# Tanveer81/ReVisionLLM

Measured on AMD Instinct MI355X. Metric: video-segments/sec (whole node), stage-2 100-seg recursion, Vicuna-7B, higher is better.
Workload: dtype fp16

## Files before the change

### include/revision_hip.h

```cpp
#ifndef REVISION_HIP_H
#define REVISION_HIP_H

#include <stddef.h>
#include <stdint.h>

#ifdef __cplusplus
extern "C" {
#endif

#define RV_ABI_VERSION 5

typedef enum { RV_OK = 0, RV_ERR_ARG = -1, RV_ERR_UNBOUND = -2, RV_ERR_HIP = -3, RV_ERR_WORKSPACE = -4 } rv_status;
typedef enum { RV_F32 = 0, RV_BF16 = 1, RV_I32 = 2, RV_I64 = 3, RV_U8 = 4, RV_F16 = 5 } rv_dtype;
typedef enum { RV_ACT_NONE = 0, RV_ACT_RELU = 1, RV_ACT_SILU_MUL = 2, RV_ACT_QUICK_GELU = 3 } rv_act;
typedef enum { RV_W_ROWMAJOR = 0, RV_W_PACKED = 1 } rv_wlayout;
typedef enum { RV_FEAT_CLS = 0, RV_FEAT_ALL = 2 } rv_feature;

typedef struct rv_ctx rv_ctx;

typedef struct rv_config {
    int32_t hidden, inter, layers, heads, vocab;
    float rms_eps, rope_theta;
    int32_t adapter_dim, adapter_heads, adapter_ff, adapter_layers;
    int32_t adapter_text;
} rv_config;

#if defined(__GNUC__)
#pragma GCC visibility push(default)
#endif

int rv_abi_version(void);
int rv_operand_dtype(void);
int rv_last_error(char* buf, size_t n);

int rv_ctx_create(const rv_config* cfg, rv_ctx** out);
void rv_ctx_destroy(rv_ctx* ctx);
int rv_ctx_set_option(rv_ctx* ctx, const char* key, int64_t value);
int rv_ctx_get_option(const rv_ctx* ctx, const char* key, int64_t* value);
int rv_numeric_status_bind(uint32_t* status_dev);
int rv_weights_bind(rv_ctx* ctx, const char* name, const void* dptr, int dtype, int64_t numel);

int rv_init_hash(void* dst, int dtype, int64_t n, uint64_t key, float step, float base, void* stream);

size_t rv_gemm_ws_bytes(void);
int rv_gemv_fp8(const void* A, int64_t lda, const void* W8, const float* w_scale, const float* bias, const float* residual,
                int64_t ldr, void* C, int64_t ldc, int out_dtype, int act, int64_t M, int64_t N, int64_t K, void* stream);
int rv_rmsnorm_quant_fp8(const float* x, const float* w, void* q8, float* scale, int64_t rows, int32_t d, float eps, void* stream);
int rv_quant_rows_fp8(const void* x16, int64_t ldx, void* q8, int64_t ldq, float* scale, int64_t rows, int64_t K, void* stream);
int rv_gemm_fp8(const rv_ctx* ctx , const void* A8, int64_t lda, const float* a_scale, const void* W8p, const float* w_scale, const float* residual,
                int64_t ldr, void* C, int64_t ldc, int out_dtype, int act, int64_t M, int64_t N, int64_t K, void* ws, size_t ws_bytes,
                void* stream);
int rv_gemm(const rv_ctx* ctx , const void* A, int64_t lda, const void* W, int64_t ldw, int w_layout, const float* bias, const float* residual,
            int64_t ldr, void* C, int64_t ldc, int out_dtype, int act, int64_t M, int64_t N, int64_t K, void* ws,
            size_t ws_bytes, void* stream);
size_t rv_gemm_rows_ws_bytes(void);
int rv_gemm_rows(const void* Xp, const void* Wp, const float* w_scale, void* C, int32_t M, int32_t N, int32_t K, void* planes,
                 int32_t* arrive, int act, int out_dtype, void* stream);
int rv_layernorm(const float* x, const float* w, const float* b, float* y_f32, void* y_bf16, void* y_pos_bf16,
                 const float* pos, int64_t period, int64_t rows, int32_t d, void* stream);
int rv_rmsnorm(const float* x, const float* w, void* y_bf16, int64_t rows, int32_t d, float eps, void* stream);
int rv_sine_pos(float* pos, int32_t T, int32_t d, void* stream);
int rv_attention(const void* q, int64_t q_row_stride, int64_t q_batch_stride, const void* k, int64_t k_row_stride,
                 int64_t k_batch_stride, int64_t k_head_stride, const void* vt, int64_t vt_batch_stride,
                 int64_t vt_head_stride, int64_t vt_d_stride, void* out, int64_t o_row_stride, int64_t o_batch_stride,
                 const uint8_t* key_pad, int32_t B, int32_t H, int32_t dh, int32_t Lq, int32_t Lk, int32_t causal,
                 int32_t q_pos0, int32_t kv_batch_div, float scale, void* stream);

int rv_frames_to_patches(const uint8_t* frames, int layout, int64_t frame_stride, int64_t row_stride, int32_t n, int32_t H, int32_t W, int32_t R,
                         int32_t patch, const float mean[3], const float std[3], void* patches, int64_t ldp, float* image, void* stream);

int rv_yuv_to_patches(const uint8_t* y, int64_t y_frame_stride, int64_t y_row_stride, const uint8_t* cb, const uint8_t* cr, int64_t c_frame_stride,
                      int64_t c_row_stride, int32_t c_pix, int32_t n, int32_t H, int32_t W, int32_t matrix, int32_t full_range, int32_t chroma_loc,
                      int32_t R, int32_t patch, const float mean[3], const float std[3], void* patches, int64_t ldp, float* image, void* stream);

typedef struct rv_yuv_surface {
    const void *y, *cb, *cr;
    int64_t y_frame_stride, y_row_stride, c_frame_stride, c_row_stride;
    int32_t sample_bytes;
    int32_t depth;
    int32_t msb_aligned;
    int32_t c_pix;
    int32_t sub_x, sub_y;
    int32_t n, H, W;
    int32_t matrix;
    int32_t full_range;
    int32_t chroma_loc;
} rv_yuv_surface;
int rv_yuv_surface_to_patches(const rv_yuv_surface* s, int32_t R, int32_t patch, const float mean[3], const float std[3], void* patches, int64_t ldp,
                              float* image, void* stream);

int rv_project_dense(rv_ctx* ctx, const void* x_bf16, void* y, int out_dtype, int64_t rows, void* stream);
size_t rv_clip_encoder_ws_bytes(const rv_ctx* ctx, int32_t N, int32_t T, int32_t Nq, int32_t Lq);
int rv_clip_encoder(rv_ctx* ctx, const void* x, const void* txt, const uint8_t* txt_mask, int32_t N, int32_t T,
                    int32_t Nq, int32_t Lq, int32_t feature, float* out, void* ws, size_t ws_bytes, void* stream);

int rv_splice_embed(rv_ctx* ctx, const int32_t* map, const float* video_rows, float* h, int64_t rows, void* stream);
size_t rv_kv_bytes(const rv_ctx* ctx, int32_t B, int32_t Smax);
size_t rv_llm_ws_bytes(const rv_ctx* ctx, int32_t B, int32_t S);
int rv_llm_forward(rv_ctx* ctx, float* h, int32_t B, int32_t S, int32_t pos0, void* kv, int32_t Smax, float* logits,
                   void* ws, size_t ws_bytes, void* stream);

int rv_llm_layers(rv_ctx* ctx, float* h, int32_t B, int32_t S, int32_t pos0, void* kv, int32_t Smax, int32_t layer_begin,
                  int32_t layer_end, void* ws, size_t ws_bytes, void* stream);

size_t rv_llm_prefill_shared_ws_bytes(const rv_ctx* ctx, int32_t B, int32_t P0, int32_t S);
int rv_llm_prefill_shared(rv_ctx* ctx, float* h, int32_t B, int32_t P0, int32_t S, void* kv, int32_t Smax, float* logits,
                          void* ws, size_t ws_bytes, void* stream);

int rv_llm_prefill_pool(rv_ctx* ctx, float* h, int32_t B, int32_t P0, int32_t S, void* kv, int32_t kv_rows, int32_t kv_row0, int32_t Smax,
                        float* logits, void* ws, size_t ws_bytes, void* stream);
int rv_llm_prefill_pool_groups(rv_ctx* ctx, float* h, int32_t G, int32_t B, int32_t P0, int32_t S, void* kv, int32_t kv_rows,
                               const int32_t* kv_row0, int32_t Smax, float* logits, void* ws, size_t ws_bytes, void* stream);
int rv_llm_prefill_pool_groups_ragged(rv_ctx* ctx, float* h, int32_t G, int32_t B, int32_t P0, int32_t S, void* kv, int32_t kv_rows,
                                      const int32_t* kv_row0, int32_t Smax, const int32_t* last_rows, float* logits, void* ws, size_t ws_bytes,
                                      void* stream);
typedef struct rv_prefill_group { int32_t B, P0, S, kv_row0; } rv_prefill_group;
int rv_llm_prefill_pool_mixed(rv_ctx* ctx, float* h, int32_t G, const rv_prefill_group* groups, void* kv, int32_t kv_rows, int32_t Smax,
                              const int32_t* last_rows, float* logits, void* ws, size_t ws_bytes, void* stream);
int rv_llm_decode_rows(rv_ctx* ctx, float* h, int32_t R, const int32_t* row_pos, void* kv, int32_t Smax, float* logits, void* ws,
                       size_t ws_bytes, void* stream);
int rv_llm_decode_rows_shared(rv_ctx* ctx, float* h, int32_t R, const int32_t* row_pos, const int32_t* row_share, void* kv, int32_t Smax,
                              float* logits, void* ws, size_t ws_bytes, void* stream);

int rv_sample(const rv_ctx* ctx , const float* logits, int32_t B, int32_t V, const float* uniforms, int32_t do_sample, float temperature,
              int32_t top_k, float top_p, int32_t* out_tokens, float* out_entropy_proc, float* out_entropy_raw,
              int32_t* out_topk_idx, float* out_topk_val, int32_t* out_nkeep, float* out_threshold, void* stream);
int rv_entropy_stats(const float* logits, int32_t B, int32_t G, int32_t V, float* out, void* stream);
int rv_topk_cosine(const void* feat, int feat_dtype, const float* q_cls, int32_t n, int32_t T, int32_t d, int32_t k,
                   float* out, void* stream);

int rv_topk_pool(const void* video, int dtype, const float* text, int32_t Nv, int32_t T, int32_t d, int32_t Nt, int32_t k,
                 float* out, int32_t* out_idx, void* stream);

#if defined(__GNUC__)
#pragma GCC visibility pop
#endif

#ifdef __cplusplus
}
#endif
#endif
```

### revisionllm_amd/csrc/engine.hip

```cpp
#include <string>
#include <unordered_map>
#include <vector>

#include "kernels.h"

struct Tensor {
    const void* p = nullptr;
    int dtype = 0;
    int64_t numel = 0;
};

struct AdapterLayer {
    const op16_t *w_in, *w_out, *w1, *w2;
    const float *b_in, *b_out, *b1, *b2, *ln1_w, *ln1_b, *ln2_w, *ln2_b;
};
struct LlmLayer {
    const op16_t *wqkv, *wo, *wgu, *wdown;
    const float *norm1, *norm2;
    const uint8_t *wqkv8 = nullptr, *wo8 = nullptr, *wgu8 = nullptr, *wdown8 = nullptr;
    const float *sqkv = nullptr, *so = nullptr, *sgu = nullptr, *sdown = nullptr;
    const uint8_t *wqkv8p = nullptr, *wo8p = nullptr, *wgu8p = nullptr, *wdown8p = nullptr;
    const op16_t *wqkv2 = nullptr, *wo2 = nullptr, *wgu2 = nullptr, *wdown2 = nullptr;
};

// ... 380 lines not shown
        const int64_t RT = (int64_t)Nq * Lq;
        hipLaunchKernelGGL(invert_mask_kernel, dim3((unsigned)cdiv(RT, 256)), dim3(256), 0, st, txt_mask, w.pad, (int)RT);
        RV_CHECK_LAUNCH("invert_mask");
        float* v32 = w.x32;
        op16_t* vp16 = w.xp16;
        RV_TRY(k_frames_in(x, w.pm + d, s16 ? nullptr : v32, vp16, R0, T, (int)d, st));
        const op16_t* vres16 = (const op16_t*)x;
        for (size_t l = 0; l < c->t2v.size(); ++l) {
            const AdapterLayer& L = c->t2v[l];
            op16_t* q16 = w.qk16;
            RV_TRY(rv_gemm_impl(txt, d, L.w_in + d * d, d, 1, L.b_in + d, nullptr, 0, w.tk16, 2 * d, RV_OP16, RV_ACT_NONE, RT, 2 * d, d, w.sk, w.sk_bytes, st));
            const int LK = Lq <= 16 ? 16 : 32;
            const int64_t NK = (int64_t)H * LK, Rq = (int64_t)(N / Nq) * T;
            const bool fold = c->opt.adapter_fold_t2v != 0 && Lq <= 32 && dh <= 128 && NK % 64 == 0 && Rq > 32;
            if (fold) {
                float* S32 = (float*)w.qk16;
                op16_t* P16 = w.a16;
                RV_TRY(k_t2v_fold(L.w_in, L.b_in, L.w_out, w.tk16, w.tv16, 2 * d, Nq, Lq, LK, H, dh, scale, w.fa1, w.fc1, w.fa2, st));
                if (Nq > 1) {
                    RV_TRY(rv_gemm_grouped_impl(vp16, d, w.fa1, NK * d, w.fc1, NK, nullptr, 0, S32, NK, RV_F32, R0, NK, d, Rq, st));
                    RV_TRY(k_t2v_softmax(S32, w.pad, P16, R0, H, LK, Lq, Rq, st));
                    if (s16)
                        RV_TRY(rv_gemm_grouped_impl(P16, NK, w.fa2, NK * d, L.b_out, 0, (const float*)vres16, d, ys16, d, RV_OP16, R0, d, NK, Rq, st, 1));
                    else
                        RV_TRY(rv_gemm_grouped_impl(P16, NK, w.fa2, NK * d, L.b_out, 0, v32, d, w.y32, d, RV_F32, R0, d, NK, Rq, st));
                }
                for (int qi = 0; qi < Nq && Nq == 1; ++qi)
                    RV_TRY(rv_gemm_impl(vp16 + qi * Rq * d, d, w.fa1 + qi * NK * d, d, 1, w.fc1 + qi * NK, nullptr, 0, S32 + qi * Rq * NK, NK, RV_F32, RV_ACT_NONE, Rq, NK, d,
                                        w.sk, w.sk_bytes, st));
                if (Nq == 1) RV_TRY(k_t2v_softmax(S32, w.pad, P16, R0, H, LK, Lq, Rq, st));
                for (int qi = 0; qi < Nq && Nq == 1; ++qi) {
                    const int64_t r0 = qi * Rq;
                    if (s16)
                        RV_TRY(rv_gemm_impl(P16 + r0 * NK, NK, w.fa2 + qi * NK * d, NK, 1, L.b_out, (const float*)(vres16 + r0 * d), d, ys16 + r0 * d, d, RV_OP16, RV_ACT_NONE, Rq, d,
                                            NK, w.sk, w.sk_bytes, st, nullptr, 1));
                    else
                        RV_TRY(rv_gemm_impl(P16 + r0 * NK, NK, w.fa2 + qi * NK * d, NK, 1, L.b_out, v32 + r0 * d, d, w.y32 + r0 * d, d, RV_F32, RV_ACT_NONE, Rq, d, NK, w.sk,
                                            w.sk_bytes, st));
                }
            } else {
                RV_TRY(rv_gemm_impl(vp16, d, L.w_in, d, 1, L.b_in, nullptr, 0, q16, d, RV_OP16, RV_ACT_NONE, R0, d, d, w.sk, w.sk_bytes, st));
                RV_TRY(k_transpose_v(w.tv16, 2 * d, w.tvt16, Nq, Lq, w.Lqpad, H, dh, st));
                AttnArgs a{q16, d, (int64_t)T * d, w.tk16, 2 * d, (int64_t)Lq * 2 * d, dh, w.tvt16, (int64_t)d * w.Lqpad, (int64_t)dh * w.Lqpad,
                           w.Lqpad, w.a16, d, (int64_t)T * d, w.pad, N, H, dh, T, Lq, 0, 0, N / Nq, scale};
                RV_TRY(k_attention(a, st));
            }
            if (s16) {
                if (!fold)
                    RV_TRY(rv_gemm_impl(w.a16, d, L.w_out, d, 1, L.b_out, (const float*)vres16, d, ys16, d, RV_OP16, RV_ACT_NONE, R0, d, d, w.sk, w.sk_bytes, st, nullptr, 1));
                RV_TRY(k_layernorm(nullptr, L.ln1_w, L.ln1_b, nullptr, w.x16, nullptr, nullptr, 0, R0, (int)d, st, 0, ys16));
                RV_TRY(rv_gemm_impl(w.x16, d, L.w1, d, 1, L.b1, nullptr, 0, w.h16, ff, RV_OP16, RV_ACT_RELU, R0, ff, d, w.sk, w.sk_bytes, st));
                RV_TRY(rv_gemm_impl(w.h16, ff, L.w2, ff, 1, L.b2, (const float*)ys16, d, ys16, d, RV_OP16, RV_ACT_NONE, R0, d, ff, w.sk, w.sk_bytes, st, nullptr, 1));
                if (l + 1 < c->t2v.size()) {
                    RV_TRY(k_layernorm(nullptr, L.ln2_w, L.ln2_b, nullptr, xs16, vp16, w.pm + d, T, R0, (int)d, st, 0, ys16));
                    vres16 = xs16;
                } else {
                    RV_TRY(k_layernorm(nullptr, L.ln2_w, L.ln2_b, nullptr, w.x16, w.xp16, w.pm + d, T, R0, (int)d, st, T, ys16));
                    RV_TRY(k_cls_rows(c->cls_token, w.pm, nullptr, w.x16, w.xp16, N, T, (int)d, st));
                }
                continue;
            }
            if (!fold)
                RV_TRY(rv_gemm_impl(w.a16, d, L.w_out, d, 1, L.b_out, v32, d, w.y32, d, RV_F32, RV_ACT_NONE, R0, d, d, w.sk, w.sk_bytes, st));
            RV_TRY(k_layernorm(w.y32, L.ln1_w, L.ln1_b, nullptr, w.x16, nullptr, nullptr, 0, R0, (int)d, st));
            RV_TRY(rv_gemm_impl(w.x16, d, L.w1, d, 1, L.b1, nullptr, 0, w.h16, ff, RV_OP16, RV_ACT_RELU, R0, ff, d, w.sk, w.sk_bytes, st));
            RV_TRY(rv_gemm_impl(w.h16, ff, L.w2, ff, 1, L.b2, w.y32, d, w.y32, d, RV_F32, RV_ACT_NONE, R0, d, ff, w.sk, w.sk_bytes, st));
            if (l + 1 < c->t2v.size()) {
                RV_TRY(k_layernorm(w.y32, L.ln2_w, L.ln2_b, v32, nullptr, vp16, w.pm + d, T, R0, (int)d, st));
            } else {
                RV_TRY(k_layernorm(w.y32, L.ln2_w, L.ln2_b, w.x32, w.x16, w.xp16, w.pm + d, T, R0, (int)d, st, T));
                RV_TRY(k_cls_rows(c->cls_token, w.pm, w.x32, w.x16, w.xp16, N, T, (int)d, st));
            }
        }
    } else {
        RV_TRY(k_build_x(x, nullptr, c->cls_token, w.pm, s16 ? nullptr : w.x32, w.x16, w.xp16, N, T, (int)d, st));
    }

    for (size_t l = 0; l < c->enc.size(); ++l) {
        const AdapterLayer& L = c->enc[l];
        if (feature == RV_FEAT_CLS && l + 1 == c->enc.size() && N > 16 && T >= 3) {
            const int64_t sx = (int64_t)(T + 1) * d;
            op16_t* kk16 = w.qk16;
            op16_t* qc16 = w.h16;
            float* y0 = w.y32;
            float* y1 = w.y32 + (int64_t)N * d;
            float* y2 = w.y32 + (int64_t)2 * N * d;
            RV_TRY(rv_gemm_impl(w.xp16, d, L.w_in + d * d, d, 1, L.b_in + d, nullptr, 0, kk16, d, RV_OP16, RV_ACT_NONE, R1, d, d, w.sk, w.sk_bytes, st));
            RV_TRY(rv_gemm_impl(w.xp16, sx, L.w_in, d, 1, L.b_in, nullptr, 0, qc16, d, RV_OP16, RV_ACT_NONE, N, d, d, w.sk, w.sk_bytes, st, nullptr, 0, 1));
            RV_TRY(rv_gemm_impl(w.x16, d, L.w_in + 2 * d * d, d, 1, L.b_in + 2 * d, nullptr, 0, w.vv16, d, RV_OP16, RV_ACT_NONE, R1, d, d, w.sk, w.sk_bytes, st));
            RV_TRY(k_transpose_v(w.vv16, d, w.vt16, N, T + 1, w.Lpad, H, dh, st));
            AttnArgs a{qc16, d, d, kk16, d, (int64_t)(T + 1) * d, dh, w.vt16, (int64_t)d * w.Lpad, (int64_t)dh * w.Lpad, w.Lpad, w.a16, d, d,
                       nullptr, N, H, dh, 1, T + 1, 0, 0, 1, scale, 1};
            RV_TRY(k_attention(a, st));
            const float* cls_res = w.x32;
            int64_t cls_ld = sx;
            if (s16) {
                float* y3 = w.y32 + (int64_t)3 * N * d;
                RV_TRY(k_rows_to_f32(w.x16, sx, y3, N, (int)d, st));
                cls_res = y3;
                cls_ld = d;
            }
            RV_TRY(rv_gemm_impl(w.a16, d, L.w_out, d, 1, L.b_out, cls_res, cls_ld, y0, d, RV_F32, RV_ACT_NONE, N, d, d, w.sk, w.sk_bytes, st, nullptr, 0, 1));
            RV_TRY(k_layernorm(y0, L.ln1_w, L.ln1_b, y1, w.x16, nullptr, nullptr, 0, N, (int)d, st, 0, nullptr, s16 ? 3 : 0));
            RV_TRY(rv_gemm_impl(w.x16, d, L.w1, d, 1, L.b1, nullptr, 0, w.h16, ff, RV_OP16, RV_ACT_RELU, N, ff, d, w.sk, w.sk_bytes, st, nullptr, 0, 1));
            RV_TRY(rv_gemm_impl(w.h16, ff, L.w2, ff, 1, L.b2, y1, d, y2, d, RV_F32, RV_ACT_NONE, N, d, ff, w.sk, w.sk_bytes, st, nullptr, 0, 1));
            if (!c->adp_proj_w)
                return k_layernorm(y2, L.ln2_w, L.ln2_b, (float*)out, nullptr, nullptr, nullptr, 0, N, (int)d, st);
            RV_TRY(k_layernorm(y2, L.ln2_w, L.ln2_b, nullptr, w.x16, nullptr, nullptr, 0, N, (int)d, st, 0, nullptr, s16 ? 1 : 0));
            return rv_gemm_impl(w.x16, d, c->adp_proj_w, d, 1, c->adp_proj_b, nullptr, 0, out, D, RV_F32, RV_ACT_NONE, N, D, d, w.sk, w.sk_bytes, st, nullptr, 0, 1);
        }
        RV_TRY(rv_gemm_impl(w.xp16, d, L.w_in, d, 1, L.b_in, nullptr, 0, w.qk16, 2 * d, RV_OP16, RV_ACT_NONE, R1, 2 * d, d, w.sk, w.sk_bytes, st));
        RV_TRY(rv_gemm_impl(w.x16, d, L.w_in + 2 * d * d, d, 1, L.b_in + 2 * d, nullptr, 0, w.vv16, d, RV_OP16, RV_ACT_NONE, R1, d, d, w.sk, w.sk_bytes, st));
        RV_TRY(k_transpose_v(w.vv16, d, w.vt16, N, T + 1, w.Lpad, H, dh, st));
        AttnArgs a{w.qk16, 2 * d, (int64_t)(T + 1) * 2 * d, w.qk16 + d, 2 * d, (int64_t)(T + 1) * 2 * d, dh, w.vt16,
                   (int64_t)d * w.Lpad, (int64_t)dh * w.Lpad, w.Lpad, w.a16, d, (int64_t)(T + 1) * d, nullptr, N, H, dh, T + 1,
                   T + 1, 0, 0, 1, scale};
        RV_TRY(k_attention(a, st));
        if (s16) {
            RV_TRY(rv_gemm_impl(w.a16, d, L.w_out, d, 1, L.b_out, (const float*)w.x16, d, ys16, d, RV_OP16, RV_ACT_NONE, R1, d, d, w.sk, w.sk_bytes, st, nullptr, 1));
            RV_TRY(k_layernorm(nullptr, L.ln1_w, L.ln1_b, nullptr, w.x16, nullptr, nullptr, 0, R1, (int)d, st, 0, ys16));
            RV_TRY(rv_gemm_impl(w.x16, d, L.w1, d, 1, L.b1, nullptr, 0, w.h16, ff, RV_OP16, RV_ACT_RELU, R1, ff, d, w.sk, w.sk_bytes, st));
            RV_TRY(rv_gemm_impl(w.h16, ff, L.w2, ff, 1, L.b2, (const float*)w.x16, d, ys16, d, RV_OP16, RV_ACT_NONE, R1, d, ff, w.sk, w.sk_bytes, st, nullptr, 1));
            RV_TRY(k_layernorm(nullptr, L.ln2_w, L.ln2_b, nullptr, w.x16, w.xp16, w.pm, T + 1, R1, (int)d, st, 0, ys16));
            continue;
        }
        RV_TRY(rv_gemm_impl(w.a16, d, L.w_out, d, 1, L.b_out, w.x32, d, w.y32, d, RV_F32, RV_ACT_NONE, R1, d, d, w.sk, w.sk_bytes, st));
        RV_TRY(k_layernorm(w.y32, L.ln1_w, L.ln1_b, w.x32, w.x16, nullptr, nullptr, 0, R1, (int)d, st));
        RV_TRY(rv_gemm_impl(w.x16, d, L.w1, d, 1, L.b1, nullptr, 0, w.h16, ff, RV_OP16, RV_ACT_RELU, R1, ff, d, w.sk, w.sk_bytes, st));
        RV_TRY(rv_gemm_impl(w.h16, ff, L.w2, ff, 1, L.b2, w.x32, d, w.y32, d, RV_F32, RV_ACT_NONE, R1, d, ff, w.sk, w.sk_bytes, st));
        RV_TRY(k_layernorm(w.y32, L.ln2_w, L.ln2_b, w.x32, w.x16, w.xp16, w.pm, T + 1, R1, (int)d, st));
    }
    if (!c->adp_proj_w) {
        const hipError_t e = feature == RV_FEAT_CLS
                                 ? hipMemcpy2DAsync(out, (size_t)d * 4, w.x32, (size_t)(T + 1) * d * 4, (size_t)d * 4, (size_t)N, hipMemcpyDeviceToDevice, st)
                                 : hipMemcpyAsync(out, w.x32, (size_t)R1 * d * 4, hipMemcpyDeviceToDevice, st);
        if (e != hipSuccess) {
            rv_set_error("rv_clip_encoder: output copy failed: %s", hipGetErrorString(e));
            return RV_ERR_HIP;
        }
        return RV_OK;
    }
    if (feature == RV_FEAT_CLS)
        return rv_gemm_impl(w.x16, (int64_t)(T + 1) * d, c->adp_proj_w, d, 1, c->adp_proj_b, nullptr, 0, out, D, RV_F32, RV_ACT_NONE, N, D,
                            d, w.sk, w.sk_bytes, st);
    return rv_gemm_impl(w.x16, d, c->adp_proj_w, d, 1, c->adp_proj_b, nullptr, 0, out, D, RV_F32, RV_ACT_NONE, R1, D, d, w.sk, w.sk_bytes, st);
}

extern "C" int rv_splice_embed(rv_ctx* c, const int32_t* map, const float* video_rows, float* h, int64_t rows, void* stream) {
    RV_CHECK_ARG(c && map && h && rows > 0, "rv_splice_embed: bad arguments");
    RV_TRY(resolve_llm(c));
    return k_splice_embed(map, c->embed, video_rows, h, rows, c->cfg.hidden, as_stream(stream));
}

extern "C" size_t rv_kv_bytes(const rv_ctx* c, int32_t B, int32_t Smax) {
    if (!c || B <= 0 || Smax <= 0) return 0;
    return (size_t)2 * c->cfg.layers * B * c->cfg.hidden * (size_t)Smax * 2;
}

namespace {
inline bool llm_parity(const rv_ctx* c) { return c->opt.precision == 1 && c->w.count("llm.L0.wqkv.p2") != 0 && c->w.count("llm.lm_head.p2") != 0; }
struct LlmWs {
    op16_t *xn16, *q16, *a16, *act16, *xl16;
    float* g32;
    float *cs, *ss;
    float* planes;
    int* arrive;
    uint8_t* x8;
    float* sa;
    void* sk;
    size_t sk_bytes;
    size_t bytes;
};
inline const int* mixed_last_rows(const LlmWs& w) { return (const int*)((const char*)w.ss + sizeof(QkvGroup) * RV_MAX_PREFILL_GROUPS); }
inline size_t mixed_tables_bytes(const rv_ctx* c) { return (size_t)RV_XP_MAX_BLOCKS * (c->cfg.hidden / 16) * 16 * 4; }
LlmWs carve_llm(const rv_ctx* c, void* ws, size_t cap, int B, int S) {
    const int64_t M = (int64_t)B * S, D = c->cfg.hidden, F = c->cfg.inter;
    Carver k(ws, cap);
    LlmWs w;
    w.sk_bytes = gemm_pp_ws_bytes();
    w.sk = k.take(w.sk_bytes);
    w.arrive = (int*)k.take((size_t)RV_ROWS_COUNTERS * 4);
    const int64_t Mp = M <= RV_ROWS_MAX ? 16 * rv_xp_blocks(M) : M;
    const size_t par = llm_parity(c) ? 2 : 1;
    w.xn16 = (op16_t*)k.take((size_t)Mp * D * 2 * par);
    w.q16 = (op16_t*)k.take((size_t)M * D * 2 * par);
    w.a16 = (op16_t*)k.take((size_t)Mp * D * 2 * par);
    w.act16 = (op16_t*)k.take((size_t)Mp * F * 2 * par);
    w.xl16 = (op16_t*)k.take((size_t)Mp * D * 2 * 2);
    w.g32 = (float*)k.take(par == 2 ? (size_t)M * (F > 3 * D ? F : 3 * D) * 4 : 0);
    w.cs = (float*)k.take((size_t)S * (D / c->cfg.heads) * 4);
    w.ss = (float*)k.take((size_t)RV_XP_MAX_BLOCKS * (D / 16) * 16 * 4);
    w.planes = (float*)k.take(gemm_rows_ws_bytes());
    w.x8 = (uint8_t*)k.take((size_t)M * (F > D ? F : D));
    w.sa = (float*)k.take((size_t)M * 4);
    w.bytes = k.off;
    return w;
}
}

extern "C" size_t rv_llm_ws_bytes(const rv_ctx* c, int32_t B, int32_t S) {
    if (!c || B <= 0 || S <= 0) return 0;
    return carve_llm(c, nullptr, 0, 1, B * S).bytes;
}

namespace {
int llm_forward_impl(rv_ctx* c, float* h, int B, int S, int pos0, int P0, void* kv, int Smax, float* logits, void* ws,
                     size_t ws_bytes, hipStream_t st, int kv_rows = 0, int kv_row0 = 0, const int* row_pos = nullptr, int G = 1,
                     const int* grow = nullptr, int l0 = 0, int l1 = -1, const int* row_share = nullptr, const int* last_rows = nullptr,
                     const AttnMixed* mx = nullptr) {
    RV_TRY(resolve_llm(c));
    const rv_config& g = c->cfg;
    if (G > 1) kv_row0 = grow[0];
    const int64_t D = g.hidden, F = g.inter, V = g.vocab, Mg = (int64_t)B * S + P0, M = Mg * G;
    const LlmWs w = carve_llm(c, ws, ws_bytes, 1, (int)M);
    if (w.bytes > ws_bytes) {
        rv_set_error("rv_llm_forward: workspace %zu < required %zu", ws_bytes, w.bytes);
        return RV_ERR_WORKSPACE;
    }
    const int H = g.heads, dh = (int)(D / H);
    if (kv_rows <= 0) kv_rows = B;
    const int64_t per_layer = (int64_t)kv_rows * D * Smax;
    op16_t* kbase = (op16_t*)kv + (int64_t)kv_row0 * D * Smax;
    op16_t* vbase = (op16_t*)kv + (int64_t)g.layers * per_layer + (int64_t)kv_row0 * D * Smax;
    const float scale = 1.0f / sqrtf((float)dh);
    int mx_len = 0, mx_min = 0;
    int64_t nseq = (int64_t)G * B;
    if (mx) {
        nseq = 0;
        for (int gi = 0; gi < mx->G; ++gi) {
            const int len = mx->gt[gi].P0 + mx->gt[gi].S;
            mx_len = len > mx_len ? len : mx_len;
            mx_min = (gi == 0 || len < mx_min) ? len : mx_min;
            nseq += mx->gt[gi].B;
        }
    }
    const int tab0 = P0 > 0 ? 0 : pos0;
    if (row_pos) RV_TRY(k_rope_table_rows(w.cs, row_pos, B, dh, g.rope_theta, st));
    else RV_TRY(k_rope_table(w.cs, mx ? mx_len : pos0 + S - tab0, tab0, dh, g.rope_theta, st));
    const bool par = llm_parity(c);
    if (c->opt.precision == 1 && !par) {
        rv_set_error("rv_llm_forward: precision = 1 (parity) needs the K-duplicated weight copies (\"<name>.p2\") bound");
        return RV_ERR_UNBOUND;
    }
    const bool fuse_norm = !par && S == 1 && P0 == 0 && M <= RV_ROWS_MAX && D % 128 == 0 && F % 128 == 0 && (M <= 32 || (D % 64 == 0 && F % 32 == 0 && V % 64 == 0));
    const bool f8 = fuse_norm && c->fp8_decode && c->opt.fp8_decode;
    const bool p8 = !par && !fuse_norm && M > 32 && c->fp8_prefill && c->opt.fp8_prefill && w.sk_bytes >= 8192;
    const bool p8_qkv = p8 && gemm_pp_fp8_supported(M, 3 * D, D, false, true), p8_o = p8 && gemm_pp_fp8_supported(M, D, D, false, false);
    const bool p8_gu = p8 && gemm_pp_fp8_supported(M, 2 * F, D, true, false), p8_down = p8 && gemm_pp_fp8_supported(M, D, F, false, false);
    auto norm_quant = [&](const float* nw) -> int {
        if (D == 4096) return k_rmsnorm_quant(h, D, nw, w.x8, w.sa, M, (int)D, g.rms_eps, st);
        RV_TRY(k_rmsnorm(h, D, nw, w.xn16, M, (int)D, g.rms_eps, st));
        return k_quant_rows_fp8(w.xn16, D, w.x8, D, w.sa, M, (int)D, st);
    };
    const int nb_d = gemv_blocks(RV_ACT_NONE, D);
    const int xp = fuse_norm ? rv_xp_blocks(M) : 0;
    GemvNorm consume;
    consume.in_sumsq = w.ss;
    consume.in_nblk = nb_d;
    consume.inv_d = 1.0f / (float)D;
    consume.eps = g.rms_eps;
    consume.x_packed = xp;
    consume.out_packed = xp;
    consume.planes = w.planes;
    consume.arrive = w.arrive;
    if (l1 < 0 || l1 > g.layers) l1 = g.layers;
    const bool tail_block = logits && l1 == g.layers && !par && !p8 && !fuse_norm && !row_pos && (S > 1 || P0 > 0) && c->opt.last_block_rows &&
                            (mx ? (int64_t)mx_min : (int64_t)P0 + S) >= 32 && (size_t)M * F * 2 >= (((size_t)nseq * D * 4 + 255) & ~(size_t)255) + (size_t)nseq * F * 2;
    QkvGroup* mx_gt = (QkvGroup*)w.ss;
    if (mx) RV_TRY(k_mixed_tables(*mx, mx_gt, last_rows == mixed_last_rows(w) ? (int*)mixed_last_rows(w) : nullptr, st));
    for (int l = l0; l < l1; ++l) {
        const LlmLayer& L = c->layers[l];
        op16_t* kc = kbase + l * per_layer;
        op16_t* vtc = vbase + l * per_layer;
        if (par) RV_TRY(k_rmsnorm_split(h, D, L.norm1, w.xn16, M, (int)D, g.rms_eps, st));
        else if (p8_qkv) RV_TRY(norm_quant(L.norm1));
        else if (!fuse_norm || l == l0) RV_TRY(k_rmsnorm(h, D, L.norm1, w.xn16, M, (int)D, g.rms_eps, st, xp));
        QkvRope qr;
        qr.cs = w.cs;
        qr.q16 = w.q16;
        qr.kc = kc;
        qr.vtc = vtc;
        qr.B = B; qr.S = S; qr.P0 = P0; qr.pos0 = pos0; qr.cs_pos0 = tab0; qr.H = H; qr.Smax = Smax;
        qr.row_pos = row_pos;
        qr.G = G;
        qr.Mg = (int)Mg;
        for (int gi = 1; gi < G; ++gi) qr.grow[gi] = grow[gi] - grow[0];
        if (mx) {
            qr.ng = mx->G;
            qr.gt = mx_gt;
        }
        if (par) {
            qr.q_ld = (int)(2 * D);
            qr.q_lo = (int)D;
            RV_TRY(rv_gemm_impl(w.xn16, 2 * D, L.wqkv2, 2 * D, 1, nullptr, nullptr, 0, w.g32, 3 * D, RV_F32, RV_ACT_NONE, M, 3 * D, 2 * D, w.sk, w.sk_bytes, st, nullptr));
            RV_TRY(k_qkv_rope_split(w.g32, 3 * D, qr, M, D, st));
        } else if (p8_qkv) {
            RV_TRY(gemm_pp_fp8(w.x8, D, w.sa, L.wqkv8p, L.sqkv, nullptr, 0, nullptr, 0, RV_F32, RV_ACT_NONE, M, 3 * D, D, &qr, w.sk, st));
        } else if (f8) {
            GemvNorm cq = (fuse_norm && l > l0) ? consume : GemvNorm{};
            cq.w_scale = L.sqkv;
            cq.x_packed = xp;
            cq.planes = w.planes;
            cq.arrive = w.arrive;
            RV_TRY(gemm_qkv_rope(w.xn16, D, L.wqkv8, M, D, qr, &cq, nullptr, 0, st, 2));
        } else {
            GemvNorm first;
// ... 330 lines not shown
```

### revisionllm_amd/csrc/kernels.h

```cpp
#pragma once
#include "common.h"

struct RvOpts {
    int gemm_tile_variant = 2;
    int gemm_cus = 0;
    int fp8_decode = 1;
    int fp8_prefill = 1;
    int sample_variant = 1;
    int gemm_arows = 1;
    int gemm_waves = 8;
    int gemm_mhalf = 2;
    int rows_single = 1;
    int rows_persistent = 1;
    int rows_spread = 0;
    int rows_fill = 240;
    int lm_head_split = 1;
    int last_block_rows = 1;
    int adapter_stream16 = 1;
    int adapter_fold_t2v = 1;
    int attn_lds = 1;
    int qkv_lds = 1;
    int precision = 0;
};
extern const RvOpts g_default_opts;
// ... 50 lines not shown
    const QkvGroup e = q.gt[gi];
    m -= e.base;
    return e;
}
#ifndef RS_PROBE
#define RS_PROBE_K_ 0
#else
#define RS_PROBE_K_ RS_PROBE
#endif
static __device__ __forceinline__ f32x4 qkv_rope_coeffs(const QkvRope& q, int m, int n) {
    const int D = q.H * 128;
    const int sec = n / D, p = (n - sec * D) & 127;
    if (sec >= 2) return f32x4{0.f, 0.f, 0.f, 0.f};
    if constexpr ((RS_PROBE_K_ & 4096) != 0) return f32x4{1.f, 0.f, 1.f, 0.f};
    if (q.row_pos) return *(const f32x4*)(q.cs + ((int64_t)m * 64 + (p >> 1)) * 2);
    int P0 = q.P0, S = q.S, pos0 = q.pos0;
    if (q.ng) { const QkvGroup e = qkv_rope_group(q, m); P0 = pos0 = e.P0; S = e.S; }
    else if (q.G > 1) m -= (m / q.Mg) * q.Mg;
    int pos;
    if (m < P0) pos = m;
    else { const int r = m - P0; const int b = r / S; pos = pos0 + (r - b * S); }
    return *(const f32x4*)(q.cs + ((int64_t)(pos - q.cs_pos0) * 64 + (p >> 1)) * 2);
}
template <bool QSPLIT>
static __device__ __forceinline__ void qkv_rope_store_t(const QkvRope& q, int m, int n, f32x4 v, f32x4 t) {
    const int D = q.H * 128;
    const int sec = n / D, hd = n - sec * D, head = hd >> 7, p = hd & 127;
    int b, pos, goff = 0;
    bool prefix = false;
    const int mrow = m;
    int B = q.B, P0 = q.P0, S = q.S, pos0 = q.pos0;
    if (q.ng) { const QkvGroup e = qkv_rope_group(q, m); B = e.B; P0 = pos0 = e.P0; S = e.S; goff = e.row; }
    else if (q.G > 1) { const int gi = m / q.Mg; m -= gi * q.Mg; goff = q.grow[gi]; }
    if (q.row_pos) { b = m; pos = (RS_PROBE_K_ & 8192) ? 170 + (m & 7) : q.row_pos[m]; if (pos < 0 || pos >= q.Smax) return; }
    else if (m < P0) { b = 0; pos = m; prefix = true; }
    else { const int r = m - P0; b = r / S; pos = pos0 + (r - b * S); }
    if (sec < 2) {
        const float a0 = __fmaf_rn(v[0], t[0], -__fmul_rn(v[1], t[1])), b0 = __fmaf_rn(v[1], t[0], __fmul_rn(v[0], t[1]));
        const float a1 = __fmaf_rn(v[2], t[2], -__fmul_rn(v[3], t[3])), b1 = __fmaf_rn(v[3], t[2], __fmul_rn(v[2], t[3]));
        const u32x2 o = pack_op16x4(f32x4{a0, b0, a1, b1});
        if (sec == 0) {
            if constexpr ((RS_PROBE_K_ & 1024) != 0) return;
            if constexpr (QSPLIT) {
                op16_t* dst = (op16_t*)q.q16 + (int64_t)mrow * q.q_ld + hd;
                *(u32x2*)dst = o;
                *(u32x2*)(dst + q.q_lo) = u32x2{pack_op16x2_lo(a0, b0), pack_op16x2_lo(a1, b1)};
            } else {
                *(u32x2*)((op16_t*)q.q16 + (int64_t)mrow * D + hd) = o;
            }
        } else {
            if constexpr ((RS_PROBE_K_ & 512) != 0) return;
            const int b0_ = (prefix ? 0 : b) + goff, b1_ = (prefix ? B : b + 1) + goff;
            for (int bb = b0_; bb < b1_; ++bb)
                *(u32x2*)((op16_t*)q.kc + (((int64_t)bb * q.H + head) * q.Smax + pos) * 128 + p) = o;
        }
    } else {
        if constexpr ((RS_PROBE_K_ & 256) != 0) return;
        const int b0_ = (prefix ? 0 : b) + goff, b1_ = (prefix ? B : b + 1) + goff;
        for (int bb = b0_; bb < b1_; ++bb) {
            op16_t* dst = (op16_t*)q.vtc + ((int64_t)bb * q.H + head) * 128 * q.Smax + rv_vt_index(p, pos);
#pragma unroll
            for (int r = 0; r < 4; ++r) dst[r * 8] = f32_to_op16(v[r]);
        }
    }
}
static __device__ __forceinline__ void qkv_rope_store(const QkvRope& q, int m, int n, f32x4 v, f32x4 t) { qkv_rope_store_t<false>(q, m, n, v, t); }
struct QkvRow {
    int mrow, pos, b0, b1;
    const float* cs;
};
static __device__ __forceinline__ QkvRow qkv_rope_row(const QkvRope& q, int m) {
    QkvRow r;
    r.mrow = m;
    int goff = 0, b;
    bool prefix = false;
    int mt = m;
    int B = q.B, P0 = q.P0, S = q.S, pos0 = q.pos0;
    if (q.ng) { const QkvGroup e = qkv_rope_group(q, mt); B = e.B; P0 = pos0 = e.P0; S = e.S; goff = e.row; }
    else if (q.G > 1) { const int gi = m / q.Mg; mt = m - gi * q.Mg; goff = q.grow[gi]; }
    if (q.row_pos) { b = mt; r.pos = q.row_pos[mt]; r.cs = q.cs + (int64_t)mt * 128; }
    else {
        if (mt < P0) { b = 0; r.pos = mt; prefix = true; }
        else { const int rr = mt - P0; b = rr / S; r.pos = pos0 + (rr - b * S); }
        r.cs = q.cs + (int64_t)(r.pos - q.cs_pos0) * 128;
    }
    r.b0 = (prefix ? 0 : b) + goff;
    r.b1 = (prefix ? B : b + 1) + goff;
    if (q.row_pos && (r.pos < 0 || r.pos >= q.Smax)) r.b1 = r.b0 - 1;
    return r;
}
static __device__ __forceinline__ void qkv_rope_store(const QkvRope& q, int m, int n, f32x4 v) {
    qkv_rope_store(q, m, n, v, qkv_rope_coeffs(q, m, n));
}

int gemm_qkv_rope(const void* A, int64_t lda, const void* Wp, int64_t M, int64_t D, const QkvRope& r, const GemvNorm* norm,
                  void* ws, size_t ws_bytes, hipStream_t st, int w_layout = 1, int64_t Kdim = 0);

int rv_gemm_impl(const void* A, int64_t lda, const void* W, int64_t ldw, int w_layout, const float* bias,
                 const float* residual, int64_t ldr, void* C, int64_t ldc, int out_dtype, int act, int64_t M, int64_t N,
                 int64_t K, void* ws, size_t ws_bytes, hipStream_t st, const GemvNorm* norm = nullptr, int res16 = 0, int no_stream = 0);
struct GemmGroups {
    int rows = 0, tiles = 0;
    int64_t w_stride = 0, bias_stride = 0;
};
int rv_gemm_grouped_impl(const void* A, int64_t lda, const void* Wp, int64_t w_stride, const float* bias, int64_t bias_stride, const float* residual, int64_t ldr, void* C,
                         int64_t ldc, int out_dtype, int64_t M, int64_t N, int64_t K, int64_t rows_per_group, hipStream_t st, int res16 = 0);
int gemv_blocks(int act, int64_t N);
int gemm_rows(const op16_t* X, const op16_t* W, const float* bias, const float* res, int64_t ldr, void* C, int64_t ldc, int out_dtype, int act,
              int M, int N, int K, hipStream_t st, const GemvNorm& nrm, const QkvRope* qr, int w_layout = 1);
size_t gemm_rows_ws_bytes();
bool gemm_arows_supported(int w_layout, int act, int64_t M, int64_t N, int64_t K);
int gemm_arows_launch(const void* A, int64_t lda, const void* Wp, const float* bias, const float* res, int64_t ldr, void* C, int64_t ldc,
                      int out_dtype, int act, int64_t M, int64_t N, int64_t K, hipStream_t st);
bool gemm_pp_supported(int w_layout, int64_t M, int64_t N, int64_t K);
bool gemm_pp_sk_supported(int w_layout, int64_t M, int64_t N, int64_t K);
int gemm_pp_sk_plan(int64_t M, int64_t N, int64_t K, bool gated);
bool gemm_pp_sk_profitable(int64_t M, int64_t N, int64_t K);
bool gemm_pp_dp_profitable(int64_t M, int64_t N, int64_t K);
int gemm_pp_dp_plan(int64_t M, int64_t N, int64_t K, bool gated);
size_t gemm_pp_ws_bytes();
bool gemm_pp_fp8_supported(int64_t M, int64_t N, int64_t K, bool gated, bool rope);
int gemm_pp_fp8(const void* A8, int64_t lda, const float* sa, const void* W8p, const float* sw, const float* res, int64_t ldr, void* C,
                int64_t ldc, int out_dtype, int act, int64_t M, int64_t N, int64_t K, const QkvRope* r, void* ws, hipStream_t st);
int gemm_pp_launch(const void* A, int64_t lda, const void* Wp, const float* bias, const float* res, int64_t ldr, void* C,
                   int64_t ldc, int out_dtype, int act, int64_t M, int64_t N, int64_t K, void* ws, hipStream_t st);
int gemm_pp_qkv_rope(const void* A, int64_t lda, const void* Wp, int64_t M, int64_t N, int64_t K, const QkvRope& r, void* ws,
                     hipStream_t st);
int k_layernorm(const float* x, const float* w, const float* b, float* y32, void* y16, void* yp16, const float* pos,
                int64_t period, int64_t rows, int d, hipStream_t st, int64_t gap = 0, const void* x_op16 = nullptr, int rnd = 0);
int k_rmsnorm_quant(const float* x, int64_t x_row_stride, const float* w, void* q8, float* scale, int64_t rows, int d, float eps,
                    hipStream_t st);
int k_quant_rows_fp8(const void* x16, int64_t ldx, void* q8, int64_t ldq, float* scale, int64_t rows, int K, hipStream_t st);
int k_rmsnorm(const float* x, int64_t x_row_stride, const float* w, void* y16, int64_t rows, int d, float eps, hipStream_t st,
              int out_packed = 0, const int* row_idx = nullptr);
int k_rmsnorm_split(const float* x, int64_t x_row_stride, const float* w, void* y16, int64_t rows, int d, float eps, hipStream_t st, int out_packed = 0,
                    const int* row_idx = nullptr);
int k_split_bf16(const float* x, int64_t ldx, void* y16, int64_t rows, int n, hipStream_t st);
int k_qkv_rope_split(const float* qkv32, int64_t ld, const QkvRope& qr, int64_t M, int64_t D, hipStream_t st);
int k_gather_last_rows(const void* a16, const float* h, const int* idx, int64_t rows, int Mg, int P0, int B, int S, void* a_out, float* h_out, int D, hipStream_t st);
int k_t2v_fold(const void* wq_p, const float* bq, const void* wo_p, const void* tk16, const void* tv16, int64_t ld, int Nq, int Lq, int LK, int H, int dh, float scale,
               void* A1p, float* c1, void* A2p, hipStream_t st);
int k_t2v_softmax(const float* S, const uint8_t* pad, void* P16, int64_t rows, int H, int LK, int Lq, int64_t rows_per_query, hipStream_t st);
int k_sine_pos(float* pos, int T, int d, hipStream_t st);
int k_frames_in(const void* x16, const float* pos, float* v32, void* vp16, int64_t rows, int T, int d, hipStream_t st);
int k_build_x(const void* src16, const float* src32, const float* cls, const float* pm, float* x32, void* x16, void* xp16,
              int64_t N, int T, int d, hipStream_t st);
int k_copy_f32(const float* src, float* dst, int64_t n, hipStream_t st);
int k_rows_to_f32(const void* src16, int64_t ld, float* dst, int64_t rows, int d, hipStream_t st);
int k_cls_rows(const float* cls, const float* pm, float* x32, void* x16, void* xp16, int64_t N, int T, int d, hipStream_t st);
int k_transpose_v(const void* v, int64_t ld, void* vt, int64_t Nb, int L, int Lpad, int H, int dh, hipStream_t st);
int k_rope_table(float* cs, int S, int pos0, int dh, float theta, hipStream_t st);
int k_rope_table_rows(float* cs, const int* row_pos, int rows, int dh, float theta, hipStream_t st);
int k_splice_embed(const int32_t* map, const void* embed, const float* video, float* h, int64_t rows, int D, hipStream_t st);

struct AttnArgs {
    const void* q; int64_t q_rs, q_bs;
    const void* k; int64_t k_rs, k_bs, k_hs;
    const void* vt; int64_t vt_bs, vt_hs, vt_ds;
    void* out; int64_t o_rs, o_bs;
    const uint8_t* key_pad;
    int B, H, dh, Lq, Lk, causal, q_pos0, kv_div;
    float scale;
    int no_split = 0;
    const int* row_pos = nullptr;
    int out_packed = 0;
    int64_t vt_ks = 8;
    int64_t out_lo = 0;
    int64_t q_lo = 0;
    const int* row_share = nullptr;
};
int k_attention(const AttnArgs& a, hipStream_t st);
struct AttnGroups {
    int G = 1;
    int64_t q_off[RV_MAX_PREFILL_GROUPS] = {0, 0, 0, 0, 0, 0, 0, 0};
    int64_t o_off[RV_MAX_PREFILL_GROUPS] = {0, 0, 0, 0, 0, 0, 0, 0};
    int64_t kv_off[RV_MAX_PREFILL_GROUPS] = {0, 0, 0, 0, 0, 0, 0, 0};
};
int k_attention_pair(const AttnArgs& a, const AttnArgs& b, hipStream_t st, const AttnGroups* groups = nullptr);
int k_attention_groups(const AttnArgs& a, hipStream_t st, const AttnGroups& groups);
struct AttnMixed {
    int G = 0, problems = 0;
    int first[RV_MAX_PREFILL_GROUPS] = {};
    QkvGroup gt[RV_MAX_PREFILL_GROUPS] = {};
};
int k_attention_mixed(const AttnArgs& a, const AttnMixed& mx, hipStream_t st);
int k_mixed_tables(const AttnMixed& mx, QkvGroup* gt, int* last_rows, hipStream_t st);
```

### revisionllm_amd/csrc/rowops.hip

```cpp
#include "common.h"
#include "kernels.h"

namespace {

template <int NV>
__global__ __launch_bounds__(256) void layernorm_kernel(const float* __restrict__ x, const float* __restrict__ w,
                                                        const float* __restrict__ b, float* __restrict__ y32,
                                                        op16_t* __restrict__ y16, op16_t* __restrict__ yp16,
                                                        const float* __restrict__ pos, int64_t period, int64_t rows, int64_t gap,
                                                        const op16_t* __restrict__ x16in, int rnd) {
    constexpr int D = NV * 256;
    const int lane = threadIdx.x & 63;
    const int64_t row = (int64_t)blockIdx.x * 4 + (threadIdx.x >> 6);
    if (row >= rows) return;
    const float* xr = x + row * D;
    const int64_t orow = gap > 0 ? row + row / gap + 1 : row;
    f32x4 v[NV];
    float s = 0.f;
#pragma unroll
    for (int i = 0; i < NV; ++i) {
        v[i] = x16in ? op16x4_to_f32(*(const u32x2*)(x16in + row * D + i * 256 + lane * 4)) : *(const f32x4*)(xr + i * 256 + lane * 4);
        if (rnd & 1) v[i] = op16x4_to_f32(pack_op16x4(f32x4{v[i][0], v[i][1], v[i][2], v[i][3]}));
        s += v[i][0] + v[i][1] + v[i][2] + v[i][3];
    }
// ... 300 lines not shown
__device__ __forceinline__ int64_t rv_wp_index(int n, int k, int K) {
    return ((((int64_t)(n >> 4) * (K >> 5) + (k >> 5)) * 64 + (n & 15) + 16 * ((k >> 3) & 3)) * 8) + (k & 7);
}
__global__ __launch_bounds__(256) void t2v_fold_kernel(const op16_t* __restrict__ wq_p, const float* __restrict__ bq, const op16_t* __restrict__ wo_p,
                                                       const op16_t* __restrict__ tk, const op16_t* __restrict__ tv, int64_t ld, int Lq, int LK, int H, int dh, int d, float scale,
                                                       op16_t* __restrict__ A1p, float* __restrict__ c1, op16_t* __restrict__ A2p) {
    const int k = blockIdx.x * 256 + threadIdx.x;
    const int hj = blockIdx.y, h = hj / LK, j = hj % LK, q = blockIdx.z;
    const int NK = H * LK;
    __shared__ float kr[128], vr[128];
    const bool valid = j < Lq;
    for (int t = threadIdx.x; t < dh; t += 256) {
        kr[t] = valid ? op16_to_f32(tk[((int64_t)q * Lq + j) * ld + h * dh + t]) : 0.f;
        vr[t] = valid ? op16_to_f32(tv[((int64_t)q * Lq + j) * ld + h * dh + t]) : 0.f;
    }
    __syncthreads();
    if (k < d) {
        float a1 = 0.f, a2 = 0.f;
        for (int t = 0; t < dh; ++t) {
            a1 += kr[t] * op16_to_f32(wq_p[rv_wp_index(h * dh + t, k, d)]);
            a2 += vr[t] * op16_to_f32(wo_p[rv_wp_index(k, h * dh + t, d)]);
        }
        A1p[(int64_t)q * NK * d + rv_wp_index(hj, k, d)] = f32_to_op16(a1 * scale);
        A2p[(int64_t)q * NK * d + rv_wp_index(k, hj, NK)] = f32_to_op16(a2);
    }
    if (blockIdx.x == 0 && threadIdx.x < 64) {
        float c = 0.f;
        for (int t = threadIdx.x; t < dh; t += 64) c += kr[t] * bq[h * dh + t];
        c = wave_sum(c);
        if (threadIdx.x == 0) c1[(int64_t)q * NK + hj] = c * scale;
    }
}
template <int DH, int LK>
__global__ __launch_bounds__(256) void t2v_fold_reg_kernel(const op16_t* __restrict__ wq_p, const float* __restrict__ bq, const op16_t* __restrict__ wo_p,
                                                           const op16_t* __restrict__ tk, const op16_t* __restrict__ tv, int64_t ld, int Lq, int H, int d, float scale,
                                                           op16_t* __restrict__ A1p, float* __restrict__ c1, op16_t* __restrict__ A2p, int Nq, int qpw) {
    const int which = blockIdx.x & 1;
    const int k = (blockIdx.x >> 1) * 256 + threadIdx.x;
    const int h = blockIdx.y;
    const int NK = H * LK;
    __shared__ __attribute__((aligned(16))) float rr[LK][DH];
    float w[DH];
    const int kc = k < d ? k : d - 1;
#pragma unroll
    for (int t = 0; t < DH; ++t) w[t] = op16_to_f32(which ? wo_p[rv_wp_index(kc, h * DH + t, d)] : wq_p[rv_wp_index(h * DH + t, kc, d)]);
    const op16_t* rows = which ? tv : tk;
    const float mul = which ? 1.0f : scale;
    for (int q = blockIdx.z * qpw; q < Nq && q < (blockIdx.z + 1) * qpw; ++q) {
        __syncthreads();
        for (int i = threadIdx.x; i < LK * DH; i += 256) {
            const int j = i / DH, t = i - j * DH;
            rr[j][t] = j < Lq ? op16_to_f32(rows[((int64_t)q * Lq + j) * ld + h * DH + t]) : 0.f;
        }
        __syncthreads();
        if (k < d) {
#pragma unroll 2
            for (int j = 0; j < LK; ++j) {
                float acc = 0.f;
#pragma unroll
                for (int t = 0; t < DH; t += 4) {
                    const f32x4 kk = *(const f32x4*)&rr[j][t];
#pragma unroll
                    for (int e = 0; e < 4; ++e) acc += kk[e] * w[t + e];
                }
                const int hj = h * LK + j;
                if (which) A2p[(int64_t)q * NK * d + rv_wp_index(k, hj, NK)] = f32_to_op16(acc);
                else A1p[(int64_t)q * NK * d + rv_wp_index(hj, k, d)] = f32_to_op16(acc * mul);
            }
        }
        if (blockIdx.x == 0 && threadIdx.x < 64) {
            for (int j = 0; j < LK; ++j) {
                float c = 0.f;
                for (int t = threadIdx.x; t < DH; t += 64) c += rr[j][t] * bq[h * DH + t];
                c = wave_sum(c);
                if (threadIdx.x == 0) c1[(int64_t)q * NK + h * LK + j] = c * scale;
            }
        }
    }
}

template <int LK>
__global__ __launch_bounds__(256) void t2v_softmax_kernel(const float* __restrict__ S, const uint8_t* __restrict__ pad, op16_t* __restrict__ P, int64_t rows, int H, int Lq,
                                                          int64_t rows_per_query) {
    const int64_t i = (int64_t)blockIdx.x * 256 + threadIdx.x;
    if (i >= rows * H) return;
    const int64_t r = i / H;
    const uint8_t* pq = pad + (r / rows_per_query) * Lq;
    unsigned valid = 0u;
    for (int j = 0; j < Lq; ++j) valid |= (pq[j] == 0 ? 1u : 0u) << j;
    const f32x4* s4 = (const f32x4*)(S + i * LK);
    f32x4 v[LK / 4];
    float mx = -INFINITY;
#pragma unroll
    for (int c = 0; c < LK / 4; ++c) {
        v[c] = s4[c];
#pragma unroll
        for (int e = 0; e < 4; ++e) {
            if (!((valid >> (c * 4 + e)) & 1u)) v[c][e] = -INFINITY;
            mx = fmaxf(mx, v[c][e]);
        }
    }
    float z = 0.f;
#pragma unroll
    for (int c = 0; c < LK / 4; ++c)
#pragma unroll
        for (int e = 0; e < 4; ++e) {
            v[c][e] = mx == -INFINITY ? 0.f : __expf(v[c][e] - mx);
            z += v[c][e];
        }
    const float iz = z > 0.f ? 1.0f / z : 0.f;
    u32x2* p2 = (u32x2*)(P + i * LK);
#pragma unroll
    for (int c = 0; c < LK / 4; ++c) p2[c] = pack_op16x4(f32x4{v[c][0] * iz, v[c][1] * iz, v[c][2] * iz, v[c][3] * iz});
}

__global__ void rope_table_kernel(float2* __restrict__ cs, int S, int pos0, int dh, float theta) {
    const int i = blockIdx.x * blockDim.x + threadIdx.x;
    const int half = dh / 2;
    if (i >= S * half) return;
    const int s = i / half, j = i % half;
    const float inv = 1.0f / powf(theta, (float)(2 * j) / (float)dh);
    const float ang = (float)(pos0 + s) * inv;
    cs[i] = make_float2(cosf(ang), sinf(ang));
}

__global__ void rope_table_rows_kernel(float2* __restrict__ cs, const int* __restrict__ row_pos, int rows, int dh, float theta) {
    const int i = blockIdx.x * blockDim.x + threadIdx.x;
    const int half = dh / 2;
    if (i >= rows * half) return;
    const int s = i / half, j = i % half;
    const int pos = row_pos[s] > 0 ? row_pos[s] : 0;
    const float inv = 1.0f / powf(theta, (float)(2 * j) / (float)dh);
    const float ang = (float)pos * inv;
    cs[i] = make_float2(cosf(ang), sinf(ang));
}

__global__ __launch_bounds__(256) void splice_embed_kernel(const int32_t* __restrict__ map, const op16_t* __restrict__ embed,
                                                           const float* __restrict__ video, float* __restrict__ h, int D) {
    const int64_t r = blockIdx.x;
    const int src = map[r];
    float* o = h + r * D;
    if (src >= 0) {
        const op16_t* e = embed + (int64_t)src * D;
        for (int c = threadIdx.x * 4; c < D; c += 1024) {
            const u32x2 raw = *(const u32x2*)(e + c);
            *(f32x4*)(o + c) = op16x4_to_f32(raw);
        }
    } else {
        const float* v = video + (int64_t)(-(src + 1)) * D;
        for (int c = threadIdx.x * 4; c < D; c += 1024) *(f32x4*)(o + c) = *(const f32x4*)(v + c);
    }
}

}

int k_layernorm(const float* x, const float* w, const float* b, float* y32, void* y16, void* yp16, const float* pos,
                int64_t period, int64_t rows, int d, hipStream_t st, int64_t gap, const void* x_op16, int rnd) {
    RV_CHECK_ARG((x || x_op16) && w && b && rows >= 0, "layernorm: bad arguments");
    RV_CHECK_ARG(!yp16 || (pos && period > 0), "layernorm: y_pos needs pos table and period");
    if (rows == 0) return RV_OK;
    const unsigned blocks = (unsigned)cdiv(rows, 4);
    if (d == 768)
        hipLaunchKernelGGL(layernorm_kernel<3>, dim3(blocks), dim3(256), 0, st, x, w, b, y32, (op16_t*)y16, (op16_t*)yp16, pos, period, rows, gap, (const op16_t*)x_op16, rnd);
    else if (d == 4096)
        hipLaunchKernelGGL(layernorm_kernel<16>, dim3(blocks), dim3(256), 0, st, x, w, b, y32, (op16_t*)y16, (op16_t*)yp16, pos, period, rows, gap, (const op16_t*)x_op16, rnd);
    else if (d == 1024)
        hipLaunchKernelGGL(layernorm_kernel<4>, dim3(blocks), dim3(256), 0, st, x, w, b, y32, (op16_t*)y16, (op16_t*)yp16, pos, period, rows, gap, (const op16_t*)x_op16, rnd);
    else if (d == 256)
        hipLaunchKernelGGL(layernorm_kernel<1>, dim3(blocks), dim3(256), 0, st, x, w, b, y32, (op16_t*)y16, (op16_t*)yp16, pos, period, rows, gap, (const op16_t*)x_op16, rnd);
    else if (d == 512)
        hipLaunchKernelGGL(layernorm_kernel<2>, dim3(blocks), dim3(256), 0, st, x, w, b, y32, (op16_t*)y16, (op16_t*)yp16, pos, period, rows, gap, (const op16_t*)x_op16, rnd);
    else {
        rv_set_error("layernorm: unsupported width %d (256, 512, 768, 1024, 4096)", d);
        return RV_ERR_ARG;
    }
    RV_CHECK_LAUNCH("layernorm");
    return RV_OK;
}

int k_rmsnorm(const float* x, int64_t x_row_stride, const float* w, void* y16, int64_t rows, int d, float eps, hipStream_t st, int out_packed, const int* row_idx) {
    RV_CHECK_ARG(x && w && y16 && d % 4 == 0 && x_row_stride % 4 == 0, "rmsnorm: bad arguments");
    RV_CHECK_ARG(!out_packed || (rows <= 16 * out_packed && d % 32 == 0), "rmsnorm: the packed decode layout holds <= 16 rows per block");
    if (rows == 0) return RV_OK;
    const dim3 grid((unsigned)cdiv(rows, 4));
    if (d == 4096)
        hipLaunchKernelGGL(rmsnorm_kernel<16>, grid, dim3(256), 0, st, x, x_row_stride, w, (op16_t*)y16, rows, d, eps, out_packed, row_idx);
    else if (d == 512)
        hipLaunchKernelGGL(rmsnorm_kernel<2>, grid, dim3(256), 0, st, x, x_row_stride, w, (op16_t*)y16, rows, d, eps, out_packed, row_idx);
    else
        hipLaunchKernelGGL(rmsnorm_kernel<0>, grid, dim3(256), 0, st, x, x_row_stride, w, (op16_t*)y16, rows, d, eps, out_packed, row_idx);
    RV_CHECK_LAUNCH("rmsnorm");
    return RV_OK;
}

int k_rmsnorm_split(const float* x, int64_t x_row_stride, const float* w, void* y16, int64_t rows, int d, float eps, hipStream_t st, int out_packed, const int* row_idx) {
    RV_CHECK_ARG(x && w && y16 && d % 4 == 0 && x_row_stride % 4 == 0, "rmsnorm_split: bad arguments");
    RV_CHECK_ARG(!out_packed || (rows <= 16 * out_packed && d % 32 == 0), "rmsnorm_split: the packed decode layout holds <= 16 rows per block");
    if (rows == 0) return RV_OK;
    hipLaunchKernelGGL(rmsnorm_split_kernel, dim3((unsigned)cdiv(rows, 4)), dim3(256), 0, st, x, x_row_stride, w, (op16_t*)y16, rows, d, eps, out_packed, row_idx);
    RV_CHECK_LAUNCH("rmsnorm_split");
    return RV_OK;
}

int k_qkv_rope_split(const float* qkv32, int64_t ld, const QkvRope& qr, int64_t M, int64_t D, hipStream_t st) {
    RV_CHECK_ARG(qkv32 && qr.cs && qr.q16 && qr.kc && qr.vtc && qr.q_ld >= 2 * D && qr.q_lo >= D && ld % 4 == 0 && D == (int64_t)qr.H * 128, "qkv_rope_split: bad arguments");
    if (M == 0) return RV_OK;
    hipLaunchKernelGGL(qkv_rope_split_kernel, dim3((unsigned)cdiv(M * (3 * D / 4), 256)), dim3(256), 0, st, qkv32, ld, qr, M, (int)(3 * D));
    RV_CHECK_LAUNCH("qkv_rope_split");
    return RV_OK;
}

int k_split_bf16(const float* x, int64_t ldx, void* y16, int64_t rows, int n, hipStream_t st) {
    RV_CHECK_ARG(x && y16 && n % 4 == 0 && ldx % 4 == 0, "split_bf16: bad arguments");
    if (rows == 0) return RV_OK;
    hipLaunchKernelGGL(split_bf16_kernel, dim3((unsigned)cdiv(rows * n / 4, 256)), dim3(256), 0, st, x, ldx, (op16_t*)y16, rows, n);
    RV_CHECK_LAUNCH("split_bf16");
    return RV_OK;
}

int k_quant_rows_fp8(const void* x16, int64_t ldx, void* q8, int64_t ldq, float* scale, int64_t rows, int K, hipStream_t st) {
    RV_CHECK_ARG(x16 && q8 && scale && K > 0 && K % 8 == 0 && ldx % 8 == 0 && ldq % 8 == 0, "quant_rows_fp8: K, ldx, ldq must be multiples of 8");
    if (rows == 0) return RV_OK;
    hipLaunchKernelGGL(quant_rows_fp8_kernel, dim3((unsigned)cdiv(rows, 4)), dim3(256), 0, st, (const op16_t*)x16, ldx, (uint8_t*)q8, ldq,
                       scale, rows, K);
    RV_CHECK_LAUNCH("quant_rows_fp8");
    return RV_OK;
}

int k_rmsnorm_quant(const float* x, int64_t x_row_stride, const float* w, void* q8, float* scale, int64_t rows, int d, float eps,
                    hipStream_t st) {
    RV_CHECK_ARG(d == 4096, "rmsnorm_quant: d = %d (only 4096 is instantiated)", d);
    if (rows == 0) return RV_OK;
    hipLaunchKernelGGL(rmsnorm_quant_kernel<16>, dim3((unsigned)cdiv(rows, 4)), dim3(256), 0, st, x, x_row_stride, w, (uint8_t*)q8, scale, rows,
                       d, eps);
    RV_CHECK_LAUNCH("rmsnorm_quant");
    return RV_OK;
}

int k_sine_pos(float* pos, int T, int d, hipStream_t st) {
    RV_CHECK_ARG(pos && T > 0 && d > 0, "sine_pos: bad arguments");
    hipLaunchKernelGGL(sine_pos_kernel, dim3((unsigned)cdiv((int64_t)T * d, 256)), dim3(256), 0, st, pos, T, d);
    RV_CHECK_LAUNCH("sine_pos");
    return RV_OK;
}

int k_frames_in(const void* x16, const float* pos, float* v32, void* vp16, int64_t rows, int T, int d, hipStream_t st) {
    hipLaunchKernelGGL(frames_in_kernel, dim3((unsigned)cdiv(rows * d / 4, 256)), dim3(256), 0, st, (const op16_t*)x16, pos, v32,
                       (op16_t*)vp16, rows, T, d);
    RV_CHECK_LAUNCH("frames_in");
    return RV_OK;
}

int k_build_x(const void* src16, const float* src32, const float* cls, const float* pm, float* x32, void* x16, void* xp16,
              int64_t N, int T, int d, hipStream_t st) {
    hipLaunchKernelGGL(build_x_kernel, dim3((unsigned)cdiv(N * (T + 1) * d / 4, 256)), dim3(256), 0, st, (const op16_t*)src16,
                       src32, cls, pm, x32, (op16_t*)x16, (op16_t*)xp16, N, T, d);
    RV_CHECK_LAUNCH("build_x");
    return RV_OK;
}

int k_cls_rows(const float* cls, const float* pm, float* x32, void* x16, void* xp16, int64_t N, int T, int d, hipStream_t st) {
    hipLaunchKernelGGL(cls_rows_kernel, dim3((unsigned)cdiv(N * d / 4, 256)), dim3(256), 0, st, cls, pm, x32, (op16_t*)x16, (op16_t*)xp16, N, T, d);
    RV_CHECK_LAUNCH("cls_rows");
    return RV_OK;
}

int k_rows_to_f32(const void* src16, int64_t ld, float* dst, int64_t rows, int d, hipStream_t st) {
    hipLaunchKernelGGL(rows_to_f32_kernel, dim3((unsigned)cdiv(rows * d / 4, 256)), dim3(256), 0, st, (const op16_t*)src16, ld, dst, rows, d);
    RV_CHECK_LAUNCH("rows_to_f32");
    return RV_OK;
}

int k_copy_f32(const float* src, float* dst, int64_t n, hipStream_t st) {
    hipLaunchKernelGGL(copy_f32_kernel, dim3((unsigned)cdiv(n, 256)), dim3(256), 0, st, src, dst, n);
    RV_CHECK_LAUNCH("copy_f32");
    return RV_OK;
}

int k_transpose_v(const void* v, int64_t ld, void* vt, int64_t Nb, int L, int Lpad, int H, int dh, hipStream_t st) {
    RV_CHECK_ARG(Lpad % 2 == 0 && Lpad >= L, "transpose_v: bad Lpad");
    dim3 grid((unsigned)cdiv(Lpad, 64), (unsigned)H, (unsigned)Nb);
    if (dh == 96)
        hipLaunchKernelGGL(transpose_v_kernel<96>, grid, dim3(256), 0, st, (const op16_t*)v, ld, (op16_t*)vt, L, Lpad, H);
    else if (dh == 128)
        hipLaunchKernelGGL(transpose_v_kernel<128>, grid, dim3(256), 0, st, (const op16_t*)v, ld, (op16_t*)vt, L, Lpad, H);
    else if (dh == 512)
        hipLaunchKernelGGL(transpose_v_kernel<512>, dim3(grid.x, grid.y * 4, grid.z), dim3(256), 0, st, (const op16_t*)v, ld, (op16_t*)vt, L, Lpad, H);
    else {
        rv_set_error("transpose_v: head dim %d unsupported", dh);
        return RV_ERR_ARG;
    }
    RV_CHECK_LAUNCH("transpose_v");
    return RV_OK;
}

int k_gather_last_rows(const void* a16, const float* h, const int* idx, int64_t rows, int Mg, int P0, int B, int S, void* a_out, float* h_out, int D, hipStream_t st) {
    RV_CHECK_ARG(a16 && h && a_out && h_out && rows > 0 && D % 4 == 0, "gather_last_rows: bad arguments");
    hipLaunchKernelGGL(gather_last_rows_kernel, dim3((unsigned)rows), dim3(256), 0, st, (const op16_t*)a16, h, idx, Mg, P0, B, S, (op16_t*)a_out, h_out, D);
    RV_CHECK_LAUNCH("gather_last_rows");
    return RV_OK;
}

int k_t2v_fold(const void* wq_p, const float* bq, const void* wo_p, const void* tk16, const void* tv16, int64_t ld, int Nq, int Lq, int LK, int H, int dh, float scale,
               void* A1p, float* c1, void* A2p, hipStream_t st) {
    const int d = H * dh;
    RV_CHECK_ARG(wq_p && bq && wo_p && tk16 && tv16 && A1p && c1 && A2p && ld >= d && Nq > 0 && Lq > 0 && Lq <= LK && (LK == 16 || LK == 32) && dh <= 128 && d % 32 == 0,
                 "t2v_fold: bad arguments");
#define RV_FOLD_REG(DH_, LK_)                                                                                                                                  \
    hipLaunchKernelGGL((t2v_fold_reg_kernel<DH_, LK_>), dim3((unsigned)(2 * cdiv(d, 256)), (unsigned)H, (unsigned)cdiv(Nq, qpw)), dim3(256), 0, st, (const op16_t*)wq_p, bq, \
                       (const op16_t*)wo_p, (const op16_t*)tk16, (const op16_t*)tv16, ld, Lq, H, d, scale, (op16_t*)A1p, c1, (op16_t*)A2p, Nq, qpw)
    const bool reg = Nq >= 3;
    const int qpw = (int)cdiv((int64_t)Nq * 2 * cdiv(d, 256) * H, 1024);
    if (reg && dh == 96 && LK == 16) RV_FOLD_REG(96, 16);
    else if (reg && dh == 96 && LK == 32) RV_FOLD_REG(96, 32);
    else if (reg && dh == 64 && LK == 16) RV_FOLD_REG(64, 16);
    else if (reg && dh == 64 && LK == 32) RV_FOLD_REG(64, 32);
    else
        hipLaunchKernelGGL(t2v_fold_kernel, dim3((unsigned)cdiv(d, 256), (unsigned)(H * LK), (unsigned)Nq), dim3(256), 0, st, (const op16_t*)wq_p, bq, (const op16_t*)wo_p,
                           (const op16_t*)tk16, (const op16_t*)tv16, ld, Lq, LK, H, dh, d, scale, (op16_t*)A1p, c1, (op16_t*)A2p);
#undef RV_FOLD_REG
    RV_CHECK_LAUNCH("t2v_fold");
    return RV_OK;
}

int k_t2v_softmax(const float* S, const uint8_t* pad, void* P16, int64_t rows, int H, int LK, int Lq, int64_t rows_per_query, hipStream_t st) {
    RV_CHECK_ARG(S && pad && P16 && rows > 0 && (LK == 16 || LK == 32) && Lq <= LK && rows_per_query > 0, "t2v_softmax: bad arguments");
    if (LK == 16)
        hipLaunchKernelGGL(t2v_softmax_kernel<16>, dim3((unsigned)cdiv(rows * H, 256)), dim3(256), 0, st, S, pad, (op16_t*)P16, rows, H, Lq, rows_per_query);
    else
        hipLaunchKernelGGL(t2v_softmax_kernel<32>, dim3((unsigned)cdiv(rows * H, 256)), dim3(256), 0, st, S, pad, (op16_t*)P16, rows, H, Lq, rows_per_query);
    RV_CHECK_LAUNCH("t2v_softmax");
    return RV_OK;
}

int k_rope_table(float* cs, int S, int pos0, int dh, float theta, hipStream_t st) {
    hipLaunchKernelGGL(rope_table_kernel, dim3((unsigned)cdiv((int64_t)S * (dh / 2), 256)), dim3(256), 0, st, (float2*)cs, S, pos0, dh, theta);
    RV_CHECK_LAUNCH("rope_table");
    return RV_OK;
}

int k_rope_table_rows(float* cs, const int* row_pos, int rows, int dh, float theta, hipStream_t st) {
    hipLaunchKernelGGL(rope_table_rows_kernel, dim3((unsigned)cdiv((int64_t)rows * (dh / 2), 256)), dim3(256), 0, st, (float2*)cs, row_pos, rows, dh, theta);
    RV_CHECK_LAUNCH("rope_table_rows");
    return RV_OK;
}

int k_splice_embed(const int32_t* map, const void* embed, const float* video, float* h, int64_t rows, int D, hipStream_t st) {
    hipLaunchKernelGGL(splice_embed_kernel, dim3((unsigned)rows), dim3(256), 0, st, map, (const op16_t*)embed, video, h, D);
    RV_CHECK_LAUNCH("splice_embed");
    return RV_OK;
}

extern "C" int rv_layernorm(const float* x, const float* w, const float* b, float* y_f32, void* y_bf16, void* y_pos_bf16,
                            const float* pos, int64_t period, int64_t rows, int32_t d, void* stream) {
    return k_layernorm(x, w, b, y_f32, y_bf16, y_pos_bf16, pos, period, rows, d, as_stream(stream));
}
extern "C" int rv_rmsnorm(const float* x, const float* w, void* y_bf16, int64_t rows, int32_t d, float eps, void* stream) {
    return k_rmsnorm(x, d, w, y_bf16, rows, d, eps, as_stream(stream));
}
extern "C" int rv_rmsnorm_quant_fp8(const float* x, const float* w, void* q8, float* scale, int64_t rows, int32_t d, float eps, void* stream) {
    RV_CHECK_ARG(x && w && q8 && scale, "rv_rmsnorm_quant_fp8: null argument");
    return k_rmsnorm_quant(x, d, w, q8, scale, rows, d, eps, as_stream(stream));
}
extern "C" int rv_sine_pos(float* pos, int32_t T, int32_t d, void* stream) { return k_sine_pos(pos, T, d, as_stream(stream)); }
```

### revisionllm_amd/engine.py

```python
import ctypes as C

import torch

from . import hip, ops
from .utils import synth


def _dev_f32(t, device):
    return t.to(device=device, dtype=torch.float32).contiguous()


def _dev16(t, device, dtype):
    if dtype == torch.float16 and t.dtype != torch.float16:
        t = t.to(device=device, dtype=torch.float32).clamp(-65504.0, 65504.0)
    return t.to(device=device, dtype=dtype).contiguous()


class PersistGate:

    _by_device = {}

    def __init__(self):
        self._event = None

    @classmethod
    def for_device(cls, device):
        key = torch.device(device).index or 0
        if key not in cls._by_device:
            cls._by_device[key] = cls()
        return cls._by_device[key]

    def begin(self, stream=None):
        if self._event is not None:
            (stream or torch.cuda.current_stream()).wait_event(self._event)

    def end(self, stream=None):
        ev = torch.cuda.Event()
        ev.record(stream or torch.cuda.current_stream())
        self._event = ev


class Engine:
    def __init__(self, shape: synth.LlamaShape = synth.VICUNA_7B, adapter_text=True, device="cuda:0", adapter_dim=768,
                 adapter_heads=8, adapter_ff=2048, adapter_layers=2, gate=None, op_dtype=None):
        if not torch.cuda.is_available():
            raise hip.HipLibraryError("no GPU visible: revisionllm_amd runs only on the HIP device path")
        self.flavour = hip.flavour_of(op_dtype)
        self.op_dtype = hip.op_dtype(self.flavour)
        self.lib = hip.lib(self.flavour)
        self.shape = shape
        self.device = torch.device(device)
        self.adapter_text = bool(adapter_text)
        self.adapter_dim, self.adapter_ff, self.adapter_layers = adapter_dim, adapter_ff, adapter_layers
        cfg = hip.RvConfig(shape.hidden, shape.inter, shape.layers, shape.heads, shape.vocab, shape.eps, shape.theta,
                           adapter_dim, adapter_heads, adapter_ff, adapter_layers, int(adapter_text))
        self._ctx = C.c_void_p()
        hip.check(self.lib.rv_ctx_create(C.byref(cfg), C.byref(self._ctx)), "rv_ctx_create")
        self._keep = {}
        self._ws = {}
        self.slot = 0
        self.slots_in_flight = set()
        self.gate = gate if gate is not None else PersistGate.for_device(self.device)
        self.has_llm = self.has_clip = self.has_linear = False
        self.numeric_status = hip.numeric_status(self.flavour, self.device)
        self.on_saturation = "warn"
        self.saturated_seen = 0

    def __del__(self):
        try:
            if getattr(self, "_ctx", None) and self._ctx.value:
                self.lib.rv_ctx_destroy(self._ctx)
                self._ctx = C.c_void_p()
        except Exception:
            pass

    def set_option(self, key, value):
        hip.check(self.lib.rv_ctx_set_option(self._ctx, key.encode(), int(value)), f"rv_ctx_set_option({key})")
        return self

    def get_option(self, key):
        v = C.c_int64()
        hip.check(self.lib.rv_ctx_get_option(self._ctx, key.encode(), C.byref(v)), f"rv_ctx_get_option({key})")
        return int(v.value)

    def _dev16(self, t):
        return _dev16(t, self.device, self.op_dtype)

    def _dev_packed(self, t):
        return ops.pack_fragments(self._dev16(t))

    def bind(self, name, t):
        assert t.is_cuda and t.is_contiguous()
        self._keep[name] = t
        hip.check(self.lib.rv_weights_bind(self._ctx, name.encode(), hip.ptr(t), hip.dtype_code(t), t.numel()),
                  f"rv_weights_bind({name})")

    def weight(self, name):
        return self._keep[name]

    def _loaded(self):
        if self.device.type == "cuda":
            torch.cuda.synchronize(self.device)

    def _bind_matrix(self, name, w, fp8, fp8_prefill=False, parity=False):
        self.bind(name, ops.pack_fragments(w))
        if parity:
            self.bind(name + ".p2", ops.pack_fragments(torch.cat([w, w], dim=1).contiguous()))
        if fp8 or fp8_prefill:
            q, sc = ops.quantize_rows_fp8(w)
            self.bind(name + ".s8", sc)
            if fp8:
                self.bind(name + ".f8", ops.pack_fp8_decode(q))
            if fp8_prefill:
                self.bind(name + ".f8p", ops.pack_fp8_prefill(q))

    def load_llm(self, get, fp8_decode=False, fp8_prefill=False, parity=False):
        s, dev = self.shape, self.device
        self.parity = bool(parity)
        self.fp8_decode = bool(fp8_decode)
        self.fp8_prefill = bool(fp8_prefill)
        self.bind("llm.embed", self._dev16(get("model.embed_tokens.weight")))
        self._bind_matrix("llm.lm_head", self._dev16(get("lm_head.weight")), fp8_decode, parity=True)
        self.bind("llm.norm", _dev_f32(get("model.norm.weight"), dev))
        for i in range(s.layers):
            p = f"model.layers.{i}."
            q, k, v = (self._dev16(get(p + f"self_attn.{n}_proj.weight")) for n in "qkv")
            q, k = pair_interleave_heads(q, s.heads), pair_interleave_heads(k, s.heads)
            self._bind_matrix(f"llm.L{i}.wqkv", torch.cat([q, k, v], dim=0).contiguous(), fp8_decode, fp8_prefill, parity)
            del q, k, v
            self._bind_matrix(f"llm.L{i}.wo", self._dev16(get(p + "self_attn.o_proj.weight")), fp8_decode, fp8_prefill, parity)
            g = self._dev16(get(p + "mlp.gate_proj.weight"))
            u = self._dev16(get(p + "mlp.up_proj.weight"))
            self._bind_matrix(f"llm.L{i}.wgu", pack_gate_up(g, u), fp8_decode, fp8_prefill, parity)
            del g, u
            self._bind_matrix(f"llm.L{i}.wdown", self._dev16(get(p + "mlp.down_proj.weight")), fp8_decode, fp8_prefill, parity)
            self.bind(f"llm.L{i}.norm1", _dev_f32(get(p + "input_layernorm.weight"), dev))
            self.bind(f"llm.L{i}.norm2", _dev_f32(get(p + "post_attention_layernorm.weight"), dev))
        self.has_llm = True
        self._loaded()

    def load_clip_adapter(self, get):
        dev = self.device
        self.bind("adp.cls_token", _dev_f32(get("global_rep_token"), dev))
        self.bind("adp.cls_pos", _dev_f32(get("global_rep_pos"), dev))
        if self.adapter_dim == self.shape.hidden and self.adapter_dim != 768:
            self.txt_proj = (self._dev_packed(get("text_mm_projector.weight")), _dev_f32(get("text_mm_projector.bias"), dev))
        else:
            self.bind("adp.proj_w", self._dev_packed(get("mm_projector.weight")))
            self.bind("adp.proj_b", _dev_f32(get("mm_projector.bias"), dev))
        stacks = ([("t2v_encoder", "t2v")] if self.adapter_text else []) + [("encoder", "enc")]
        for ref, tag in stacks:
            for l in range(self.adapter_layers):
                r, o = f"{ref}.layers.{l}.", f"adp.{tag}.{l}."
                self.bind(o + "w_in", self._dev_packed(get(r + "self_attn.in_proj_weight")))
                self.bind(o + "b_in", _dev_f32(get(r + "self_attn.in_proj_bias"), dev))
                self.bind(o + "w_out", self._dev_packed(get(r + "self_attn.out_proj.weight")))
                self.bind(o + "b_out", _dev_f32(get(r + "self_attn.out_proj.bias"), dev))
                self.bind(o + "w1", self._dev_packed(get(r + "linear1.weight")))
                self.bind(o + "b1", _dev_f32(get(r + "linear1.bias"), dev))
                self.bind(o + "w2", self._dev_packed(get(r + "linear2.weight")))
                self.bind(o + "b2", _dev_f32(get(r + "linear2.bias"), dev))
                for n in ("1", "2"):
                    self.bind(o + f"ln{n}_w", _dev_f32(get(r + f"norm{n}.weight"), dev))
                    self.bind(o + f"ln{n}_b", _dev_f32(get(r + f"norm{n}.bias"), dev))
        self.has_clip = True
        self._loaded()

    def load_linear_projector(self, get):
        if self.adapter_dim != 768:
            self.frame_proj = (self._dev_packed(get("weight")), _dev_f32(get("bias"), self.device))
        else:
            self.bind("proj.w", self._dev_packed(get("weight")))
            self.bind("proj.b", _dev_f32(get("bias"), self.device))
        self.has_linear = True
        self._loaded()

    def _synth_get(self, spec, seed, prefix, grid=None):
        table = {n: (shp, a, base) for n, shp, a, base in spec}
        grid_dt = {None: None, "bf16": torch.bfloat16, "f16": torch.float16}[grid]

        def get(name):
            shp, a, base = table[name]
            t = torch.empty(shp, dtype=torch.float32, device=self.device)
            ops.init_hash_(t, prefix + name, seed, a, base)
            if grid_dt is not None and len(shp) > 1:
                t = t.to(grid_dt).float()
            return t
        return get

    def init_synthetic(self, seed=0, llm=True, clip=True, linear=False, llm_prefix="", clip_prefix="model.mm_projector.",
                       linear_prefix="model.mm_projector.", fp8_decode=False, fp8_prefill=False, cond=None, parity=False, grid=None):
        if llm:
            self.load_llm(self._synth_get(synth.llama_spec(self.shape, cond=cond), seed, llm_prefix, grid), fp8_decode=fp8_decode, fp8_prefill=fp8_prefill, parity=parity)
        if clip:
            self.load_clip_adapter(self._synth_get(synth.clip_encoder_spec(hidden=self.shape.hidden, text=self.adapter_text,
                                                                           cross_attn=self.adapter_dim != 768), seed,
                                                   clip_prefix, grid))
        if linear:
            self.load_linear_projector(self._synth_get(synth.linear_projector_spec(hidden=self.shape.hidden), seed, linear_prefix, grid))
        return self

    def _workspace(self, key, nbytes):
        key = (self.slot, key)
        t = self._ws.get(key)
        if t is None or t.numel() < nbytes:
            t = torch.zeros(max(int(nbytes), 256), dtype=torch.uint8, device=self.device)
            self._ws[key] = t
        return t

    _NUMERIC_KEY = ("numeric", "saturated")

    def _status_words(self):
        words = [(key, ws[8188:8192].view(torch.int32)) for key, ws in list(self._ws.items())
                 if isinstance(key, tuple) and key[0] != "kv" and key[1] in ("llm", "clip") and ws.numel() >= 8192]
        if words:
            words.append((self._NUMERIC_KEY, self.numeric_status[:1]))
        return words

    def saturated(self, reset=False):
        n = self.get_option("saturated")
        if reset:
            self.set_option("saturated", 0)
            self.saturated_seen = 0
        return n

    def _note_saturation(self, count):
        if count <= self.saturated_seen:
            return
        new, self.saturated_seen = count - self.saturated_seen, count
        msg = (f"{new} fp16 store(s) saturated at +-65504 since the last check ({count} in total): activations of this checkpoint leave the fp16 range; "
               "the affected elements lost accuracy (no inf was produced).  Use op_dtype='bf16' for the reference's exponent range.")
        if self.on_saturation == "raise":
            raise hip.HipLibraryError(msg)
        if self.on_saturation == "warn":
            import warnings
            warnings.warn(msg, RuntimeWarning, stacklevel=3)

    def handoff_status_async(self):
        words = self._status_words()
        if not words:
            return None
        host = torch.empty(len(words), dtype=torch.int32, pin_memory=True)
        host.copy_(torch.cat([w for _, w in words]), non_blocking=True)
        return [k for k, _ in words], host

    def check_handoff_status(self, snapshot=None):
        if snapshot is None:
            words = self._status_words()
            if not words:
                return
            keys, vals = [k for k, _ in words], torch.cat([w for _, w in words]).cpu()
        else:
            keys, vals = snapshot
        bad = [(k, int(v)) for k, v in zip(keys, vals.tolist()) if v != 0 and k != self._NUMERIC_KEY]
        sat = [int(v) & 0xffffffff for k, v in zip(keys, vals.tolist()) if k == self._NUMERIC_KEY]
        if sat:
            self._note_saturation(sat[0])
        if bad:
            for k, _ in bad:
                ws = self._ws.get(k)
                if ws is not None:
                    ws[8188:8192].zero_()
            key, st = bad[0]
            raise hip.HipLibraryError(f"workspace '{key}': an in-kernel hand-off wait timed out (status {st}); results of the last calls are invalid")

    def project_dense(self, x, out_dtype=torch.float32):
        lead = x.shape[:-1]
        x2 = self._dev16(x).reshape(-1, x.shape[-1])
        y = torch.empty(x2.shape[0], self.shape.hidden, dtype=out_dtype, device=self.device)
        hip.check(self.lib.rv_project_dense(self._ctx, hip.ptr(x2), hip.ptr(y), hip.dtype_code(y), x2.shape[0], hip.stream()),
                  "rv_project_dense")
        return y.reshape(*lead, self.shape.hidden)

    def clip_encoder(self, x, txt=None, txt_mask=None, feature="cls"):
        N, T, _ = x.shape
        x = self._dev16(x)
        wide = self.adapter_dim != 768
        if wide:
            if getattr(self, "frame_proj", None) is None or getattr(self, "txt_proj", None) is None:
                raise hip.HipLibraryError("the cross_attn ClipEncoder needs the Linear projector (load_linear_projector) and its text projector bound")
            x = ops.gemm(x.reshape(N * T, -1), self.frame_proj[0], bias=self.frame_proj[1], out_dtype=self.op_dtype, w_packed=True,
                         ctx=self).view(N, T, self.adapter_dim)
        if self.adapter_text:
            txt = self._dev16(txt)
            Nq, Lq = txt.shape[0], txt.shape[1]
            if wide:
                txt = ops.gemm(txt.reshape(Nq * Lq, -1), self.txt_proj[0], bias=self.txt_proj[1], out_dtype=self.op_dtype, w_packed=True,
                               ctx=self).view(Nq, Lq, self.adapter_dim)
            m = ops.h2d((txt_mask != 0).to(torch.uint8), self.device).contiguous()
        else:
            txt, m, Nq, Lq = None, None, 0, 0
        feat = hip.RV_FEAT_CLS if feature == "cls" else hip.RV_FEAT_ALL
        D = self.shape.hidden
        out = torch.empty((N, D) if feat == hip.RV_FEAT_CLS else (N, T + 1, D), dtype=torch.float32, device=self.device)
        nbytes = self.lib.rv_clip_encoder_ws_bytes(self._ctx, N, T, Nq, Lq)
        ws = self._workspace("clip", nbytes)
        hip.check(self.lib.rv_clip_encoder(self._ctx, hip.ptr(x), hip.ptr(txt), hip.ptr(m), N, T, Nq, Lq, feat, hip.ptr(out),
                                           hip.ptr(ws), ws.numel(), hip.stream()), "rv_clip_encoder")
        return out

    def splice_embed(self, row_map, video_rows):
        B, S = row_map.shape
        h = torch.empty(B, S, self.shape.hidden, dtype=torch.float32, device=self.device)
        rm = ops.h2d(row_map, self.device, torch.int32).contiguous()
        vr = _dev_f32(video_rows, self.device) if video_rows is not None else None
        hip.check(self.lib.rv_splice_embed(self._ctx, hip.ptr(rm), hip.ptr(vr), hip.ptr(h), B * S, hip.stream()), "rv_splice_embed")
        return h

    def new_kv(self, B, Smax, reuse=True):
        Smax = (Smax + 31) // 32 * 32
        key = ("kv", self.slot, B, Smax)
        t = self._ws.get(key) if reuse else None
        if t is None:
            nbytes = self.lib.rv_kv_bytes(self._ctx, B, Smax)
            t = torch.zeros(nbytes // 2, dtype=self.op_dtype, device=self.device)
            if reuse:
                for k_ in [k_ for k_ in self._ws if isinstance(k_, tuple) and k_[0] == "kv" and k_[1] == self.slot][:-3]:
                    del self._ws[k_]
                self._ws[key] = t
        return t, Smax

    @staticmethod
    def vt_logical(vt, *lead, head_dim=128, Smax=None):
        return vt.view(*lead, Smax // 8, head_dim, 8).movedim(-3, -2).reshape(*lead, head_dim, Smax)

    def _persist_begin(self):
        self.gate.begin(torch.cuda.current_stream(self.device))

    def _persist_end(self):
        self.gate.end(torch.cuda.current_stream(self.device))

    def llm_forward(self, h, pos0, kv, Smax, logits=None):
        B, S, _ = h.shape
        assert h.dtype == torch.float32 and h.is_contiguous()
        if logits is None:
            logits = torch.empty(B, self.shape.vocab, dtype=torch.float32, device=self.device)
        nbytes = self.lib.rv_llm_ws_bytes(self._ctx, B, S)
        ws = self._workspace("llm", nbytes)
        if B * S > 16:
            self._persist_begin()
        hip.check(self.lib.rv_llm_forward(self._ctx, hip.ptr(h), B, S, pos0, hip.ptr(kv), Smax, hip.ptr(logits), hip.ptr(ws),
                                          ws.numel(), hip.stream()), "rv_llm_forward")
        if B * S > 16:
            self._persist_end()
        return logits


    def llm_layers(self, h, pos0, kv, Smax, layer_begin, layer_end):
        B, S, _ = h.shape
        assert h.dtype == torch.float32 and h.is_contiguous()
        ws = self._workspace("llm", self.lib.rv_llm_ws_bytes(self._ctx, B, S))
        if B * S > 16:
            self._persist_begin()
        hip.check(self.lib.rv_llm_layers(self._ctx, hip.ptr(h), B, S, pos0, hip.ptr(kv), Smax, layer_begin, layer_end, hip.ptr(ws), ws.numel(),
                                         hip.stream()), "rv_llm_layers")
        if B * S > 16:
            self._persist_end()
        return h

    def llm_prefill_shared(self, h, B, P0, kv, Smax, logits=None):
        assert h.dtype == torch.float32 and h.is_contiguous() and (h.shape[0] - P0) % B == 0
        S = (h.shape[0] - P0) // B
        if logits is None:
            logits = torch.empty(B, self.shape.vocab, dtype=torch.float32, device=self.device)
        ws = self._workspace("llm", self.lib.rv_llm_prefill_shared_ws_bytes(self._ctx, B, P0, S))
        self._persist_begin()
        hip.check(self.lib.rv_llm_prefill_shared(self._ctx, hip.ptr(h), B, P0, S, hip.ptr(kv), Smax, hip.ptr(logits), hip.ptr(ws),
                                                 ws.numel(), hip.stream()), "rv_llm_prefill_shared")
        self._persist_end()
        return logits


    def new_kv_pool(self, rows, Smax):
        Smax = (Smax + 31) // 32 * 32
        nbytes = self.lib.rv_kv_bytes(self._ctx, rows, Smax)
        return torch.zeros(nbytes // 2, dtype=self.op_dtype, device=self.device), Smax

    def llm_prefill_pool(self, h, B, P0, kv, kv_rows, kv_row0, Smax, logits=None):
        assert h.dtype == torch.float32 and h.is_contiguous() and (h.shape[0] - P0) % B == 0
        S = (h.shape[0] - P0) // B
        if logits is None:
            logits = torch.empty(B, self.shape.vocab, dtype=torch.float32, device=self.device)
        ws = self._workspace("llm", self.lib.rv_llm_prefill_shared_ws_bytes(self._ctx, B, P0, S))
        self._persist_begin()
        hip.check(self.lib.rv_llm_prefill_pool(self._ctx, hip.ptr(h), B, P0, S, hip.ptr(kv), kv_rows, kv_row0, Smax, hip.ptr(logits), hip.ptr(ws),
                                               ws.numel(), hip.stream()), "rv_llm_prefill_pool")
        self._persist_end()
        return logits

    def llm_prefill_pool_groups(self, h, G, B, P0, kv, kv_rows, row0s, Smax, logits=None, last_rows=None):
        import ctypes
        assert h.dtype == torch.float32 and h.is_contiguous() and h.shape[0] % G == 0 and (h.shape[0] // G - P0) % B == 0
        S = (h.shape[0] // G - P0) // B
        if logits is None:
            logits = torch.empty(G * B, self.shape.vocab, dtype=torch.float32, device=self.device)
        ws = self._workspace("llm", self.lib.rv_llm_ws_bytes(self._ctx, h.shape[0], 1))
        rows = (ctypes.c_int32 * G)(*[int(r) for r in row0s])
        self._persist_begin()
        if last_rows is not None:
            assert last_rows.dtype == torch.int32 and last_rows.is_cuda and last_rows.numel() == G * B
            hip.check(self.lib.rv_llm_prefill_pool_groups_ragged(self._ctx, hip.ptr(h), G, B, P0, S, hip.ptr(kv), kv_rows, rows, Smax, hip.ptr(last_rows),
                                                                 hip.ptr(logits), hip.ptr(ws), ws.numel(), hip.stream()), "rv_llm_prefill_pool_groups_ragged")
        else:
            hip.check(self.lib.rv_llm_prefill_pool_groups(self._ctx, hip.ptr(h), G, B, P0, S, hip.ptr(kv), kv_rows, rows, Smax, hip.ptr(logits), hip.ptr(ws),
                                                          ws.numel(), hip.stream()), "rv_llm_prefill_pool_groups")
        self._persist_end()
        return logits

    def mixed_prefill_supported(self):
        return not (self.get_option("precision") == 1 or (getattr(self, "fp8_prefill", False) and self.get_option("fp8_prefill")))

    def llm_prefill_pool_mixed(self, h, groups, kv, R, Smax, last_rows=None, logits=None):
        groups = [tuple(int(v) for v in g) for g in groups]
        rows, nb = sum(P0 + B * S for B, P0, S, _ in groups), sum(g[0] for g in groups)
        assert h.dtype == torch.float32 and h.is_contiguous() and h.shape[0] == rows, (tuple(h.shape), rows)
        if logits is None:
            logits = torch.empty(nb, self.shape.vocab, dtype=torch.float32, device=self.device)
        ws = self._workspace("llm", self.lib.rv_llm_ws_bytes(self._ctx, max(rows, 1), 1))
        tab = (hip.RvPrefillGroup * max(len(groups), 1))(*[hip.RvPrefillGroup(*g) for g in groups])
        if last_rows is not None:
            assert last_rows.dtype == torch.int32 and last_rows.is_cuda and last_rows.numel() == nb
        self._persist_begin()
        try:
            hip.check(self.lib.rv_llm_prefill_pool_mixed(self._ctx, hip.ptr(h), len(groups), tab, hip.ptr(kv), R, Smax, hip.ptr(last_rows), hip.ptr(logits), hip.ptr(ws),
                                                         ws.numel(), hip.stream()), "rv_llm_prefill_pool_mixed")
        finally:
            self._persist_end()
        return logits

    def llm_decode_rows(self, h, row_pos, kv, Smax, logits=None, row_share=None):
        R = h.shape[0]
        assert h.dtype == torch.float32 and h.is_contiguous() and row_pos.dtype == torch.int32 and row_pos.is_cuda
        if logits is None:
            logits = torch.empty(R, self.shape.vocab, dtype=torch.float32, device=self.device)
        ws = self._workspace("llm", self.lib.rv_llm_ws_bytes(self._ctx, R, 1))
        if row_share is not None:
            assert row_share.dtype == torch.int32 and row_share.is_cuda and row_share.numel() == R
            hip.check(self.lib.rv_llm_decode_rows_shared(self._ctx, hip.ptr(h), R, hip.ptr(row_pos), hip.ptr(row_share), hip.ptr(kv), Smax, hip.ptr(logits),
                                                         hip.ptr(ws), ws.numel(), hip.stream()), "rv_llm_decode_rows_shared")
            return logits
        hip.check(self.lib.rv_llm_decode_rows(self._ctx, hip.ptr(h), R, hip.ptr(row_pos), hip.ptr(kv), Smax, hip.ptr(logits), hip.ptr(ws), ws.numel(),
                                              hip.stream()), "rv_llm_decode_rows")
        return logits


def pair_interleave_heads(w, heads):
    rows, D = w.shape
    dh = rows // heads
    return w.view(heads, 2, dh // 2, D).transpose(1, 2).reshape(rows, D).contiguous()


def pack_gate_up(gate, up):
    F, D = gate.shape
    assert F % 16 == 0
    return torch.stack([gate.view(F // 16, 16, D), up.view(F // 16, 16, D)], dim=1).reshape(2 * F, D).contiguous()
```

### revisionllm_amd/eval/stage2.py

```python
import json
import math
import re

import numpy as np
import torch

from .. import ops, sched
from ..inference import _decode, _prompt_ids, inference
from ..model.adapter import pad_sequences_1d

QUERY_TEMPLATE = "During which video can we see {}?"


def cut_windows(ctx_l, debug_window=125, feature_fps=5, stride=5, num_frames=250):
    clip_length = debug_window * feature_fps
    num_window = math.ceil(ctx_l / (clip_length // stride)) - 1
    times, idx = [], []
    for i in range(num_window):
        start = max(i * clip_length // stride, 0)
        end = min(i * clip_length // stride + clip_length, ctx_l - 1)
        if end - start < clip_length:
            start = end - clip_length
        times.append((start, end))
        idx.append(np.linspace(start, end, num_frames, dtype=np.int32))
    return times, (np.stack(idx) if idx else np.zeros((0, num_frames), np.int32))


def plan_groups(W, batch, zooms=(4, 2, 1)):
    plan = []
    for z in zooms:
        b = batch // z
        for g in range(math.ceil(W / b)):
            start = g * b
            end = min(start + b, W)
            if end - start < b:
                start = end - b
            plan.append((z, start, end))
    return plan


def group_span(W, start, end):
    r = range(W)[start:end]
    return (r.start if len(r) else 0), len(r)


def get_ground_truth_windows(start, end, duration):
    clip_len = 0.2
    start, end = start / clip_len, end / clip_len
    size = int(900 / 2)
    ids = list(range(math.floor(start / size), math.ceil(end / size) + 1))
    return ids, math.ceil(duration / clip_len / size) + 1


def answer_to_window(output, zoom, index, start, grounding_windows):
    m = re.search(r"(\d+)", output)
    if not m:
        return None
    n = int(m.group(1)) // zoom
    if n < len(index):
        n = int(index[n])
    n = min(len(grounding_windows) - 1, max(0, start + n))
    return grounding_windows[n]


def iou(outputs, gt, num_frames_clip, num_frames_video, starts, indexes, single, hierarchy_zooms, grounding_windows):
    clip_frames, frames = {}, []
    for i, output in enumerate(outputs):
        w = answer_to_window(output, hierarchy_zooms[i], indexes[i], starts[i], grounding_windows)
        if w is None:
            continue
        f, t = max(0, w - 1), min(num_frames_video, w + 1)
        clip_frames[i] = (int(f), int(t))
        frames.append((f, t))
    s, e = min(gt), max(gt)
    inter = [max(0, min(t, e) - max(f, s)) for f, t in frames]
    return clip_frames, [1] if sum(inter) > 0 else [0]


def write_log(log_path, video_id, task, query_id, answer, info=None):
    log = {"video_id": video_id, "task": task, "query_id": query_id, "answer": answer}
    if info is not None:
        log["info"] = info
    with open(log_path, "a") as f:
        f.write(json.dumps(log) + "\n")


def _proposal_rows(answer0, n_group_rows, zooms_so_far, indexes, starts, i_inner, grounding_windows, single=True):
    m = None
    if not single:
        m = re.search(r"(\d+) (to|and) (\d+)", answer0)
    if not m:
        m = re.search(r"(\d+)", answer0)
    if not m:
        return None
    n = int(m.group(1)) // zooms_so_far[i_inner]
    if n < len(indexes[i_inner]):
        n = int(indexes[i_inner][n])
    n = min(len(grounding_windows) - 1, max(0, starts[i_inner] + n))
    w = grounding_windows[n]
    return list(range(max(0, w - 1), min(w + 1, n_group_rows - 1)))


def _steps_until_eos(new_tokens, eos):
    G = new_tokens.shape[1]
    if eos is None:
        return [G] * new_tokens.shape[0]
    out = []
    for row in new_tokens.tolist():
        out.append(row.index(eos) + 1 if eos in row else G)
    return out



def encode_windows(model, features, query_feats):
    mask = torch.ones(1, query_feats.shape[0])
    return model.engine.clip_encoder(features, query_feats[None], mask, "cls")


def window_cosine(features, query_cls, k=3):
    return ops.topk_cosine(features, query_cls, min(features.shape[1], k))


def call_row_index(plan, perms, device, W=None):
    firsts = [start if start >= 0 else group_span(W, start, end)[0] for _, start, end in plan]
    idx = [(f + p.long()).repeat_interleave(z) if z > 1 else f + p.long() for f, (z, _, _), p in zip(firsts, plan, perms)]
    return ops.h2d(torch.cat(idx), device), [int(i.numel()) for i in idx]


def build_call_rows(cls, plan, perms, index=None):
    idx, counts = index if index is not None else call_row_index(plan, perms, cls.device, cls.shape[0])
    return list(cls.index_select(0, idx).split(counts))


def launch_calls(model, tokenizer, query, rows, calls, uniforms=None, max_new_tokens=1024, max_calls_per_generate=16, width=None,
                 forced_tokens=None):
    return sched.drive(launch_calls_steps(model, tokenizer, query, rows, calls, uniforms, max_new_tokens, max_calls_per_generate, width,
                                          forced_tokens))


def launch_calls_steps(model, tokenizer, query, rows, calls, uniforms=None, max_new_tokens=1024, max_calls_per_generate=16, width=None,
                       forced_tokens=None, server=None):
    ids_of = {}

    def prompt_ids(c):
        q = query if isinstance(query, str) else query[c]
        if q not in ids_of:
            ids_of[q] = _prompt_ids(q, tokenizer, 1)[0]
        return ids_of[q]

    ragged = server is not None and getattr(server, "prefill_batch", 1) > 1 and getattr(server, "ragged", True)
    groups = {}
    for c in calls:
        groups.setdefault((None if ragged else rows[c].shape[0], prompt_ids(c).shape[1]), []).append(c)
    order, toks, ents = [], [], []
    for (_, _), cs in groups.items():
        for c0 in range(0, len(cs), max_calls_per_generate):
            sel = cs[c0:c0 + max_calls_per_generate]
            counts = [int(rows[c].shape[0]) for c in sel]
            n_rows = counts[0] if len(set(counts)) == 1 else counts
            ids = torch.cat([prompt_ids(c) for c in sel], 0)
            u = None if uniforms is None else uniforms[:, sel]
            forced = None if forced_tokens is None else forced_tokens[:, sel]
            out = yield from model.generate_steps(ids, video_rows=torch.cat([rows[c] for c in sel], 0), rows_per_sample=n_rows,
                                                  do_sample=True, temperature=0.05, num_beams=1, max_new_tokens=max_new_tokens,
                                                  output_scores=False, return_dict_in_generate=True, uniforms=u, forced_tokens=forced,
                                                  server=server, new_tokens_only=True)
            order.extend(sel)
            toks.append(out["new_tokens"] if out.get("new_tokens") is not None else out["sequences"][:, ids.shape[1]:])
            ents.append(out["entropy"])
    dev = model.engine.device
    if not order:
        w0 = width or 0
        return [], torch.zeros(0, w0, dtype=torch.int32, device=dev), torch.zeros(0, w0, device=dev), torch.zeros(0, dtype=torch.int32, device=dev)
    width = width or max(t.shape[1] for t in toks)
    if len(toks) == 1 and toks[0].shape[1] == width and toks[0].dtype == torch.int32:
        return order, toks[0], ents[0], torch.full((len(order),), width, dtype=torch.int32, device=dev)
    tok = torch.zeros(len(order), width, dtype=torch.int32, device=dev)
    ent = torch.zeros(len(order), width, dtype=torch.float32, device=dev)
    nst = torch.empty(len(order), dtype=torch.int32, device=dev)
    r = 0
    for t, e in zip(toks, ents):
        n, g = t.shape
        if g > width:
            raise ValueError(f"a call generated {g} tokens > wire capacity {width}")
        tok[r:r + n, :g] = t
        ent[r:r + n, :g] = e
        nst[r:r + n] = g
        r += n
    return order, tok, ent, nst


def finish_calls(order, tok, ent, nst, eos):
    res = {}
    for j, c in enumerate(order):
        n = int(nst[j])
        row = tok[j, :n]
        g = _steps_until_eos(row[None], eos)[0]
        e = ent[j, :g]
        res[c] = (row[:g].tolist(), float(e.max()), float(e.mean()))
    return res


def generate_calls(model, tokenizer, query, rows, calls, uniforms=None, max_new_tokens=1024, max_calls_per_generate=16, forced_tokens=None):
    order, tok, ent, nst = launch_calls(model, tokenizer, query, rows, calls, uniforms, max_new_tokens, max_calls_per_generate,
                                        forced_tokens=forced_tokens)
    tok, ent, nst = tok.cpu(), ent.cpu(), nst.cpu()
    model.engine.check_handoff_status()
    return finish_calls(order, tok, ent, nst, model.generation_config.eos_token_id)


def assemble(plan, perms, call_results, cos, tokenizer, zooms, grounding_windows, single=True):
    stop_str = "</s>"
    W = len(cos)
    answers, max_ent, mean_ent, score_cos, starts, indexes, hz = [], [], [], [], [], [], []
    i_call = 0
    for z in zooms:
        level = [p for p in plan if p[0] == z]
        for i, (_, start, end) in enumerate(level):
            idx = perms[i_call]
            toks, emax, emean = call_results[i_call]
            text = tokenizer.batch_decode([toks], skip_special_tokens=True)[0].strip()
            if text.endswith(stop_str):
                text = text[:-len(stop_str)]
            text = text.strip()
            starts.append(start)
            indexes.append(idx)
            hz.append(z)
            answers.append(text)
            max_ent.append(1 / emax)
            mean_ent.append(1 / emean)
            first, count = (start, end - start) if start >= 0 else group_span(W, start, end)
            prop = _proposal_rows(text, count * z, hz, indexes, starts, i, grounding_windows, single)
            if prop is None:
                score_cos.append(0)
            else:
                score_cos.extend(float(cos[first + int(idx[n // z])]) for n in prop)
            i_call += 1
    return dict(answers=answers, starts=starts, indexes=indexes, hierarchy_zooms=hz, max_entropy=max_ent,
                mean_entropy=mean_ent, score_cos=score_cos, grounding_windows=grounding_windows, plan=plan)


def make_perms(plan, generator=None, W=None):
    return [torch.randperm(end - start if start >= 0 else group_span(W, start, end)[1], generator=generator) for _, start, end in plan]


def run_query(model, tokenizer, features, query_feats, query_cls, sentence, batch=100, zooms=(4, 2, 1), perms=None,
              mode="batched", grounding_windows=None, uniforms=None, max_new_tokens=1024, max_calls_per_generate=16, single=True,
              forced_tokens=None):
    W = features.shape[0]
    if grounding_windows is None:
        grounding_windows = list(range(W))
    zooms = tuple(zooms)
    if W == 0:
        return dict(answers=[], starts=[], indexes=[], hierarchy_zooms=[], max_entropy=[], mean_entropy=[], score_cos=[],
                    grounding_windows=grounding_windows, plan=[])
    plan = plan_groups(W, batch, zooms)
    perms = [torch.as_tensor(p).long() for p in (perms if perms is not None else make_perms(plan, W=W))]
    query = "<video>\n" + QUERY_TEMPLATE.format(sentence)

    if mode == "batched":
        index = call_row_index(plan, perms, features.device, W)
        cls = encode_windows(model, features, query_feats)
        cos = window_cosine(features, query_cls)
        rows = build_call_rows(cls, plan, perms, index)
        res = generate_calls(model, tokenizer, query, rows, list(range(len(plan))), uniforms, max_new_tokens, max_calls_per_generate,
                             forced_tokens)
        return assemble(plan, perms, res, cos.cpu(), tokenizer, zooms, grounding_windows, single)
    if mode != "reference":
        raise ValueError(f"mode must be 'reference' or 'batched', got {mode!r}")

    qf = pad_sequences_1d(query_feats[None], dtype=query_feats.dtype, device=query_feats.device)
    answers, max_ent, mean_ent, score_cos, starts, indexes, hz = [], [], [], [], [], [], []
    i_call = 0
    for z in zooms:
        level = [p for p in plan if p[0] == z]
        for i, (_, start, end) in enumerate(level):
            idx = perms[i_call]
            feat = features[start:end][None][:, idx.to(features.device)]
            if z > 1:
                feat = feat.repeat_interleave(z, 1)
            starts.append(start)
            indexes.append(idx)
            ans, out = inference(model, feat, qf, query, tokenizer, return_list=True)
            answers.extend(ans)
            hz.append(z)
            st = ops.entropy_stats(torch.stack(out["scores"], 1))
            max_ent.extend(1 / float(e[0]) for e in st)
            mean_ent.extend(1 / float(e[2]) for e in st)
            prop = _proposal_rows(ans[0], feat.shape[1], hz, indexes, starts, i, grounding_windows, single)
            if prop is None:
                score_cos.append(0)
            elif prop:
                sc = ops.topk_cosine(feat[0, prop[0]:prop[-1] + 1], query_cls, min(feat.shape[2], 3))
                score_cos.extend(float(x) for x in sc.tolist())
            i_call += 1
    return dict(answers=answers, starts=starts, indexes=indexes, hierarchy_zooms=hz, max_entropy=max_ent,
                mean_entropy=mean_ent, score_cos=score_cos, grounding_windows=grounding_windows, plan=plan)


def log_record(res, timestamps, batch, num_frames=250, single=True):
    frames, ious = iou(res["answers"], timestamps, num_frames, batch, res["starts"], res["indexes"], single,
                       res["hierarchy_zooms"], res["grounding_windows"])
    return {"gt": timestamps, "frames": frames, "iou": ious, "score_cos": res["score_cos"], "mean_entropy": res["mean_entropy"],
            "max_entropy": res["max_entropy"], "hierarchy_zooms": res["hierarchy_zooms"]}
```

### revisionllm_amd/hip.py

```python
import ctypes as C
import os

import torch

_HERE = os.path.dirname(os.path.abspath(__file__))
LIB_PATHS = {"f16": os.environ.get("REVISION_HIP_LIB") or os.path.join(_HERE, "librevision_hip.so"),
             "bf16": os.environ.get("REVISION_HIP_LIB_BF16") or os.path.join(_HERE, "librevision_hip_bf16.so")}
LIB_PATH = LIB_PATHS["f16"]
OP_DTYPES = {"f16": torch.float16, "bf16": torch.bfloat16}

RV_F32, RV_BF16, RV_I32, RV_I64, RV_U8, RV_F16 = 0, 1, 2, 3, 4, 5
RV_ACT_NONE, RV_ACT_RELU, RV_ACT_SILU_MUL, RV_ACT_QUICK_GELU = 0, 1, 2, 3
RV_FEAT_CLS, RV_FEAT_ALL = 0, 2
TOPK_CAP = 64

_DT = {torch.float32: RV_F32, torch.bfloat16: RV_BF16, torch.float16: RV_F16, torch.int32: RV_I32, torch.int64: RV_I64, torch.uint8: RV_U8}


class RvConfig(C.Structure):
    _fields_ = [("hidden", C.c_int32), ("inter", C.c_int32), ("layers", C.c_int32), ("heads", C.c_int32),
                ("vocab", C.c_int32), ("rms_eps", C.c_float), ("rope_theta", C.c_float), ("adapter_dim", C.c_int32),
                ("adapter_heads", C.c_int32), ("adapter_ff", C.c_int32), ("adapter_layers", C.c_int32),
                ("adapter_text", C.c_int32)]


class RvPrefillGroup(C.Structure):
    _fields_ = [("B", C.c_int32), ("P0", C.c_int32), ("S", C.c_int32), ("kv_row0", C.c_int32)]


class RvYuvSurface(C.Structure):
    _fields_ = [("y", C.c_void_p), ("cb", C.c_void_p), ("cr", C.c_void_p), ("y_frame_stride", C.c_int64), ("y_row_stride", C.c_int64),
                ("c_frame_stride", C.c_int64), ("c_row_stride", C.c_int64), ("sample_bytes", C.c_int32), ("depth", C.c_int32), ("msb_aligned", C.c_int32),
                ("c_pix", C.c_int32), ("sub_x", C.c_int32), ("sub_y", C.c_int32), ("n", C.c_int32), ("H", C.c_int32), ("W", C.c_int32),
                ("matrix", C.c_int32), ("full_range", C.c_int32), ("chroma_loc", C.c_int32)]


class HipLibraryError(RuntimeError):
    pass


_libs = {}
_flavour = os.environ.get("REVISION_OP_DTYPE", "f16")
if _flavour not in OP_DTYPES:
    raise ValueError(f"REVISION_OP_DTYPE={_flavour!r}: expected one of {sorted(OP_DTYPES)}")


def flavour():
    return _flavour


def set_flavour(f):
    global _flavour
    f = flavour_of(f)
    prev, _flavour = _flavour, f
    return prev


def flavour_of(x):
    if x is None:
        return _flavour
    if isinstance(x, str):
        if x not in OP_DTYPES:
            raise ValueError(f"unknown operand flavour {x!r}")
        return x
    dt = x.dtype if torch.is_tensor(x) else x
    for k, v in OP_DTYPES.items():
        if v == dt:
            return k
    raise HipLibraryError(f"{dt} is not an operand type of librevision_hip (fp16 or bf16)")


def op_dtype(f=None):
    return OP_DTYPES[flavour_of(f)]

_p, _i32, _i64, _f, _sz, _u64 = C.c_void_p, C.c_int32, C.c_int64, C.c_float, C.c_size_t, C.c_uint64

SIGNATURES = {
    "rv_abi_version": (C.c_int, []),
    "rv_operand_dtype": (C.c_int, []),
    "rv_last_error": (C.c_int, [C.c_char_p, _sz]),
    "rv_ctx_create": (C.c_int, [C.POINTER(RvConfig), C.POINTER(_p)]),
    "rv_ctx_destroy": (None, [_p]),
    "rv_weights_bind": (C.c_int, [_p, C.c_char_p, _p, C.c_int, _i64]),
    "rv_init_hash": (C.c_int, [_p, C.c_int, _i64, _u64, _f, _f, _p]),
    "rv_ctx_set_option": (C.c_int, [_p, C.c_char_p, _i64]),
    "rv_ctx_get_option": (C.c_int, [_p, C.c_char_p, C.POINTER(_i64)]),
    "rv_numeric_status_bind": (C.c_int, [_p]),
    "rv_gemm_ws_bytes": (_sz, []),
    "rv_gemm_rows_ws_bytes": (_sz, []),
    "rv_gemm_rows": (C.c_int, [_p, _p, _p, _p, _i32, _i32, _i32, _p, _p, C.c_int, C.c_int, _p]),
    "rv_gemm": (C.c_int, [_p, _p, _i64, _p, _i64, C.c_int, _p, _p, _i64, _p, _i64, C.c_int, C.c_int, _i64, _i64, _i64, _p, _sz, _p]),
    "rv_rmsnorm_quant_fp8": (C.c_int, [_p, _p, _p, _p, _i64, _i32, _f, _p]),
    "rv_quant_rows_fp8": (C.c_int, [_p, _i64, _p, _i64, _p, _i64, _i64, _p]),
    "rv_gemm_fp8": (C.c_int, [_p, _p, _i64, _p, _p, _p, _p, _i64, _p, _i64, C.c_int, C.c_int, _i64, _i64, _i64, _p, C.c_size_t, _p]),
    "rv_gemv_fp8": (C.c_int, [_p, _i64, _p, _p, _p, _p, _i64, _p, _i64, C.c_int, C.c_int, _i64, _i64, _i64, _p]),
    "rv_layernorm": (C.c_int, [_p, _p, _p, _p, _p, _p, _p, _i64, _i64, _i32, _p]),
    "rv_rmsnorm": (C.c_int, [_p, _p, _p, _i64, _i32, _f, _p]),
    "rv_sine_pos": (C.c_int, [_p, _i32, _i32, _p]),
    "rv_attention": (C.c_int, [_p, _i64, _i64, _p, _i64, _i64, _i64, _p, _i64, _i64, _i64, _p, _i64, _i64, _p, _i32, _i32,
                               _i32, _i32, _i32, _i32, _i32, _i32, _f, _p]),
    "rv_frames_to_patches": (C.c_int, [_p, C.c_int, _i64, _i64, _i32, _i32, _i32, _i32, _i32, C.POINTER(_f), C.POINTER(_f), _p, _i64, _p, _p]),
    "rv_yuv_to_patches": (C.c_int, [_p, _i64, _i64, _p, _p, _i64, _i64, _i32, _i32, _i32, _i32, _i32, _i32, _i32, _i32, _i32, C.POINTER(_f), C.POINTER(_f), _p,
                                    _i64, _p, _p]),
    "rv_yuv_surface_to_patches": (C.c_int, [C.POINTER(RvYuvSurface), _i32, _i32, C.POINTER(_f), C.POINTER(_f), _p, _i64, _p, _p]),
    "rv_project_dense": (C.c_int, [_p, _p, _p, C.c_int, _i64, _p]),
    "rv_clip_encoder_ws_bytes": (_sz, [_p, _i32, _i32, _i32, _i32]),
    "rv_clip_encoder": (C.c_int, [_p, _p, _p, _p, _i32, _i32, _i32, _i32, _i32, _p, _p, _sz, _p]),
    "rv_splice_embed": (C.c_int, [_p, _p, _p, _p, _i64, _p]),
    "rv_kv_bytes": (_sz, [_p, _i32, _i32]),
    "rv_llm_ws_bytes": (_sz, [_p, _i32, _i32]),
    "rv_llm_forward": (C.c_int, [_p, _p, _i32, _i32, _i32, _p, _i32, _p, _p, _sz, _p]),
    "rv_llm_layers": (C.c_int, [_p, _p, _i32, _i32, _i32, _p, _i32, _i32, _i32, _p, _sz, _p]),
    "rv_llm_prefill_shared_ws_bytes": (_sz, [_p, _i32, _i32, _i32]),
    "rv_llm_prefill_shared": (C.c_int, [_p, _p, _i32, _i32, _i32, _p, _i32, _p, _p, _sz, _p]),
    "rv_llm_prefill_pool": (C.c_int, [_p, _p, _i32, _i32, _i32, _p, _i32, _i32, _i32, _p, _p, _sz, _p]),
    "rv_llm_prefill_pool_groups": (C.c_int, [_p, _p, _i32, _i32, _i32, _i32, _p, _i32, _p, _i32, _p, _p, _sz, _p]),
    "rv_llm_prefill_pool_groups_ragged": (C.c_int, [_p, _p, _i32, _i32, _i32, _i32, _p, _i32, _p, _i32, _p, _p, _p, _sz, _p]),
    "rv_llm_prefill_pool_mixed": (C.c_int, [_p, _p, _i32, _p, _p, _i32, _i32, _p, _p, _p, _sz, _p]),
    "rv_llm_decode_rows": (C.c_int, [_p, _p, _i32, _p, _p, _i32, _p, _p, _sz, _p]),
    "rv_llm_decode_rows_shared": (C.c_int, [_p, _p, _i32, _p, _p, _p, _i32, _p, _p, _sz, _p]),
    "rv_sample": (C.c_int, [_p, _p, _i32, _i32, _p, _i32, _f, _i32, _f, _p, _p, _p, _p, _p, _p, _p, _p]),
    "rv_entropy_stats": (C.c_int, [_p, _i32, _i32, _i32, _p, _p]),
    "rv_topk_cosine": (C.c_int, [_p, C.c_int, _p, _i32, _i32, _i32, _i32, _p, _p]),
    "rv_topk_pool": (C.c_int, [_p, C.c_int, _p, _i32, _i32, _i32, _i32, _i32, _p, _p, _p]),
}


def lib(f=None):
    f = flavour_of(f)
    h = _libs.get(f)
    if h is None:
        path = LIB_PATHS[f]
        if not os.path.exists(path):
            raise HipLibraryError(
                f"{path} not found: build it with `python -m revisionllm_amd.build` (hipcc, gfx950). "
                "revisionllm_amd has no CPU fallback.")
        try:
            h = C.CDLL(path)
        except OSError as e:
            raise HipLibraryError(f"cannot load {path}: {e}") from e
        for name, (res, args) in SIGNATURES.items():
            fn = getattr(h, name)
            fn.restype, fn.argtypes = res, args
        if h.rv_operand_dtype() != _DT[OP_DTYPES[f]]:
            raise HipLibraryError(f"{path} is not the {f} build of the library (rv_operand_dtype() = {h.rv_operand_dtype()})")
        _libs[f] = h
    return h


_numeric = {}


def numeric_status(f=None, device=None):
    f = flavour_of(f)
    dev = torch.device("cuda", torch.cuda.current_device()) if device is None else torch.device(device)
    if dev.index is None:
        dev = torch.device("cuda", torch.cuda.current_device())
    key = (f, dev.index)
    t = _numeric.get(key)
    if t is None:
        t = torch.zeros(4, dtype=torch.int32, device=dev)
        with torch.cuda.device(dev):
            torch.cuda.synchronize(dev)
            check(lib(f).rv_numeric_status_bind(C.c_void_p(t.data_ptr())), "rv_numeric_status_bind")
        _numeric[key] = t
    return t


def last_error():
    buf = C.create_string_buffer(512)
    msgs = []
    for h in _libs.values():
        h.rv_last_error(buf, 512)
        if buf.value:
            msgs.append(buf.value.decode())
    return " | ".join(msgs)


def check(rc, what):
    if rc != 0:
        msgs = last_error().split(" | ")
        name = what.split("(")[0]
        mine = [m for m in msgs if name in m]
        raise HipLibraryError(f"{what} failed (status {rc}): {' | '.join(mine or msgs)}")


OPTION_KEYS = ("gemm_tile_variant", "gemm_cus", "gemm_arows", "fp8_decode", "fp8_prefill", "sample_variant", "rows_fill", "rows_spread", "rows_persistent", "rows_single", "gemm_waves", "gemm_mhalf", "precision", "lm_head_split", "last_block_rows", "adapter_stream16", "adapter_fold_t2v", "attn_lds", "qkv_lds")


class Options:

    def __init__(self, flavour=None, **kw):
        self.flavour = flavour_of(flavour)
        self.lib = lib(self.flavour)
        self._ctx = C.c_void_p()
        check(self.lib.rv_ctx_create(None, C.byref(self._ctx)), "rv_ctx_create(options)")
        for k, v in kw.items():
            self.set(k, v)

    def set(self, key, value):
        check(self.lib.rv_ctx_set_option(self._ctx, key.encode(), int(value)), f"rv_ctx_set_option({key})")
        return self

    def get(self, key):
        v = _i64()
        check(self.lib.rv_ctx_get_option(self._ctx, key.encode(), C.byref(v)), f"rv_ctx_get_option({key})")
        return int(v.value)

    def __del__(self):
        try:
            if self._ctx and self._ctx.value:
                self.lib.rv_ctx_destroy(self._ctx)
                self._ctx = C.c_void_p()
        except Exception:
            pass


def ctx_ptr(ctx, f=None):
    if ctx is None:
        return None
    if f is not None and ctx.flavour != flavour_of(f):
        raise HipLibraryError(f"a {ctx.flavour} context was passed to a {flavour_of(f)} call")
    return ctx._ctx


def ptr(t):
    if t is None:
        return None
    if not t.is_cuda:
        raise HipLibraryError("librevision_hip needs device tensors (got a CPU tensor); there is no CPU path")
    return C.c_void_p(t.data_ptr())


def stream():
    return C.c_void_p(torch.cuda.current_stream().cuda_stream)


def dtype_code(t):
    return _DT[t.dtype]
```

### revisionllm_amd/model/revision_llama.py

```python
from types import SimpleNamespace

import numpy as np
import torch

from .. import hip, ops
from ..constants import IMAGE_TOKEN_INDEX, MEMORY_TOKEN_INDEX
from ..engine import Engine
from ..utils import synth


class GenerateOutput(dict):
    __getattr__ = dict.get


class GenerationConfig(SimpleNamespace):
    pass


class _Projector:

    def __init__(self, owner):
        self._o = owner

    def __call__(self, images, query_feats=None, query_mask=None, iteration_step=None):
# ... 82 lines not shown
        self.op_flavour = engine.flavour if engine is not None else hip.flavour_of(op_dtype)
        self.dtype = hip.op_dtype(self.op_flavour)
        self.uniform_fn = None
        self.after_prefill = None

    def _ensure_engine(self, adapter_text=None, adapter_dim=768):
        if self.engine is None:
            self.engine = Engine(self.shape, adapter_text=bool(adapter_text), device=self._device, adapter_dim=adapter_dim, op_dtype=self.op_flavour)
        elif adapter_text is not None and (bool(adapter_text) != self.engine.adapter_text or adapter_dim != self.engine.adapter_dim):
            raise RuntimeError("the engine's ClipEncoder topology (text-conditioned layers on / off, width) differs from this model's")
        return self.engine

    def get_model(self):
        return self.model

    @property
    def device(self):
        return self._device

    def eval(self):
        return self

    def cuda(self, device=None):
        return self

    _dtype_note_done = False

    def _dtype_request(self, what, asked):
        if asked is not None and asked != self.dtype and asked in (torch.float16, torch.bfloat16) and not ReVisionLlamaForCausalLM._dtype_note_done:
            ReVisionLlamaForCausalLM._dtype_note_done = True
            print(f"[revisionllm_amd] {what}: ignored - this model computes with {str(self.dtype).replace('torch.', '')} operands "
                  f"(librevision_hip{'_bf16' if self.op_flavour == 'bf16' else ''}.so, f32 accumulation and residual stream); pass op_dtype="
                  f"'{'bf16' if asked == torch.bfloat16 else 'f16'}' to load_pretrained_model's args (--op_dtype) to change the operand type", flush=True)
        return self

    def bfloat16(self):
        return self._dtype_request(".bfloat16()", torch.bfloat16)

    def half(self):
        return self._dtype_request(".half()", torch.float16)

    def float(self):
        return self

    def to(self, *args, **kwargs):
        asked = kwargs.get("dtype", next((a for a in args if isinstance(a, torch.dtype)), None))
        return self._dtype_request(f".to({asked})", asked)

    def encode_images(self, images, query_feats, iteration_step=None):
        m = self.model
        eng = self.engine
        if m.clip_adapter and m.clip_adapter_feature == "alternate":
            if iteration_step is None:
                raise TypeError("unsupported operand type(s) for %: 'NoneType' and 'int' (clip_adapter_feature='alternate' needs iteration_step)")
            if isinstance(images, (list, tuple)):
                raise TypeError("clip_adapter_feature='alternate': a list of feature tensors is not a valid input of the ClipEncoder adapter "
                                "(the reference's list branch calls mm_projector without query features, vtimellm_arch.py:102-108)")
            if query_feats is None:
                raise TypeError("'NoneType' object is not subscriptable (clip_adapter_feature='alternate' needs query_feats=(feats, mask))")
            qf, qm = query_feats[0], query_feats[1]
            if int(iteration_step) % 2 == 0:
                if m.hierarchy:
                    b, v, t, d = images.shape
                    y, rps = eng.clip_encoder(images.reshape(b * v, t, d), qf, qm, "cls"), v
                else:
                    y, rps = eng.clip_encoder(images, qf, qm, "cls"), 1
            else:
                if images.dim() != 3:
                    raise ValueError("clip_adapter_feature='alternate' at an odd iteration_step projects the temporal rows of [b,t,d] features "
                                     "(vtimellm_arch.py:112-113)")
                y = eng.clip_encoder(images, qf, qm, "all")[:, 1:].reshape(-1, self.shape.hidden)
                rps = images.shape[1]
            w, b_ = m.alternate_layer_norm
            return ops.layernorm(y.contiguous(), w, b_, want=("f32",))[0], rps
        if isinstance(images, (list, tuple)):
            images = torch.cat(list(images), dim=0)
        if not m.clip_adapter:
            y = eng.project_dense(images)
            return y.reshape(-1, self.shape.hidden), images.shape[1]
        qf, qm = (query_feats[0], query_feats[1]) if query_feats is not None else (None, None)
        if m.hierarchy:
            b, v, t, d = images.shape
            y = eng.clip_encoder(images.reshape(b * v, t, d), qf, qm, "cls")
            return y, v
        if m.clip_adapter_feature == "cls":
            return eng.clip_encoder(images, qf, qm, "cls"), 1
        y = eng.clip_encoder(images, qf, qm, "all")
        if m.clip_adapter_feature == "temporal":
            return y[:, 1:].reshape(-1, self.shape.hidden), images.shape[1]
        return y.reshape(-1, self.shape.hidden), images.shape[1] + 1

    @staticmethod
    def build_row_map_ragged(input_ids, rows_per_sample, pad_id=0):
        out, lens, off = [], [], 0
        for b, row in enumerate(input_ids.cpu().tolist()):
            if MEMORY_TOKEN_INDEX in row or row.count(IMAGE_TOKEN_INDEX) != 1:
                raise NotImplementedError("ragged generates take exactly one <video> per sample and no <memory>")
            n = int(rows_per_sample[b])
            i = row.index(IMAGE_TOKEN_INDEX)
            out.append(row[:i] + [-(off + k + 1) for k in range(n)] + row[i + 1:])
            off += n
            lens.append(len(out[-1]))
        S = max(lens)
        return torch.tensor([r + [pad_id] * (S - len(r)) for r in out], dtype=torch.int32), lens

    @staticmethod
    def build_row_map(input_ids, rows_per_sample, attention_mask=None, memory=None):
        ids = input_ids.cpu().tolist()
        mask = attention_mask.cpu().tolist() if attention_mask is not None else None
        out = []
        for b, row in enumerate(ids):
            if mask is not None:
                row = [t for t, m in zip(row, mask[b]) if m]
            if (MEMORY_TOKEN_INDEX in row) != (memory is not None):
                raise ValueError("a <memory> slot (-300) needs visual_memory / prefix_memory and the other way round (inference.py:29-30 appends the "
                                 "marker exactly when a memory is given)")
            r, used, used_mem = [], 0, 0
            for t in row:
                if t == IMAGE_TOKEN_INDEX:
                    if used:
                        raise NotImplementedError("more than one <video> per sample")
                    r.extend(-(b * rows_per_sample + i + 1) for i in range(rows_per_sample))
                    used = 1
                elif t == MEMORY_TOKEN_INDEX:
                    if used_mem or not used:
                        raise NotImplementedError("one <memory> per sample, behind its <video> (vtimellm_arch.py:207-232)")
                    prefix, M, base = memory
                    r.extend(int(x) for x in prefix[b])
                    r.extend(-(base + b * M + i + 1) for i in range(M))
                    used_mem = 1
                else:
                    r.append(t)
            out.append(r)
        if len({len(r) for r in out}) != 1:
            raise NotImplementedError("ragged batches: every row of a generate() call must have the same length "
                                      "(inference() repeats one prompt, inference.py:36)")
        return torch.tensor(out, dtype=torch.int32)

    @torch.no_grad()
    def generate(self, input_ids, images=None, query_feats=None, **kwargs):
        gen = self.generate_steps(input_ids, images=images, query_feats=query_feats, **kwargs)
        try:
            while True:
                ev = next(gen)
                if ev is not None:
                    ev.synchronize()
        except StopIteration as stop:
            return stop.value

    def generate_steps(self, input_ids, images=None, query_feats=None, do_sample=False, temperature=None, num_beams=1,
                       max_new_tokens=None, use_cache=True, visual_memory=None, prefix_memory=None, output_scores=False,
                       return_dict_in_generate=False, output_hidden_states=False, output_logits=False, top_k=None, top_p=None,
                       attention_mask=None, uniforms=None, forced_tokens=None, video_rows=None, rows_per_sample=None,
                       share_prefix=True, eos_lookahead=1, server=None, iteration_step=None, new_tokens_only=False, **kwargs):
        if num_beams != 1:
            raise NotImplementedError("beam search is not on the grounding path (num_beams=1, inference.py:51)")
        if (visual_memory is None) != (prefix_memory is None):
            raise ValueError("visual_memory and prefix_memory come together (vtimellm_arch.py:220-222 concatenates them)")
        eng = self._ensure_engine()
        gc = self.generation_config
        temperature = gc.temperature if temperature is None else temperature
        top_k = gc.top_k if top_k is None else top_k
        top_k = 0 if top_k is None else int(top_k)
        top_p = gc.top_p if top_p is None else top_p
        max_new_tokens = 20 if max_new_tokens is None else max_new_tokens
        eos, pad = gc.eos_token_id, gc.pad_token_id
        dev = eng.device

        if video_rows is None:
            if images is None:
                video_rows, rows_per_sample = None, 0
            else:
                video_rows, rows_per_sample = self.encode_images(images, query_feats, iteration_step)
        if uniforms is not None:
            uniforms = ops.h2d(uniforms, dev, torch.float32)
        if forced_tokens is not None:
            forced_tokens = ops.h2d(forced_tokens, dev, torch.long)
        memory = None
        if visual_memory is not None:
            if self.model.clip_adapter:
                raise NotImplementedError("visual_memory with a ClipEncoder adapter: the reference's mm_projector(vis_mem) call (vtimellm_arch.py:222) passes no "
                                          "query features and fails in ClipEncoder.forward (transformer.py:119); only the Linear projector runs this path")
            if video_rows is None or isinstance(rows_per_sample, (list, tuple)):
                raise NotImplementedError("visual_memory needs the video features of an ordinary (non-ragged) generate")
            vis = visual_memory[:, None] if visual_memory.dim() == 2 else visual_memory
            pm = torch.as_tensor(prefix_memory).long().cpu()
            if pm.dim() != 2 or pm.shape[0] != vis.shape[0] or vis.shape[0] != input_ids.shape[0]:
                raise ValueError("visual_memory [B,768] / [B,M,768] and prefix_memory int [B,Lp]: one memory per row of input_ids")
            mem_rows = eng.project_dense(vis).reshape(-1, self.shape.hidden)
            memory = (pm.tolist(), int(vis.shape[1]), int(video_rows.reshape(-1, self.shape.hidden).shape[0]))
            video_rows = video_rows.reshape(-1, self.shape.hidden)
            video_rows = torch.cat([video_rows, mem_rows.to(video_rows.dtype)], 0)
        lens = None
        if isinstance(rows_per_sample, (list, tuple)) and len(set(rows_per_sample)) > 1:
            if attention_mask is not None:
                raise NotImplementedError("ragged generates (different numbers of video rows per sample) do not take an attention_mask")
            row_map, lens = self.build_row_map_ragged(input_ids, rows_per_sample, pad if pad is not None else 0)
            ragged_ok = (server is not None and getattr(server, "prefill_batch", 1) > 1 and not output_scores and not output_logits
                         and self.after_prefill is None and max_new_tokens >= 1 and server.fits(row_map.shape[1], max_new_tokens, row_map.shape[0]))
            if not ragged_ok:
                return (yield from self._generate_split_by_rows(input_ids, video_rows, rows_per_sample, uniforms, forced_tokens, pad,
                                                                dict(do_sample=do_sample, temperature=temperature, max_new_tokens=max_new_tokens, output_scores=output_scores,
                                                                     return_dict_in_generate=return_dict_in_generate, output_logits=output_logits, top_k=top_k, top_p=top_p,
                                                                     share_prefix=share_prefix, eos_lookahead=eos_lookahead, server=server, new_tokens_only=new_tokens_only)))
        else:
            if isinstance(rows_per_sample, (list, tuple)):
                rows_per_sample = int(rows_per_sample[0]) if len(rows_per_sample) else 0
            row_map = self.build_row_map(input_ids, rows_per_sample, attention_mask, memory)
        B, S = row_map.shape
        P0 = self._common_text_prefix(row_map) if (share_prefix and B > 1) else 0
        job = None
        if (server is not None and not output_scores and not output_logits and self.after_prefill is None
                and server.fits(S, max_new_tokens, B) and max_new_tokens >= 1):
            job = server.reserve(B)
            while job is None and getattr(server, "blocking", False):
                from .. import sched
                yield sched.RETRY
                job = server.reserve(B)
        if job is not None:
            try:
                return (yield from self._generate_in_pool(server, job, eng, dev, input_ids, row_map, video_rows, B, S, P0, do_sample, temperature, top_k,
                                                          top_p, max_new_tokens, uniforms, forced_tokens, return_dict_in_generate, lens,
                                                          new_tokens_only))
            finally:
                if not job.finished:
                    server.abandon(job)
        if lens is not None:
            return (yield from self._generate_split_by_rows(input_ids, video_rows, rows_per_sample, uniforms, forced_tokens, pad,
                                                            dict(do_sample=do_sample, temperature=temperature, max_new_tokens=max_new_tokens, output_scores=output_scores,
                                                                 return_dict_in_generate=return_dict_in_generate, output_logits=output_logits, top_k=top_k, top_p=top_p,
                                                                 share_prefix=share_prefix, eos_lookahead=eos_lookahead, server=server, new_tokens_only=new_tokens_only)))
        slot = eng.slot
        if slot in eng.slots_in_flight:
            raise RuntimeError(f"engine slot {slot} already has a generate in flight: give every call in flight its own workspace slot "
                               "(sched.Task(..., slot=i) / engine.slot) - two generates on one slot share one recycled KV cache")
        eng.slots_in_flight.add(slot)
        try:
            return (yield from self._generate_alone(eng, dev, input_ids, row_map, video_rows, B, S, P0, do_sample, temperature, top_k, top_p,
                                                    max_new_tokens, uniforms, forced_tokens, return_dict_in_generate, output_scores, output_logits,
                                                    eos, pad, eos_lookahead))
        finally:
            eng.slots_in_flight.discard(slot)

    def _generate_split_by_rows(self, input_ids, video_rows, rows_per_sample, uniforms, forced_tokens, pad, kw):
        counts = [int(r) for r in rows_per_sample]
        starts = [0]
        for r in counts:
            starts.append(starts[-1] + r)
        if kw.get("output_scores") or kw.get("output_logits"):
            raise NotImplementedError("ragged generates return no per-step scores / logits: call generate per equal-geometry group for those")
        parts = []
        for r in sorted(set(counts)):
            sel = [i for i, c in enumerate(counts) if c == r]
            rows = torch.cat([video_rows[starts[i]:starts[i + 1]] for i in sel], 0) if video_rows is not None else None
            out = yield from self.generate_steps(input_ids[sel], video_rows=rows, rows_per_sample=r,
                                                 uniforms=None if uniforms is None else uniforms[:, sel],
                                                 forced_tokens=None if forced_tokens is None else forced_tokens[:, sel], **dict(kw, return_dict_in_generate=True))
            parts.append((sel, out))
        B = len(counts)
        merged = GenerateOutput()
        for key in ("sequences", "new_tokens", "entropy", "entropy_raw"):
            vals = [(sel, out.get(key)) for sel, out in parts]
            if any(v is None for _, v in vals):
                continue
            width = max(v.shape[1] for _, v in vals)
            fill = (pad if pad is not None else 0) if key in ("sequences", "new_tokens") else 0
            full = torch.full((B, width), fill, dtype=vals[0][1].dtype, device=vals[0][1].device)
            for sel, v in vals:
                full[torch.as_tensor(sel, device=full.device), :v.shape[1]] = v
            merged[key] = full
        if not kw.get("return_dict_in_generate"):
            return merged["sequences"]
        return merged

    def _generate_in_pool(self, server, job, eng, dev, input_ids, row_map, video_rows, B, S, P0, do_sample, temperature, top_k, top_p,
                          max_new_tokens, uniforms, forced_tokens, return_dict_in_generate, lens=None, new_tokens_only=False):
        pool = job.pool
        for ev in job.free_events:
            torch.cuda.current_stream(dev).wait_event(ev)
        batched = getattr(server, "prefill_batch", 1) > 1
        if not batched and getattr(server, "fifo_prefill", False) and server.prefill_tail is not None:
            torch.cuda.current_stream(dev).wait_event(server.prefill_tail)
        if 16 <= P0 < S:
            flat = torch.cat([row_map[0, :P0], row_map[:, P0:].reshape(-1)])[None]
            h, p0 = eng.splice_embed(flat, video_rows)[0], P0
        else:
            h, p0 = eng.splice_embed(row_map, video_rows).view(B * S, -1), 0
        if lens is not None and not batched:
            raise NotImplementedError("ragged generates need a DecodeServer with prefill_batch > 1 (its prefill passes carry the per-sequence last rows)")
        if do_sample and uniforms is None:
            uniforms = (torch.rand(max_new_tokens, B, device=dev) if self.uniform_fn is None
                        else torch.stack([self.uniform_fn(s_, B).to(dev).float() for s_ in range(max_new_tokens)]))
        if batched:
            ticket = server.submit_prefill(job, h, B, p0, lens)
            from .. import sched
            while ticket.ready is None:
                yield sched.RETRY
            first, ready = ticket.first, ticket.ready
            torch.cuda.current_stream(dev).wait_event(ready)
        else:
            first = eng.llm_prefill_pool(h, B, p0, pool.kv, pool.R, job.r0, pool.Smax)
            ready = None
        if ready is None:
            ready = torch.cuda.Event()
            ready.record()
            if getattr(server, "fifo_prefill", False):
                server.prefill_tail = ready
        yield ready
        start = S if lens is None else [int(n) for n in lens]
        server.join(job, start, first, ready, max_new_tokens, (bool(do_sample), float(temperature), int(top_k), float(top_p if top_p is not None else 1.0)),
                    uniforms=uniforms if do_sample else None, forced=forced_tokens, shared_prefix=p0)
        from .. import sched
        while not job.finished:
            yield sched.RETRY
        yield job.done_event
        if new_tokens_only and return_dict_in_generate:
            return GenerateOutput(sequences=None, new_tokens=job.tokens, entropy=job.entropy, entropy_raw=job.entropy_raw)
        seqs = torch.cat([ops.h2d(input_ids, dev, torch.long), job.tokens.long()], dim=1)
        if not return_dict_in_generate:
            return seqs
        return GenerateOutput(sequences=seqs, entropy=job.entropy, entropy_raw=job.entropy_raw)

    def _generate_alone(self, eng, dev, input_ids, row_map, video_rows, B, S, P0, do_sample, temperature, top_k, top_p, max_new_tokens,
                        uniforms, forced_tokens, return_dict_in_generate, output_scores, output_logits, eos, pad, eos_lookahead):
        cap = min(max_new_tokens, 64)
        kv, Smax = eng.new_kv(B, S + cap)
        if 16 <= P0 < S:
            flat = torch.cat([row_map[0, :P0], row_map[:, P0:].reshape(-1)])[None]
            h = eng.splice_embed(flat, video_rows)[0]
            logits = eng.llm_prefill_shared(h, B, P0, kv, Smax)
        else:
            h = eng.splice_embed(row_map, video_rows)
            logits = eng.llm_forward(h, 0, kv, Smax)
        if self.after_prefill is not None:
            self.after_prefill()

        seqs = ops.h2d(input_ids, dev, torch.long)
        unfinished = torch.ones(B, dtype=torch.int32, device=dev)
        raw_steps, score_steps, ent_p, ent_r, new_tokens = [], [], [], [], []
        pos = S
        if do_sample and uniforms is None and self.uniform_fn is None:
            uniforms = torch.rand(max_new_tokens, B, device=dev)
        flags = []
        if eos is not None:
            flag_host = torch.empty(max_new_tokens, dtype=torch.int32).pin_memory()
        n_steps = 0
        for step in range(max_new_tokens):
            if do_sample:
                if uniforms is not None:
                    u = uniforms[step].contiguous()
                else:
                    u = self.uniform_fn(step, B).to(dev).float().contiguous()
                o = ops.sample(logits, u, True, temperature, top_k, top_p, ctx=eng)
            else:
                o = ops.sample(logits, None, False, ctx=eng)
            nxt = o["tokens"] if forced_tokens is None else forced_tokens[step].int()
            ent_p.append(o["entropy_proc"])
            ent_r.append(o["entropy_raw"])
            if output_logits or (output_scores and (not do_sample or self.scores_mode == "raw")):
                raw_steps.append(logits.clone())
            if output_scores and do_sample and self.scores_mode == "processed" and (not top_k or top_k > hip.TOPK_CAP):
                sc = logits * float(np.float32(1.0) / np.float32(temperature))
                score_steps.append(sc.masked_fill(sc < o["threshold"][:, None], float("-inf")))
            elif output_scores and do_sample and self.scores_mode == "processed":
                V = logits.shape[1]
                sc = torch.full((B, V + 1), float("-inf"), device=dev)
                keep = torch.arange(hip.TOPK_CAP, device=dev)[None] < o["n_keep"][:, None]
                idx = torch.where(keep, o["topk_idx"], torch.full_like(o["topk_idx"], V)).long()
                score_steps.append(sc.scatter(1, idx, o["topk_val"])[:, :V].contiguous())
            if eos is not None:
                nxt = nxt * unfinished + pad * (1 - unfinished)
                unfinished = unfinished * (nxt != eos).int()
                flag_host[step:step + 1].copy_(unfinished.max().reshape(1), non_blocking=True)
                ev = torch.cuda.Event()
                ev.record()
                flags.append(ev)
            new_tokens.append(nxt)
            n_steps = step + 1
            if step == max_new_tokens - 1:
                break
            if eos is not None and step >= eos_lookahead:
                yield flags[step - eos_lookahead]
                if int(flag_host[step - eos_lookahead]) == 0:
                    n_steps = step - eos_lookahead + 1
                    break
            if pos + 1 > Smax:
                kv, Smax = self._grow_kv(kv, B, Smax, min(S + max_new_tokens, Smax * 2))
            h1 = eng.splice_embed(nxt[:, None], None)
            logits = eng.llm_forward(h1, pos, kv, Smax)
            pos += 1
        if eos is not None and n_steps == len(new_tokens) and n_steps > 0:
            for s_ in range(max(0, n_steps - eos_lookahead - 1), n_steps):
                yield flags[s_]
                if int(flag_host[s_]) == 0:
                    n_steps = s_ + 1
                    break

        def cut(lst):
            return lst[:n_steps]
        new_tokens, ent_p, ent_r, raw_steps, score_steps = cut(new_tokens), cut(ent_p), cut(ent_r), cut(raw_steps), cut(score_steps)
        seqs = torch.cat([seqs, torch.stack(new_tokens, dim=1).long()], dim=1)
        if not return_dict_in_generate:
            return seqs
        out = GenerateOutput(sequences=seqs, entropy=torch.stack(ent_p, 1), entropy_raw=torch.stack(ent_r, 1))
        if output_scores:
            out["scores"] = tuple(score_steps) if (do_sample and self.scores_mode == "processed") else tuple(raw_steps)
        if output_logits:
            out["logits"] = tuple(raw_steps)
        return out

    @staticmethod
    def _common_text_prefix(row_map):
        same = (row_map == row_map[:1]).all(dim=0) & (row_map[0] >= 0)
        bad = (~same).nonzero()
        return int(bad[0]) if bad.numel() else row_map.shape[1]

    def _grow_kv(self, kv, B, Smax, new_smax):
        s = self.shape
        new, new_smax = self.engine.new_kv(B, new_smax)
        half_old, half_new = kv.numel() // 2, new.numel() // 2
        k_old = kv[:half_old].view(s.layers, B, s.heads, Smax, s.head_dim)
        v_old = kv[half_old:].view(s.layers, B, s.heads, Smax // 8, s.head_dim, 8)
        new[:half_new].view(s.layers, B, s.heads, new_smax, s.head_dim)[:, :, :, :Smax] = k_old
        new[half_new:].view(s.layers, B, s.heads, new_smax // 8, s.head_dim, 8)[:, :, :, :Smax // 8] = v_old
        return new, new_smax


VTimeLLMLlamaForCausalLM = ReVisionLlamaForCausalLM
```

### revisionllm_amd/parallel.py

```python
import torch
import torch.distributed as dist

from . import sched
from .eval import stage2
from .ops import h2d as ops_h2d


LOCAL = object()


def force_collectives():
    import os
    return os.environ.get("REVISION_FORCE_COLLECTIVES", "0") == "1" and dist.is_initialized()


def shard_bounds(n, rank, world):
    base, rem = divmod(n, world)
    lo = rank * base + min(rank, rem)
    return lo, lo + base + (1 if rank < rem else 0)


def deal(n_items, rank, world, offset=0):
    first = (rank - offset) % world
    return list(range(first, n_items, world))


def _all_gather_cat(padded, group):
    world = dist.get_world_size(group)
    if dist.get_backend(group) == "nccl":
        out = torch.empty((world * padded.shape[0],) + tuple(padded.shape[1:]), dtype=padded.dtype, device=padded.device)
        dist.all_gather_into_tensor(out, padded.contiguous(), group=group)
        return out
    parts = [torch.empty_like(padded) for _ in range(world)]
    dist.all_gather(parts, padded.contiguous(), group=group)
    return torch.cat(parts, 0)


def allgather_rows(local, n_total, group=None):
    world = dist.get_world_size(group)
    if world == 1 and not force_collectives():
        return local
    per = -(-n_total // world)
    pad = torch.zeros((per,) + tuple(local.shape[1:]), dtype=local.dtype, device=local.device)
    pad[: local.shape[0]] = local
    out = _all_gather_cat(pad, group)
    parts = []
    for r in range(world):
        lo, hi = shard_bounds(n_total, r, world)
        parts.append(out[r * per: r * per + (hi - lo)])
    return torch.cat(parts, 0)


def allgather_calls(results, n_calls, max_tokens, device, group=None):
    world = dist.get_world_size(group)
    if world == 1:
        return dict(results)
    per = -(-n_calls // world)
    tok = torch.full((per, 2 + max_tokens), -1, dtype=torch.int32, device=device)
    ent = torch.zeros((per, 2), dtype=torch.float32, device=device)
    for j, (c, (t, emax, emean)) in enumerate(sorted(results.items())):
        if len(t) > max_tokens:
            raise ValueError(f"call {c} generated {len(t)} tokens > wire capacity {max_tokens}")
        tok[j, 0], tok[j, 1] = c, len(t)
        tok[j, 2:2 + len(t)] = torch.tensor(t, dtype=torch.int32)
        ent[j, 0], ent[j, 1] = emax, emean
    tok_all, ent_all = _all_gather_cat(tok, group).cpu(), _all_gather_cat(ent, group).cpu()
    out = {}
    for j in range(tok_all.shape[0]):
        c = int(tok_all[j, 0])
        if c >= 0:
            n = int(tok_all[j, 1])
            out[c] = (tok_all[j, 2:2 + n].tolist(), float(ent_all[j, 0]), float(ent_all[j, 1]))
    return out


class HipStages:

    def __init__(self, model, tokenizer):
        self.model, self.tokenizer = model, tokenizer

    def encode(self, features, query_feats):
        return stage2.encode_windows(self.model, features, query_feats)

    def cosine(self, features, query_cls):
        return stage2.window_cosine(features, query_cls)

    def generate(self, query, rows, calls, uniforms, max_new_tokens):
        return stage2.generate_calls(self.model, self.tokenizer, query, rows, calls, uniforms, max_new_tokens)

    def generate_async(self, query, rows, calls, uniforms, max_new_tokens, width):
        return stage2.launch_calls(self.model, self.tokenizer, query, rows, calls, uniforms, max_new_tokens, width=width)

    def generate_steps(self, query, rows, calls, uniforms, max_new_tokens, width):
        return stage2.launch_calls_steps(self.model, self.tokenizer, query, rows, calls, uniforms, max_new_tokens, width=width,
                                         server=getattr(self, "server", None), forced_tokens=getattr(self, "forced_tokens", None))

    def gate(self):
        return self.model.engine.gate

    @property
    def eos(self):
        return self.model.generation_config.eos_token_id

    def check(self, snapshot=None):
        self.model.engine.check_handoff_status(snapshot)

    def status_async(self):
        return self.model.engine.handoff_status_async()


class PendingQuery:
    """A launched, not yet collected pass of one or more recursions (``launch_queries_sharded``)."""


def launch_queries_sharded(stages, tokenizer, features_local, W, queries, batch=100, zooms=(4, 2, 1), perms=None, uniforms=None,
                           max_new_tokens=64, grounding_windows=None, group=None, single=True):
    return sched.drive(launch_queries_sharded_steps(stages, tokenizer, features_local, W, queries, batch, zooms, perms, uniforms,
                                                    max_new_tokens, grounding_windows, group, single))


def _gated(stages, world, fn):
    gate = stages.gate() if ((world > 1 or force_collectives()) and hasattr(stages, "gate")) else None
    if gate is not None:
        gate.begin()
    out = fn()
    if gate is not None:
        gate.end()
    return out


def launch_queries_sharded_steps(stages, tokenizer, features_local, W, queries, batch=100, zooms=(4, 2, 1), perms=None, uniforms=None,
                                 max_new_tokens=64, grounding_windows=None, group=None, single=True, turn=None):
    alone = group is LOCAL or not dist.is_initialized()
    world = 1 if alone else dist.get_world_size(group)
    rank = 0 if alone else dist.get_rank(group)
    exchange = world > 1 or (not alone and force_collectives())
    lo, hi = shard_bounds(W, rank, world)
    feats_of = features_local if isinstance(features_local, (list, tuple)) else [features_local] * len(queries)
    assert len(feats_of) == len(queries) and all(f.shape[0] == hi - lo for f in feats_of), f"rank {rank} must hold windows [{lo},{hi})"
    zooms = tuple(zooms)
    plan = stage2.plan_groups(W, batch, zooms)
    nc, nq = len(plan), len(queries)
    if perms is None:
        raise ValueError("perms must be given (identical on all ranks); use stage2.make_perms with a seeded generator")
    perms = [[torch.as_tensor(p).long() for p in pq] for pq in perms]
    if grounding_windows is None:
        grounding_windows = list(range(W))
    dev = feats_of[0].device
    index = [stage2.call_row_index(plan, perms[qi], dev, W) for qi in range(nq)]
    rows, prompts, cos_all = [], {}, []
    srv = getattr(stages, "server", None)
    batched_enc = srv is not None and getattr(srv, "encode_batch", 1) > 1
    tickets = [srv.submit_encode(feats_of[qi], qf) for qi, (qf, _, _) in enumerate(queries)] if batched_enc else None
    for qi, (qf, qc, sentence) in enumerate(queries):
        if batched_enc:
            while tickets[qi].ready is None:
                yield sched.RETRY
            torch.cuda.current_stream(dev).wait_event(tickets[qi].ready)
            cls_local = tickets[qi].cls
            cls_local.record_stream(torch.cuda.current_stream(dev))
        else:
            cls_local = stages.encode(feats_of[qi], qf)
        cos_local = stages.cosine(feats_of[qi], qc)
        if exchange:
            cls_local, cos_local = _gated(stages, world, lambda: (allgather_rows(cls_local, W, group),
                                                                  allgather_rows(cos_local[:, None], W, group)[:, 0]))
        cos_all.append(cos_local)
        rows.extend(stage2.build_call_rows(cls_local, plan, None, index[qi]))
        for c in range(nc):
            prompts[qi * nc + c] = "<video>\n" + stage2.QUERY_TEMPLATE.format(sentence)
    p = PendingQuery()
    p.seq = getattr(stages, "_seq_next", 0)
    stages._seq_next = p.seq + 1
    mine = deal(nc * nq, rank, world, offset=p.seq)
    p.args = (plan, perms, tokenizer, zooms, grounding_windows, single, nq)
    p.stages = stages
    cos = torch.stack(cos_all, 0)
    if hasattr(stages, "generate_async"):
        width = min(max_new_tokens, 128)
        if hasattr(stages, "generate_steps"):
            order, tok, ent, nst = yield from stages.generate_steps(prompts, rows, mine, uniforms, max_new_tokens, width)
        else:
            order, tok, ent, nst = stages.generate_async(prompts, rows, mine, uniforms, max_new_tokens, width)
        if not exchange and dev.type == "cuda":
            p.order = list(order)
            src = (tok, ent, nst, cos)
            p.host = tuple(torch.empty(t.shape, dtype=t.dtype, pin_memory=True) for t in src)
            for h, t in zip(p.host, src):
                h.copy_(t, non_blocking=True)
            p.status = stages.status_async() if hasattr(stages, "status_async") else None
            p.event = torch.cuda.Event()
            p.event.record()
            return p
        per = -(-(nc * nq) // world)
        tw = torch.full((per, 2 + width), -1, dtype=torch.int32, device=dev)
        ew = torch.zeros((per, width), dtype=torch.float32, device=dev)
        n = len(order)
        if n:
            tw[:n, 0] = ops_h2d(torch.tensor(order, dtype=torch.int32), dev)
            tw[:n, 1], tw[:n, 2:], ew[:n] = nst.to(dev), tok.to(dev), ent.to(dev)
        if exchange:
            while turn is not None and not turn.finishing:
                yield sched.RETRY
            tw, ew = _gated(stages, world, lambda: (_all_gather_cat(tw, group), _all_gather_cat(ew, group)))
        if dev.type == "cuda":
            p.host = tuple(torch.empty(t.shape, dtype=t.dtype, pin_memory=True) for t in (tw, ew, cos))
            for h, t in zip(p.host, (tw, ew, cos)):
                h.copy_(t, non_blocking=True)
            p.status = stages.status_async() if hasattr(stages, "status_async") else None
            p.event = torch.cuda.Event()
            p.event.record()
        else:
            p.host, p.event = (tw, ew, cos), None
    else:
        res = stages.generate(prompts, rows, mine, uniforms, max_new_tokens)
        if world > 1:
            res = allgather_calls(res, nc * nq, max_new_tokens, dev, group)
        p.res, p.cos = res, cos.cpu()
    return p


def collect_queries(p):
    plan, perms, tokenizer, zooms, grounding_windows, single, nq = p.args
    nc = len(plan)
    if hasattr(p, "event"):
        if p.event is not None:
            p.event.synchronize()
        if getattr(p, "order", None) is not None:
            tok, ent, nst, cos = p.host
            res = stage2.finish_calls(p.order, tok, ent, nst, p.stages.eos)
        else:
            tw, ew, cos = p.host
            rows_ = [j for j in range(tw.shape[0]) if int(tw[j, 0]) >= 0]
            res = stage2.finish_calls([int(tw[j, 0]) for j in rows_], tw[rows_][:, 2:], ew[rows_], tw[rows_][:, 1], p.stages.eos)
        if getattr(p, "status", None) is not None:
            p.stages.check(p.status)
        else:
            p.stages.check()
    else:
        res, cos = p.res, p.cos
    return [stage2.assemble(plan, perms[qi], {c: res[qi * nc + c] for c in range(nc)}, cos[qi], tokenizer, zooms, grounding_windows, single)
            for qi in range(nq)]


def run_queries_sharded(stages, tokenizer, features_local, W, queries, batch=100, zooms=(4, 2, 1), perms=None, uniforms=None,
                        max_new_tokens=64, grounding_windows=None, group=None, single=True):
    return collect_queries(launch_queries_sharded(stages, tokenizer, features_local, W, queries, batch, zooms, perms, uniforms,
                                                  max_new_tokens, grounding_windows, group, single))


def launch_query_sharded(stages, tokenizer, features_local, W, query_feats, query_cls, sentence, batch=100, zooms=(4, 2, 1),
                         perms=None, uniforms=None, max_new_tokens=64, grounding_windows=None, group=None, single=True):
    if perms is None:
        raise ValueError("perms must be given (identical on all ranks); use stage2.make_perms with a seeded generator")
    return launch_queries_sharded(stages, tokenizer, features_local, W, [(query_feats, query_cls, sentence)], batch, zooms, [perms],
                                  uniforms, max_new_tokens, grounding_windows, group, single)


def collect_query(p):
    return collect_queries(p)[0]


def run_query_sharded(stages, tokenizer, features_local, W, query_feats, query_cls, sentence, batch=100, zooms=(4, 2, 1),
                      perms=None, uniforms=None, max_new_tokens=64, grounding_windows=None, group=None, single=True):
    return collect_query(launch_query_sharded(stages, tokenizer, features_local, W, query_feats, query_cls, sentence, batch, zooms,
                                              perms, uniforms, max_new_tokens, grounding_windows, group, single))
```

### revisionllm_amd/serve.py

```python
import collections

import torch

from . import hip, ops


class Job:

    def __init__(self, r0, B):
        self.r0, self.B = r0, B
        self.step, self.steps = 0, 0
        self.uniforms = self.forced = None
        self.joined = self.finished = False
        self.done_event = None
        self.tokens = self.entropy = self.entropy_raw = None
        self.flag_host, self.flag_events = None, collections.deque()


class DecodePool:

    def __init__(self, model, rows=32, smax=256, gmax=64, max_ahead=2, slot=97, gang=False):
        eng = model.engine
        assert 1 <= rows <= 144
        self.model, self.eng, self.R, self.G, self.max_ahead, self.slot = model, eng, rows, gmax, max_ahead, slot
# ... 98 lines not shown
        progressed = self._drain() if self.draining else False
        if not self.jobs or len(self.in_flight) >= self.max_ahead:
            return progressed
        if self.gang and (not self.sealed or self.pending > 0):
            return progressed
        self._step()
        return True

    def _drain(self):
        left, done = [], False
        for job in self.draining:
            if all(fe.query() for _, fe in job.flag_events):
                n = job.steps
                for s_, _ in job.flag_events:
                    if int(job.flag_host[s_]) == 0:
                        n = s_ + 1
                        break
                prev = self.eng.slot
                with torch.cuda.stream(self.stream):
                    self._finish(job, n)
                self.eng.slot = prev
                done = True
            else:
                left.append(job)
        self.draining = left
        return done

    def wait_one(self):
        if self.in_flight:
            self.in_flight.popleft().synchronize()
            return True
        if self.draining:
            self.draining[0].flag_events[-1][1].synchronize()
            return True
        return False

    def _finish(self, job, n):
        r = slice(job.r0, job.r0 + job.B)
        job.tokens = self.tok_out[r, :n].clone()
        job.entropy = self.ent_out[r, :n].clone()
        job.entropy_raw = self.entr_out[r, :n].clone()
        self.pos[r] = -1
        job.done_event = torch.cuda.Event()
        job.done_event.record(self.stream)
        job.finished = True
        self.live -= 1
        self._release(job, job.done_event)

    def _step(self):
        eng = self.eng
        do_sample, temperature, top_k, top_p = self.sampling
        gc = self.model.generation_config
        eos, pad = gc.eos_token_id, gc.pad_token_id
        prev_slot = eng.slot
        eng.slot = self.slot
        with torch.cuda.stream(self.stream):
            if eos is not None:
                still = []
                for job in self.jobs:
                    ended = None
                    while job.flag_events and job.flag_events[0][1].query():
                        s_, _ = job.flag_events.popleft()
                        if int(job.flag_host[s_]) == 0:
                            ended = s_ + 1
                            break
                    if ended is not None:
                        self._finish(job, ended)
                    else:
                        still.append(job)
                self.jobs = still
                if not self.jobs:
                    eng.slot = prev_slot
                    return
            if do_sample:
                self.uni = self.uni_all.gather(0, self.stepidx.clamp(max=self.G)[None])[0]
            o = ops.sample(self.logits, self.uni if do_sample else None, do_sample, temperature, top_k, top_p, ctx=eng)
            tokens = o["tokens"]
            for job in self.jobs:
                if job.forced is not None:
                    tokens[job.r0:job.r0 + job.B] = job.forced[job.step].int()
            active = self.pos >= 0
            if eos is not None:
                tokens = tokens * self.unfinished + pad * (1 - self.unfinished)
                self.unfinished = self.unfinished * (tokens != eos).int()
            tokens = torch.where(active, tokens, torch.zeros_like(tokens))
            col = torch.where(active, self.stepidx.clamp(max=self.G - 1), torch.full_like(self.stepidx, self.G))[:, None]
            self.tok_out.scatter_(1, col, tokens[:, None])
            self.ent_out.scatter_(1, col, o["entropy_proc"][:, None])
            self.entr_out.scatter_(1, col, o["entropy_raw"][:, None])
            self.stepidx += active.long()
            self.rows_served += sum(j.B for j in self.jobs)
            self.steps_run += 1
            still = []
            for job in self.jobs:
                if eos is not None:
                    if job.flag_host is None:
                        job.flag_host = torch.empty(job.steps, dtype=torch.int32).pin_memory()
                    job.flag_host[job.step:job.step + 1].copy_(self.unfinished[job.r0:job.r0 + job.B].max().reshape(1), non_blocking=True)
                    fe = torch.cuda.Event()
                    fe.record(self.stream)
                    job.flag_events.append((job.step, fe))
                job.step += 1
                if job.step >= job.steps:
                    if eos is not None:
                        self.pos[job.r0:job.r0 + job.B] = -1
                        self.draining.append(job)
                    else:
                        self._finish(job, job.steps)
                else:
                    still.append(job)
            self.jobs = still
            if self.jobs:
                h = eng.splice_embed(tokens[:, None], None).view(self.R, -1)
                eng.llm_decode_rows(h, self.pos, self.kv, self.Smax, logits=self.logits, row_share=self.share if self.share_prefix else None)
                self.pos += (self.pos >= 0).int()
            ev = torch.cuda.Event()
            ev.record(self.stream)
            self.in_flight.append(ev)
        eng.slot = prev_slot


def team_fill(tiles_m, per_x=32):
    if tiles_m > per_x:
        return 0.5
    ts = (per_x // tiles_m) * tiles_m
    if tiles_m >= 10 and tiles_m % 2 == 0:
        ts = max(ts, (tiles_m // 2) * (per_x // (tiles_m // 2)))
    return ts / per_x


def best_prefill_batch(avail, rows, per_x=32):
    best, best_cost = 1, None
    for n in range(1, max(1, avail) + 1):
        tiles = -(-n * rows // 256)
        cost = tiles / (team_fill(tiles, per_x) * n)
        if best_cost is None or cost <= best_cost * 1.0001:
            best, best_cost = n, cost
    return best


def best_prefill_count(rows, per_x=32):
    best, best_cost, total = 1, None, 0
    for n, r in enumerate(rows, 1):
        total += int(r)
        tiles = -(-total // 256)
        cost = tiles / (team_fill(tiles, per_x) * n)
        if best_cost is None or cost <= best_cost * 1.0001:
            best, best_cost = n, cost
    return best


class PrefillTicket:

    def __init__(self, job, h, B, P0, event, lens=None):
        self.job, self.h, self.B, self.P0, self.event = job, h, B, P0, event
        self.lens = tuple(int(n) for n in lens) if lens is not None else None
        self.ready = self.first = None

    @property
    def key(self):
        return (id(self.job.pool), self.B, self.P0, self.h.shape[0], self.lens)

    @property
    def S(self):
        return (self.h.shape[0] - self.P0) // self.B

    @property
    def mixable(self):
        return self.S > 16 and (self.P0 == 0 or self.P0 > 16) and 32 <= self.P0 + self.S <= self.job.pool.Smax


class EncodeTicket:

    def __init__(self, features, query_feats, event):
        self.features, self.query_feats, self.event = features, query_feats, event
        self.ready = self.cls = None

    @property
    def key(self):
        return (tuple(self.features.shape), tuple(self.query_feats.shape), self.features.dtype)

    @property
    def key_any_length(self):
        return (tuple(self.features.shape), tuple(self.query_feats.shape[1:]), self.features.dtype, self.query_feats.dtype)


class DecodeServer:

    def __init__(self, model, rows=32, smax=256, gmax=64, max_ahead=2, slot=97, pools=1, gang=False, prefill_batch=1, pool_factory=None, encode_batch=1,
                 mixed_prefill=False):
        self.mixed_prefill = bool(mixed_prefill)
        assert pools >= 1 and (pools >= 2 or not gang), "the gang policy alternates between at least two pools"
        assert 1 <= prefill_batch <= 8
        self.prefill_batch, self.pf_queue, self.pf_inflight = prefill_batch, [], []
        self.pf_stream = torch.cuda.Stream(model.engine.device) if prefill_batch > 1 else None
        self.pf_slot = slot + 16
        self.pf_batches = self.pf_tickets = 0
        self.pf_hist = {}
        assert 1 <= encode_batch <= 16
        self.encode_batch, self.enc_queue, self.enc_inflight = encode_batch, [], []
        self.enc_stream = torch.cuda.Stream(model.engine.device) if encode_batch > 1 else None
        self.enc_slot = slot + 17
        self.enc_batches = self.enc_tickets = 0
        dev_ = getattr(getattr(model, "engine", None), "device", None)
        self.cus_per_xcd = (max(8, torch.cuda.get_device_properties(dev_).multi_processor_count // 8)
                            if getattr(dev_, "type", "cpu") == "cuda" and torch.cuda.is_available() else 32)
        make = pool_factory or DecodePool
        self.pools = [make(model, rows, smax, gmax, max_ahead, slot + i, gang) for i in range(pools)]
        self.gang, self.blocking, self.fill = gang, gang, 0
        self.fifo_prefill, self.prefill_tail = gang, None
        self.model = model

    @property
    def kv(self):
        return self.pools[0].kv

    @property
    def R(self):
        return self.pools[0].R

    @property
    def Smax(self):
        return self.pools[0].Smax

    @property
    def steps_run(self):
        return sum(p.steps_run for p in self.pools)

    @property
    def rows_served(self):
        return sum(p.rows_served for p in self.pools)

    @property
    def jobs(self):
        return [j for p in self.pools for j in p.jobs]

    @property
    def draining(self):
        return [j for p in self.pools for j in p.draining]

    @property
    def free(self):
        return [f for p in self.pools for f in p.free]

    def fits(self, S, max_new_tokens, B=1):
        return self.pools[0].fits(S, max_new_tokens, B)

    def reserve(self, B):
        if not self.gang:
            return self.pools[0].reserve(B)
        for _ in range(2):
            p = self.pools[self.fill]
            if p.sealed:
                nxt = (self.fill + 1) % len(self.pools)
                if self.pools[nxt].live > 0:
                    return None
                self.fill, p = nxt, self.pools[nxt]
                p.sealed = False
            job = p.reserve(B)
            if job is None:
                assert p.live > 0, (B, p.free)
                p.sealed = True
                continue
            if p.free_rows() < B:
                p.sealed = True
            return job
        return None

    def join(self, job, *a, **kw):
        return job.pool.join(job, *a, **kw)

    def abandon(self, job):
        self.pf_queue = [t for t in self.pf_queue if t.job is not job]
        job.pool.abandon(job, extra_streams=(self.pf_stream,) if self.pf_stream is not None else ())

    def submit_prefill(self, job, h, B, P0, lens=None):
        ev = torch.cuda.Event()
        ev.record()
        t = PrefillTicket(job, h, B, P0, ev, lens)
        self.pf_queue.append(t)
        return t

    def _pump_prefill(self, partial=False, force=False):
        if not self.pf_queue:
            return False
        self.pf_inflight = [e for e in self.pf_inflight if not e.query()]
        lead = self.pf_queue[0]
        n = 1
        mix = self._mix_ok() and lead.mixable
        if mix:
            while n < len(self.pf_queue) and n < self.prefill_batch and self.pf_queue[n].job.pool is lead.job.pool and self.pf_queue[n].mixable:
                n += 1
        else:
            while n < len(self.pf_queue) and n < self.prefill_batch and self.pf_queue[n].key == lead.key:
                n += 1
        full = n == self.prefill_batch or n < len(self.pf_queue)
        if not full and not force and not (partial and not self.pf_inflight):
            return False
        if mix:
            n = best_prefill_count([int(t.h.shape[0]) for t in self.pf_queue[:n]], self.cus_per_xcd)
        else:
            n = best_prefill_batch(n, int(lead.h.shape[0]), self.cus_per_xcd)
        batch, self.pf_queue = self.pf_queue[:n], self.pf_queue[n:]
        mix = mix and any(t.key != lead.key for t in batch)
        eng, pool = self.model.engine, lead.job.pool
        prev = eng.slot
        eng.slot = self.pf_slot
        with torch.cuda.stream(self.pf_stream):
            for t in batch:
                self.pf_stream.wait_event(t.event)
                t.h.record_stream(self.pf_stream)
            if mix:
                groups, last, base = [], [], 0
                for t in batch:
                    groups.append((t.B, t.P0, t.S, t.job.r0))
                    last += [base + t.P0 + b * t.S + ((t.lens[b] - t.P0) if t.lens is not None else t.S) - 1 for b in range(t.B)]
                    base += int(t.h.shape[0])
                ragged = any(t.lens is not None for t in batch)
                logits = eng.llm_prefill_pool_mixed(torch.cat([t.h for t in batch]), groups, pool.kv, pool.R, pool.Smax,
                                                    last_rows=ops.h2d(torch.tensor(last, dtype=torch.int32), eng.device) if ragged else None)
            elif lead.lens is not None:
                Mg = lead.h.shape[0]
                S_ = (Mg - lead.P0) // lead.B
                last = [g * Mg + lead.P0 + b * S_ + (lead.lens[b] - lead.P0 - 1) for g in range(n) for b in range(lead.B)]
                logits = eng.llm_prefill_pool_groups(torch.cat([t.h for t in batch]) if n > 1 else lead.h, n, lead.B, lead.P0, pool.kv, pool.R,
                                                     [t.job.r0 for t in batch], pool.Smax, last_rows=ops.h2d(torch.tensor(last, dtype=torch.int32), eng.device))
            elif n == 1:
                logits = eng.llm_prefill_pool(lead.h, lead.B, lead.P0, pool.kv, pool.R, lead.job.r0, pool.Smax)
            else:
                logits = eng.llm_prefill_pool_groups(torch.cat([t.h for t in batch]), n, lead.B, lead.P0, pool.kv, pool.R,
                                                     [t.job.r0 for t in batch], pool.Smax)
            ev = torch.cuda.Event()
            ev.record(self.pf_stream)
        eng.slot = prev
        row = 0
        for t in batch:
            t.first = logits[row:row + t.B]
            row += t.B
            t.ready = ev
            t.h = None
        self.pf_inflight.append(ev)
        self.pf_batches += 1
        self.pf_tickets += n
        self.pf_hist[n] = self.pf_hist.get(n, 0) + n
        return True

    def _mix_ok(self):
        if not self.mixed_prefill:
            return False
        ok = getattr(self.model.engine, "mixed_prefill_supported", None)
        return True if ok is None else bool(ok())

    def submit_encode(self, features, query_feats):
        ev = torch.cuda.Event()
        ev.record()
        t = EncodeTicket(features, query_feats, ev)
        self.enc_queue.append(t)
        return t

    def _pump_encode(self, partial=False, force=False):
        if not self.enc_queue:
            return False
        self.enc_inflight = [e for e in self.enc_inflight if not e.query()]
        lead = self.enc_queue[0]
        n = 1
        key = (lambda t: t.key_any_length) if self.mixed_prefill else (lambda t: t.key)
        while n < len(self.enc_queue) and n < self.encode_batch and key(self.enc_queue[n]) == key(lead):
            n += 1
        full = n == self.encode_batch or n < len(self.enc_queue)
        if not full and not force and not (partial and not self.enc_inflight):
            return False
        batch, self.enc_queue = self.enc_queue[:n], self.enc_queue[n:]
        eng = self.model.engine
        prev = eng.slot
        eng.slot = self.enc_slot
        with torch.cuda.stream(self.enc_stream):
            for t in batch:
                self.enc_stream.wait_event(t.event)
                t.features.record_stream(self.enc_stream)
                t.query_feats.record_stream(self.enc_stream)
            N = lead.features.shape[0]
            x = torch.cat([t.features for t in batch]) if n > 1 else lead.features
            Lq = max(t.query_feats.shape[0] for t in batch)
            if all(t.query_feats.shape[0] == Lq for t in batch):
                txt = torch.stack([t.query_feats for t in batch])
                mask = torch.ones(n, txt.shape[1])
            else:
                txt = torch.stack([torch.nn.functional.pad(t.query_feats, (0, 0, 0, Lq - t.query_feats.shape[0])) for t in batch])
                mask = torch.tensor([[1.0] * t.query_feats.shape[0] + [0.0] * (Lq - t.query_feats.shape[0]) for t in batch])
            cls = eng.clip_encoder(x, txt, mask, "cls")
            ev = torch.cuda.Event()
            ev.record(self.enc_stream)
        eng.slot = prev
        for i, t in enumerate(batch):
            t.cls = cls[i * N:(i + 1) * N]
            t.ready = ev
            t.features = t.query_feats = None
        self.enc_inflight.append(ev)
        self.enc_batches += 1
        self.enc_tickets += n
        return True

    def pump(self):
        progressed = False
        if self.enc_queue:
            progressed |= self._pump_encode()
        if self.pf_queue:
            progressed |= self._pump_prefill()
        for p in self.pools:
            progressed |= p.pump()
        return progressed

    def idle(self):
        moved = bool(self.enc_queue) and self._pump_encode(partial=True)
        return (bool(self.pf_queue) and self._pump_prefill(partial=True)) or moved

    def wait_one(self):
        for p in self.pools:
            if p.wait_one():
                return True
        return False

    def flush(self):
        if self.enc_queue and self._pump_encode(force=True):
            return True
        if self.pf_queue and self._pump_prefill(force=True):
            return True
        if self.gang:
            p = self.pools[self.fill]
            if not p.sealed and p.live > 0 and p.pending == 0:
                p.sealed = True
                return True
        return False
```

Before: 6591.

## Assemble prefill rows directly into a ring buffer via index plan, avoiding gathers and cats

Stage-2 call rows become lazy index plans into the CLS table instead of materialized index_select copies. A new assemble_rows kernel writes the embedding lookups and the table gathers straight into a per-pass slot of a ring buffer owned by the decode server, so batched prefill passes can use a contiguous slice instead of torch.cat. A fused to_op16 conversion kernel also replaces the multi-step clamp/convert path in _dev16. This adds slot event tracking and wraparound copy logic, which carries a risk of cross-stream hazards.

```diff
diff --git a/include/revision_hip.h b/include/revision_hip.h
--- a/include/revision_hip.h
+++ b/include/revision_hip.h
@@ -60,6 +60,7 @@
                  const float* pos, int64_t period, int64_t rows, int32_t d, void* stream);
 int rv_rmsnorm(const float* x, const float* w, void* y_bf16, int64_t rows, int32_t d, float eps, void* stream);
 int rv_sine_pos(float* pos, int32_t T, int32_t d, void* stream);
+int rv_to_op16(const void* x, int src_dtype, int64_t ldx, void* y, int64_t ldy, int64_t rows, int64_t cols, void* stream);
 int rv_attention(const void* q, int64_t q_row_stride, int64_t q_batch_stride, const void* k, int64_t k_row_stride,
                  int64_t k_batch_stride, int64_t k_head_stride, const void* vt, int64_t vt_batch_stride,
                  int64_t vt_head_stride, int64_t vt_d_stride, void* out, int64_t o_row_stride, int64_t o_batch_stride,
@@ -95,6 +96,8 @@
                     int32_t Nq, int32_t Lq, int32_t feature, float* out, void* ws, size_t ws_bytes, void* stream);
 
 int rv_splice_embed(rv_ctx* ctx, const int32_t* map, const float* video_rows, float* h, int64_t rows, void* stream);
+int rv_assemble_rows(rv_ctx* ctx, const int32_t* map, const float* table, int64_t table_rows, const int64_t* idx, int64_t n_idx, float* dst,
+                     int64_t dst_row0, int64_t rows, void* stream);
 size_t rv_kv_bytes(const rv_ctx* ctx, int32_t B, int32_t Smax);
 size_t rv_llm_ws_bytes(const rv_ctx* ctx, int32_t B, int32_t S);
 int rv_llm_forward(rv_ctx* ctx, float* h, int32_t B, int32_t S, int32_t pos0, void* kv, int32_t Smax, float* logits,
diff --git a/revisionllm_amd/csrc/engine.hip b/revisionllm_amd/csrc/engine.hip
--- a/revisionllm_amd/csrc/engine.hip
+++ b/revisionllm_amd/csrc/engine.hip
@@ -556,6 +556,16 @@
     return k_splice_embed(map, c->embed, video_rows, h, rows, c->cfg.hidden, as_stream(stream));
 }
 
+extern "C" int rv_assemble_rows(rv_ctx* c, const int32_t* map, const float* table, int64_t table_rows, const int64_t* idx, int64_t n_idx, float* dst,
+                                int64_t dst_row0, int64_t rows, void* stream) {
+    RV_CHECK_ARG(c && map && dst && rows > 0 && dst_row0 >= 0 && table_rows >= 0 && n_idx >= 0, "rv_assemble_rows: bad arguments");
+    RV_CHECK_ARG(table || table_rows == 0, "rv_assemble_rows: table_rows without a table");
+    RV_CHECK_ARG(idx || n_idx == 0, "rv_assemble_rows: n_idx without an index plan");
+    RV_TRY(resolve_llm(c));
+    return k_assemble_rows(map, c->embed, c->cfg.vocab, table, idx, n_idx, table_rows, dst + dst_row0 * (int64_t)c->cfg.hidden, rows, c->cfg.hidden,
+                           as_stream(stream));
+}
+
 extern "C" size_t rv_kv_bytes(const rv_ctx* c, int32_t B, int32_t Smax) {
     if (!c || B <= 0 || Smax <= 0) return 0;
     return (size_t)2 * c->cfg.layers * B * c->cfg.hidden * (size_t)Smax * 2;
diff --git a/revisionllm_amd/csrc/kernels.h b/revisionllm_amd/csrc/kernels.h
--- a/revisionllm_amd/csrc/kernels.h
+++ b/revisionllm_amd/csrc/kernels.h
@@ -226,6 +226,9 @@
 int k_rope_table(float* cs, int S, int pos0, int dh, float theta, hipStream_t st);
 int k_rope_table_rows(float* cs, const int* row_pos, int rows, int dh, float theta, hipStream_t st);
 int k_splice_embed(const int32_t* map, const void* embed, const float* video, float* h, int64_t rows, int D, hipStream_t st);
+int k_assemble_rows(const int32_t* map, const void* embed, int vocab, const float* table, const int64_t* idx, int64_t n_idx, int64_t table_rows,
+                    float* dst, int64_t rows, int D, hipStream_t st);
+int k_to_op16(const void* x, int src_dtype, int64_t ldx, void* y, int64_t ldy, int64_t rows, int64_t cols, hipStream_t st);
 
 struct AttnArgs {
     const void* q; int64_t q_rs, q_bs;
diff --git a/revisionllm_amd/csrc/rowops.hip b/revisionllm_amd/csrc/rowops.hip
--- a/revisionllm_amd/csrc/rowops.hip
+++ b/revisionllm_amd/csrc/rowops.hip
@@ -476,6 +476,80 @@
     }
 }
 
+__global__ __launch_bounds__(256) void assemble_rows_kernel(const int32_t* __restrict__ map, const op16_t* __restrict__ embed, int vocab,
+                                                            const float* __restrict__ table, const int64_t* __restrict__ idx, int64_t n_idx,
+                                                            int64_t table_rows, float* __restrict__ dst, int64_t rows, int D) {
+    const int64_t r = (int64_t)blockIdx.x * 4 + (threadIdx.x >> 6);
+    if (r >= rows) return;
+    const int lane = threadIdx.x & 63;
+    const int src = map[r];
+    float* o = dst + r * D;
+    if (src >= 0 && src < vocab) {
+        const op16_t* e = embed + (int64_t)src * D;
+        for (int c = lane * 8; c < D; c += 512) {
+            const u32x4 raw = *(const u32x4*)(e + c);
+            *(f32x4*)(o + c) = op16x4_to_f32(u32x2{raw[0], raw[1]});
+            *(f32x4*)(o + c + 4) = op16x4_to_f32(u32x2{raw[2], raw[3]});
+        }
+        return;
+    }
+    const int64_t v = -((int64_t)src + 1);
+    int64_t t = -1;
+    if (src < 0) t = idx ? (v < n_idx ? idx[v] : -1) : v;
+    if (t >= 0 && t < table_rows) {
+        const float* s = table + t * D;
+        for (int c = lane * 4; c < D; c += 256) *(f32x4*)(o + c) = *(const f32x4*)(s + c);
+    } else {
+        const float nan = __uint_as_float(0x7fc00000u);
+        for (int c = lane * 4; c < D; c += 256) *(f32x4*)(o + c) = f32x4{nan, nan, nan, nan};
+    }
+}
+
+template <int SRC>
+__device__ __forceinline__ float to_op16_load(const void* p, int64_t i) {
+    if (SRC == 0) return ((const float*)p)[i];
+    const uint16_t b = ((const uint16_t*)p)[i];
+    if (SRC == 1) return __uint_as_float(((uint32_t)b) << 16);
+    return (float)__builtin_bit_cast(_Float16, b);
+}
+template <int SRC>
+__global__ __launch_bounds__(256) void to_op16_kernel(const void* __restrict__ x, int64_t ldx, op16_t* __restrict__ y, int64_t ldy, int64_t rows,
+                                                      int64_t cols) {
+    const int64_t pairs = (cols + 1) / 2;
+    for (int64_t i = (int64_t)blockIdx.x * 256 + threadIdx.x; i < rows * pairs; i += (int64_t)gridDim.x * 256) {
+        const int64_t r = i / pairs, c = (i % pairs) * 2;
+        y[r * ldy + c] = f32_to_op16(to_op16_load<SRC>(x, r * ldx + c));
+        if (c + 1 < cols) y[r * ldy + c + 1] = f32_to_op16(to_op16_load<SRC>(x, r * ldx + c + 1));
+    }
+}
+
+}
+
+int k_assemble_rows(const int32_t* map, const void* embed, int vocab, const float* table, const int64_t* idx, int64_t n_idx, int64_t table_rows,
+                    float* dst, int64_t rows, int D, hipStream_t st) {
+    RV_CHECK_ARG(D > 0 && D % 8 == 0, "assemble_rows: the hidden size must be a multiple of 8");
+    hipLaunchKernelGGL(assemble_rows_kernel, dim3((unsigned)cdiv(rows, 4)), dim3(256), 0, st, map, (const op16_t*)embed, vocab, table, idx, n_idx,
+                       table_rows, dst, rows, D);
+    RV_CHECK_LAUNCH("assemble_rows");
+    return RV_OK;
+}
+
+int k_to_op16(const void* x, int src_dtype, int64_t ldx, void* y, int64_t ldy, int64_t rows, int64_t cols, hipStream_t st) {
+    if (rows == 0 || cols == 0) return RV_OK;
+    const int64_t work = rows * ((cols + 1) / 2);
+    const unsigned blocks = (unsigned)(cdiv(work, 256) < 65536 ? cdiv(work, 256) : 65536);
+    if (src_dtype == RV_F32)
+        hipLaunchKernelGGL(to_op16_kernel<0>, dim3(blocks), dim3(256), 0, st, x, ldx, (op16_t*)y, ldy, rows, cols);
+    else if (src_dtype == RV_BF16)
+        hipLaunchKernelGGL(to_op16_kernel<1>, dim3(blocks), dim3(256), 0, st, x, ldx, (op16_t*)y, ldy, rows, cols);
+    else if (src_dtype == RV_F16)
+        hipLaunchKernelGGL(to_op16_kernel<2>, dim3(blocks), dim3(256), 0, st, x, ldx, (op16_t*)y, ldy, rows, cols);
+    else {
+        rv_set_error("to_op16: source dtype %d (RV_F32, RV_BF16 or RV_F16)", src_dtype);
+        return RV_ERR_ARG;
+    }
+    RV_CHECK_LAUNCH("to_op16");
+    return RV_OK;
 }
 
 int k_layernorm(const float* x, const float* w, const float* b, float* y32, void* y16, void* yp16, const float* pos,
@@ -687,3 +761,7 @@
     return k_rmsnorm_quant(x, d, w, q8, scale, rows, d, eps, as_stream(stream));
 }
 extern "C" int rv_sine_pos(float* pos, int32_t T, int32_t d, void* stream) { return k_sine_pos(pos, T, d, as_stream(stream)); }
+extern "C" int rv_to_op16(const void* x, int src_dtype, int64_t ldx, void* y, int64_t ldy, int64_t rows, int64_t cols, void* stream) {
+    RV_CHECK_ARG(x && y && rows >= 0 && cols >= 0 && ldx >= cols && ldy >= cols, "rv_to_op16: bad arguments");
+    return k_to_op16(x, src_dtype, ldx, y, ldy, rows, cols, as_stream(stream));
+}
diff --git a/revisionllm_amd/engine.py b/revisionllm_amd/engine.py
--- a/revisionllm_amd/engine.py
+++ b/revisionllm_amd/engine.py
@@ -11,9 +11,29 @@
 
 
 def _dev16(t, device, dtype):
-    if dtype == torch.float16 and t.dtype != torch.float16:
+    if t.dtype == dtype:
+        return t.to(device=device).contiguous()
+    if t.is_cuda and t.device == torch.device(device) and t.dtype in _TO_OP16_SRC and t.dim() >= 1 and t.numel() > 0:
+        return to_op16(t, dtype)
+    if dtype == torch.float16:
         t = t.to(device=device, dtype=torch.float32).clamp(-65504.0, 65504.0)
     return t.to(device=device, dtype=dtype).contiguous()
+
+
+_TO_OP16_SRC = (torch.float32, torch.bfloat16, torch.float16)
+
+
+def to_op16(t, dtype):
+    cols = t.shape[-1]
+    rows = t.numel() // cols
+    if t.dim() == 2 and t.stride(1) == 1 and t.stride(0) >= cols:
+        x, ldx = t, (t.stride(0) if rows > 1 else cols)
+    else:
+        x, ldx = t.contiguous(), cols
+    y = torch.empty(t.shape, dtype=dtype, device=t.device)
+    with torch.cuda.device(t.device):
+        hip.check(hip.lib(dtype).rv_to_op16(hip.ptr(x), hip.dtype_code(x), ldx, hip.ptr(y), cols, rows, cols, hip.stream()), "rv_to_op16")
+    return y
 
 
 class PersistGate:
@@ -307,6 +327,18 @@
         hip.check(self.lib.rv_splice_embed(self._ctx, hip.ptr(rm), hip.ptr(vr), hip.ptr(h), B * S, hip.stream()), "rv_splice_embed")
         return h
 
+    def assemble_rows(self, row_map, table, index, out, row0=0):
+        n = int(row_map.numel())
+        D = self.shape.hidden
+        assert out.dtype == torch.float32 and out.is_cuda and out.is_contiguous() and out.shape[-1] == D and 0 <= row0 and row0 + n <= out.numel() // D
+        rm = ops.h2d(row_map, self.device, torch.int32).contiguous()
+        tb = _dev_f32(table, self.device).view(-1, D) if table is not None else None
+        if index is not None:
+            assert index.dtype == torch.int64 and index.is_cuda and index.is_contiguous()
+        hip.check(self.lib.rv_assemble_rows(self._ctx, hip.ptr(rm), hip.ptr(tb), tb.shape[0] if tb is not None else 0, hip.ptr(index),
+                                            index.numel() if index is not None else 0, hip.ptr(out), row0, n, hip.stream()), "rv_assemble_rows")
+        return out.view(-1, D)[row0:row0 + n]
+
     def new_kv(self, B, Smax, reuse=True):
         Smax = (Smax + 31) // 32 * 32
         key = ("kv", self.slot, B, Smax)
diff --git a/revisionllm_amd/eval/stage2.py b/revisionllm_amd/eval/stage2.py
--- a/revisionllm_amd/eval/stage2.py
+++ b/revisionllm_amd/eval/stage2.py
@@ -132,6 +132,37 @@
     return list(cls.index_select(0, idx).split(counts))
 
 
+class PlannedRows:
+
+    def __init__(self, table, index, start, n):
+        self.table, self.index, self.start, self.n = table, index, int(start), int(n)
+
+    @property
+    def shape(self):
+        return (self.n, self.table.shape[1])
+
+    def gather(self):
+        return self.table.index_select(0, self.index[self.start:self.start + self.n])
+
+
+def plan_call_rows(cls, index):
+    idx, counts = index
+    out, start = [], 0
+    for n in counts:
+        out.append(PlannedRows(cls, idx, start, n))
+        start += n
+    return out
+
+
+def _video_rows_of(rows, sel):
+    first = rows[sel[0]]
+    if all(isinstance(rows[c], PlannedRows) and rows[c].table is first.table and rows[c].index is first.index for c in sel):
+        if all(rows[b].start == rows[a].start + rows[a].n for a, b in zip(sel, sel[1:])):
+            return first.table, first.index[first.start:rows[sel[-1]].start + rows[sel[-1]].n]
+    parts = [rows[c].gather() if isinstance(rows[c], PlannedRows) else rows[c] for c in sel]
+    return (torch.cat(parts, 0) if len(parts) > 1 else parts[0]), None
+
+
 def launch_calls(model, tokenizer, query, rows, calls, uniforms=None, max_new_tokens=1024, max_calls_per_generate=16, width=None,
                  forced_tokens=None):
     return sched.drive(launch_calls_steps(model, tokenizer, query, rows, calls, uniforms, max_new_tokens, max_calls_per_generate, width,
@@ -161,7 +192,8 @@
             ids = torch.cat([prompt_ids(c) for c in sel], 0)
             u = None if uniforms is None else uniforms[:, sel]
             forced = None if forced_tokens is None else forced_tokens[:, sel]
-            out = yield from model.generate_steps(ids, video_rows=torch.cat([rows[c] for c in sel], 0), rows_per_sample=n_rows,
+            video_rows, video_index = _video_rows_of(rows, sel)
+            out = yield from model.generate_steps(ids, video_rows=video_rows, video_index=video_index, rows_per_sample=n_rows,
                                                   do_sample=True, temperature=0.05, num_beams=1, max_new_tokens=max_new_tokens,
                                                   output_scores=False, return_dict_in_generate=True, uniforms=u, forced_tokens=forced,
                                                   server=server, new_tokens_only=True)
diff --git a/revisionllm_amd/hip.py b/revisionllm_amd/hip.py
--- a/revisionllm_amd/hip.py
+++ b/revisionllm_amd/hip.py
@@ -107,6 +107,8 @@
     "rv_clip_encoder_ws_bytes": (_sz, [_p, _i32, _i32, _i32, _i32]),
     "rv_clip_encoder": (C.c_int, [_p, _p, _p, _p, _i32, _i32, _i32, _i32, _i32, _p, _p, _sz, _p]),
     "rv_splice_embed": (C.c_int, [_p, _p, _p, _p, _i64, _p]),
+    "rv_assemble_rows": (C.c_int, [_p, _p, _p, _i64, _p, _i64, _p, _i64, _i64, _p]),
+    "rv_to_op16": (C.c_int, [_p, C.c_int, _i64, _p, _i64, _i64, _i64, _p]),
     "rv_kv_bytes": (_sz, [_p, _i32, _i32]),
     "rv_llm_ws_bytes": (_sz, [_p, _i32, _i32]),
     "rv_llm_forward": (C.c_int, [_p, _p, _i32, _i32, _i32, _p, _i32, _p, _p, _sz, _p]),
diff --git a/revisionllm_amd/model/revision_llama.py b/revisionllm_amd/model/revision_llama.py
--- a/revisionllm_amd/model/revision_llama.py
+++ b/revisionllm_amd/model/revision_llama.py
@@ -258,7 +258,7 @@
                        max_new_tokens=None, use_cache=True, visual_memory=None, prefix_memory=None, output_scores=False,
                        return_dict_in_generate=False, output_hidden_states=False, output_logits=False, top_k=None, top_p=None,
                        attention_mask=None, uniforms=None, forced_tokens=None, video_rows=None, rows_per_sample=None,
-                       share_prefix=True, eos_lookahead=1, server=None, iteration_step=None, new_tokens_only=False, **kwargs):
+                       share_prefix=True, eos_lookahead=1, server=None, iteration_step=None, new_tokens_only=False, video_index=None, **kwargs):
         if num_beams != 1:
             raise NotImplementedError("beam search is not on the grounding path (num_beams=1, inference.py:51)")
         if (visual_memory is None) != (prefix_memory is None):
@@ -282,6 +282,8 @@
             uniforms = ops.h2d(uniforms, dev, torch.float32)
         if forced_tokens is not None:
             forced_tokens = ops.h2d(forced_tokens, dev, torch.long)
+        if video_index is not None and not (visual_memory is None and getattr(server, "prefill_batch", 1) > 1 and hasattr(server, "prefill_rows")):
+            video_rows, video_index = video_rows.index_select(0, video_index), None
         memory = None
         if visual_memory is not None:
             if self.model.clip_adapter:
@@ -305,6 +307,8 @@
             ragged_ok = (server is not None and getattr(server, "prefill_batch", 1) > 1 and not output_scores and not output_logits
                          and self.after_prefill is None and max_new_tokens >= 1 and server.fits(row_map.shape[1], max_new_tokens, row_map.shape[0]))
             if not ragged_ok:
+                if video_index is not None:
+                    video_rows, video_index = video_rows.index_select(0, video_index), None
                 return (yield from self._generate_split_by_rows(input_ids, video_rows, rows_per_sample, uniforms, forced_tokens, pad,
                                                                 dict(do_sample=do_sample, temperature=temperature, max_new_tokens=max_new_tokens, output_scores=output_scores,
                                                                      return_dict_in_generate=return_dict_in_generate, output_logits=output_logits, top_k=top_k, top_p=top_p,
@@ -327,10 +331,12 @@
             try:
                 return (yield from self._generate_in_pool(server, job, eng, dev, input_ids, row_map, video_rows, B, S, P0, do_sample, temperature, top_k,
                                                           top_p, max_new_tokens, uniforms, forced_tokens, return_dict_in_generate, lens,
-                                                          new_tokens_only))
+                                                          new_tokens_only, video_index))
             finally:
                 if not job.finished:
                     server.abandon(job)
+        if video_index is not None:
+            video_rows, video_index = video_rows.index_select(0, video_index), None
         if lens is not None:
             return (yield from self._generate_split_by_rows(input_ids, video_rows, rows_per_sample, uniforms, forced_tokens, pad,
                                                             dict(do_sample=do_sample, temperature=temperature, max_new_tokens=max_new_tokens, output_scores=output_scores,
@@ -380,25 +386,28 @@
         return merged
 
     def _generate_in_pool(self, server, job, eng, dev, input_ids, row_map, video_rows, B, S, P0, do_sample, temperature, top_k, top_p,
-                          max_new_tokens, uniforms, forced_tokens, return_dict_in_generate, lens=None, new_tokens_only=False):
+                          max_new_tokens, uniforms, forced_tokens, return_dict_in_generate, lens=None, new_tokens_only=False, video_index=None):
         pool = job.pool
         for ev in job.free_events:
             torch.cuda.current_stream(dev).wait_event(ev)
         batched = getattr(server, "prefill_batch", 1) > 1
         if not batched and getattr(server, "fifo_prefill", False) and server.prefill_tail is not None:
             torch.cuda.current_stream(dev).wait_event(server.prefill_tail)
-        if 16 <= P0 < S:
-            flat = torch.cat([row_map[0, :P0], row_map[:, P0:].reshape(-1)])[None]
-            h, p0 = eng.splice_embed(flat, video_rows)[0], P0
+        flat, p0 = (torch.cat([row_map[0, :P0], row_map[:, P0:].reshape(-1)])[None], P0) if 16 <= P0 < S else (row_map, 0)
+        slot = server.prefill_rows(int(flat.numel())) if batched and hasattr(server, "prefill_rows") else None
+        if slot is not None:
+            h = eng.assemble_rows(flat, video_rows, video_index, slot.buf, slot.row0)
         else:
-            h, p0 = eng.splice_embed(row_map, video_rows).view(B * S, -1), 0
+            if video_index is not None:
+                video_rows, video_index = video_rows.index_select(0, video_index), None
+            h = eng.splice_embed(flat, video_rows).view(int(flat.numel()), -1)
         if lens is not None and not batched:
             raise NotImplementedError("ragged generates need a DecodeServer with prefill_batch > 1 (its prefill passes carry the per-sequence last rows)")
         if do_sample and uniforms is None:
             uniforms = (torch.rand(max_new_tokens, B, device=dev) if self.uniform_fn is None
                         else torch.stack([self.uniform_fn(s_, B).to(dev).float() for s_ in range(max_new_tokens)]))
         if batched:
-            ticket = server.submit_prefill(job, h, B, p0, lens)
+            ticket = server.submit_prefill(job, h, B, p0, lens, slot=slot) if slot is not None else server.submit_prefill(job, h, B, p0, lens)
             from .. import sched
             while ticket.ready is None:
                 yield sched.RETRY
diff --git a/revisionllm_amd/parallel.py b/revisionllm_amd/parallel.py
--- a/revisionllm_amd/parallel.py
+++ b/revisionllm_amd/parallel.py
@@ -75,6 +75,8 @@
 
 
 class HipStages:
+
+    planned_rows = True
 
     def __init__(self, model, tokenizer):
         self.model, self.tokenizer = model, tokenizer
@@ -166,7 +168,8 @@
             cls_local, cos_local = _gated(stages, world, lambda: (allgather_rows(cls_local, W, group),
                                                                   allgather_rows(cos_local[:, None], W, group)[:, 0]))
         cos_all.append(cos_local)
-        rows.extend(stage2.build_call_rows(cls_local, plan, None, index[qi]))
+        rows.extend(stage2.plan_call_rows(cls_local, index[qi]) if getattr(stages, "planned_rows", False) and hasattr(stages, "generate_steps")
+                    else stage2.build_call_rows(cls_local, plan, None, index[qi]))
         for c in range(nc):
             prompts[qi * nc + c] = "<video>\n" + stage2.QUERY_TEMPLATE.format(sentence)
     p = PendingQuery()
diff --git a/revisionllm_amd/serve.py b/revisionllm_amd/serve.py
--- a/revisionllm_amd/serve.py
+++ b/revisionllm_amd/serve.py
@@ -274,8 +274,9 @@
 
 class PrefillTicket:
 
-    def __init__(self, job, h, B, P0, event, lens=None):
+    def __init__(self, job, h, B, P0, event, lens=None, slot=None):
         self.job, self.h, self.B, self.P0, self.event = job, h, B, P0, event
+        self.slot = slot
         self.lens = tuple(int(n) for n in lens) if lens is not None else None
         self.ready = self.first = None
 
@@ -290,6 +291,12 @@
     @property
     def mixable(self):
         return self.S > 16 and (self.P0 == 0 or self.P0 > 16) and 32 <= self.P0 + self.S <= self.job.pool.Smax
+
+
+class PassSlot:
+
+    def __init__(self, buf, index, row0):
+        self.buf, self.index, self.row0 = buf, index, row0
 
 
 class EncodeTicket:
@@ -319,6 +326,8 @@
         self.pf_slot = slot + 16
         self.pf_batches = self.pf_tickets = 0
         self.pf_hist = {}
+        self.pf_buf, self.pf_slot_rows, self.pf_next, self.pf_slot_events, self._pf_store = None, 0, 0, [], None
+        self.pf_copied = 0
         assert 1 <= encode_batch <= 16
         self.encode_batch, self.enc_queue, self.enc_inflight = encode_batch, [], []
         self.enc_stream = torch.cuda.Stream(model.engine.device) if encode_batch > 1 else None
@@ -396,10 +405,57 @@
         self.pf_queue = [t for t in self.pf_queue if t.job is not job]
         job.pool.abandon(job, extra_streams=(self.pf_stream,) if self.pf_stream is not None else ())
 
-    def submit_prefill(self, job, h, B, P0, lens=None):
+    PF_RING = 3
+
+    def prefill_rows(self, rows):
+        if self.pf_stream is None:
+            return None
+        eng = self.model.engine
+        D, n = eng.shape.hidden, self.PF_RING * self.prefill_batch
+        cur = torch.cuda.current_stream(eng.device)
+        if self.pf_buf is None or rows != self.pf_slot_rows:
+            if self.pf_queue and self.pf_buf is not None:
+                if rows > self.pf_slot_rows:
+                    return None
+            else:
+                pending = tuple(e for evs in self.pf_slot_events for e in evs if not e.query())
+                need = (n + self.prefill_batch - 1) * rows
+                if self._pf_store is None or self._pf_store.shape[0] < need:
+                    self._pf_store = torch.empty(need, D, dtype=torch.float32, device=eng.device)
+                self.pf_buf = self._pf_store[:need]
+                self.pf_slot_rows, self.pf_next, self.pf_slot_events = rows, 0, [pending] * n
+        s = self.pf_next
+        self.pf_next = (s + 1) % n
+        for e in self.pf_slot_events[s]:
+            if not e.query():
+                cur.wait_event(e)
+        self.pf_slot_events[s] = ()
+        return PassSlot(self.pf_buf, s, s * self.pf_slot_rows)
+
+    def _pass_rows(self, batch):
+        if len(batch) == 1:
+            return batch[0].h
+        buf = self.pf_buf
+        if buf is not None and all(t.slot is not None and t.slot.buf is buf for t in batch):
+            start = [t.slot.row0 for t in batch]
+            end = [t.slot.row0 + int(t.h.shape[0]) for t in batch]
+            breaks = [i for i in range(1, len(batch)) if start[i] != end[i - 1]]
+            if not breaks:
+                return buf[start[0]:end[-1]]
+            ring_end = self.PF_RING * self.prefill_batch * self.pf_slot_rows
+            if len(breaks) == 1 and end[breaks[0] - 1] == ring_end and start[breaks[0]] == 0 and ring_end + end[-1] <= buf.shape[0]:
+                buf[ring_end:ring_end + end[-1]].copy_(buf[:end[-1]])
+                self.pf_copied += len(batch) - breaks[0]
+                return buf[start[0]:ring_end + end[-1]]
+        self.pf_copied += len(batch)
+        return torch.cat([t.h for t in batch])
+
+    def submit_prefill(self, job, h, B, P0, lens=None, slot=None):
         ev = torch.cuda.Event()
         ev.record()
-        t = PrefillTicket(job, h, B, P0, ev, lens)
+        t = PrefillTicket(job, h, B, P0, ev, lens, slot)
+        if slot is not None and slot.buf is self.pf_buf:
+            self.pf_slot_events[slot.index] = (ev,)
         self.pf_queue.append(t)
         return t
 
@@ -439,24 +495,26 @@
                     last += [base + t.P0 + b * t.S + ((t.lens[b] - t.P0) if t.lens is not None else t.S) - 1 for b in range(t.B)]
                     base += int(t.h.shape[0])
                 ragged = any(t.lens is not None for t in batch)
-                logits = eng.llm_prefill_pool_mixed(torch.cat([t.h for t in batch]), groups, pool.kv, pool.R, pool.Smax,
+                logits = eng.llm_prefill_pool_mixed(self._pass_rows(batch), groups, pool.kv, pool.R, pool.Smax,
                                                     last_rows=ops.h2d(torch.tensor(last, dtype=torch.int32), eng.device) if ragged else None)
             elif lead.lens is not None:
                 Mg = lead.h.shape[0]
                 S_ = (Mg - lead.P0) // lead.B
                 last = [g * Mg + lead.P0 + b * S_ + (lead.lens[b] - lead.P0 - 1) for g in range(n) for b in range(lead.B)]
-                logits = eng.llm_prefill_pool_groups(torch.cat([t.h for t in batch]) if n > 1 else lead.h, n, lead.B, lead.P0, pool.kv, pool.R,
+                logits = eng.llm_prefill_pool_groups(self._pass_rows(batch), n, lead.B, lead.P0, pool.kv, pool.R,
                                                      [t.job.r0 for t in batch], pool.Smax, last_rows=ops.h2d(torch.tensor(last, dtype=torch.int32), eng.device))
             elif n == 1:
                 logits = eng.llm_prefill_pool(lead.h, lead.B, lead.P0, pool.kv, pool.R, lead.job.r0, pool.Smax)
             else:
-                logits = eng.llm_prefill_pool_groups(torch.cat([t.h for t in batch]), n, lead.B, lead.P0, pool.kv, pool.R,
+                logits = eng.llm_prefill_pool_groups(self._pass_rows(batch), n, lead.B, lead.P0, pool.kv, pool.R,
                                                      [t.job.r0 for t in batch], pool.Smax)
             ev = torch.cuda.Event()
             ev.record(self.pf_stream)
         eng.slot = prev
         row = 0
         for t in batch:
+            if t.slot is not None and t.slot.buf is self.pf_buf:
+                self.pf_slot_events[t.slot.index] = (ev,)
             t.first = logits[row:row + t.B]
             row += t.B
             t.ready = ev
```

Result: no change. 6586 (median of 2 runs) (-0.1%).
